# google-research/frame-interpolation

Measured on AMD Instinct MI355X. Metric: interpolated frames/sec @1080p, higher is better.
Workload: dtype f32; 1 GPU; 1080p_2x2: 1920x1080 pair, align 64, block_shape [2, 2] -> 4 tile(s) of 960x576 in one batch, film_net published config, seeded synthetic weights, t=0.5; parallelism=1 independent GPU(s), weights RCCL-broadcast once, exec=direct launches, two lanes, lanes=1

## Files before the change

### __graft_entry__.py

```python
import os
import sys

ROOT = os.path.dirname(os.path.abspath(__file__))
PKG = os.path.join(ROOT, 'frame-interpolation_amd')
for _p in (ROOT, PKG):
    if _p not in sys.path:
        sys.path.insert(0, _p)


def build() -> None:
    from film_hip import build as film_build
    out = film_build.build(verbose=True)
    if os.environ.get('FILM_EXTRA_FAMILIES', '0') in ('', '0'):
        os.environ['FILM_EXTRA_FAMILIES'] = '1'
        try:
            print('built', film_build.build(verbose=True))
        finally:
            os.environ['FILM_EXTRA_FAMILIES'] = '0'
    from film_hip import engine
    lib = engine.load_library()
    for sym in engine.EXPORTED_SYMBOLS:
        getattr(lib, sym)
    import eval.interpolator
    print('built', out, engine.FilmEngine.version())


def smoke() -> None:
    import numpy as np
    from film_hip import weights as W
    from film_hip.options import PUBLISHED
    from eval.interpolator import Interpolator
    from oracle import film_oracle as fo

    weights = W.make_synthetic_weights(PUBLISHED, seed=0)
    rng = np.random.default_rng(7)
    x0 = rng.random((1, 64, 64, 3), dtype=np.float32)
    x1 = np.roll(x0, (2, -1), axis=(1, 2)) + rng.normal(0, 0.01, x0.shape).astype(np.float32)
    it = Interpolator('', align=64, weights=weights, device=0)
    got = it(x0, x1, np.full((1,), 0.5, np.float32))
    want = fo.film_forward(x0, x1, weights, fo.Options())
    err = float(np.abs(got - want).max())
    print(f'smoke: hip vs oracle max|d| = {err:.3e}, psnr = {fo.psnr(got, want):.1f} dB')
    assert got.shape == want.shape and np.isfinite(got).all()
    assert err < 1e-3, f'smoke parity failed: {err}'


if __name__ == '__main__':
    if len(sys.argv) > 1 and sys.argv[1] == 'smoke':
        smoke()
    else:
        build()
```

### frame-interpolation_amd/csrc/conv_buf_impl.h

```cpp
#pragma once
#include "conv_common.h"

template <int BM, int BN, int WGM, int WGN, int FLAGS>
__global__ __launch_bounds__(WGM* WGN * 64) void conv_buf_kernel(ConvParams p) {
  constexpr int NW = WGM * WGN, NT = NW * 64;
  constexpr int WTM = BM / WGM, WTN = BN / WGN;
  constexpr int TM = WTM / 32, TN = WTN / 32;
  constexpr int RPP = NT / 4;
  constexpr int AR = BM / RPP;
  constexpr int BR = (BN + RPP - 1) / RPP;
  constexpr int STAGE = (BM + BN) * 16;
  static_assert(BM % RPP == 0 && TM >= 1 && TN >= 1 && RPP % 16 == 0, "bad tile");
  constexpr unsigned OOB = 0xFFFFFFFFu;

  extern __shared__ __attribute__((aligned(1024))) float smem[];

  const int t = threadIdx.x;
  const int lane = t & 63;
  const int wv = __builtin_amdgcn_readfirstlane(t >> 6);
  const int l31 = lane & 31, half = lane >> 5;
  const int wm = wv / WGN, wn = wv % WGN;

  int bx = blockIdx.x, by = blockIdx.y;
  if constexpr ((FLAGS & CONV_B_XCD_M) != 0) conv_xcd_remap(bx, by);
  const int m0 = bx * BM;
  const int n0 = by * BN;

  const int srow = t >> 2;
  const int scol = (t & 3) * 4;
  const int pcol = ((t & 3) ^ ((t >> 4) & 3)) * 4;
  const int ksz = p.ksize;
  const int pad = (ksz - 1) >> 1;
  const int fpy = p.fold == 2 ? (int)(blockIdx.z >> 1) : p.py, fpx = p.fold == 2 ? (int)(blockIdx.z & 1) : p.px;
  const int ntaps = p.fold == 2 ? (fpy + 1) * (fpx + 1) : p.fold ? p.ftaps : ksz * ksz;
  auto tap_dy = [&](int tp) { return p.fold == 2 ? (fpx ? tp >> 1 : tp) : p.fold ? (int)p.tdy[tp] : tp / ksz - pad; };
  auto tap_dx = [&](int tp) { return p.fold == 2 ? (fpx ? tp & 1 : 0) : p.fold ? (int)p.tdx[tp] : tp % ksz - pad; };
  const float* const wbase = p.fold == 2 ? p.w + p.fold_woff[blockIdx.z] : p.w;
  const int ksplit = p.fold ? 1 : (p.ksplit > 1 ? p.ksplit : 1);
  const int split = ksplit > 1 ? (int)blockIdx.z : 0;
  const int HW = p.H * p.W;
  int ab[AR], ay[AR], ax[AR];
  unsigned amask[AR];
#pragma unroll
  for (int i = 0; i < AR; ++i) {
    const int m = m0 + srow + RPP * i;
    const bool valid = m < p.M;
    const int mm = valid ? m : 0;
    const int b = mm / HW;
    const int r = mm - b * HW;
    const int y = r / p.W;
    const int x = r - y * p.W;
    ab[i] = b; ay[i] = y; ax[i] = x;
    unsigned mask = 0;
    for (int tp = 0; tp < ntaps; ++tp) {
      const int yy = y + tap_dy(tp), xx = x + tap_dx(tp);
      if (valid && yy >= 0 && yy < p.H && xx >= 0 && xx < p.W) mask |= 1u << tp;
    }
    amask[i] = mask;
  }
  const int Ktot = ntaps * p.Ctot;
  const conv_rsrc_t brsrc = conv_make_rsrc(wbase);
  unsigned boff[BR];
#pragma unroll
  for (int i = 0; i < BR; ++i) boff[i] = (unsigned)(((n0 + (srow + RPP * i) % BN) * Ktot + scol) * 4);
  const bool bstore = (BN % RPP == 0) || srow < BN;

  int tap = 0, sg = 0, c0 = 0, segC = p.seg[0].C;
  conv_rsrc_t arsrc = conv_make_rsrc(p.seg[0].ptr);
  unsigned aoff[AR];
  unsigned acen[AR];
  auto setup_seg = [&]() {
    const ConvSeg& s = p.seg[sg];
    arsrc = conv_make_rsrc(s.ptr);
    segC = s.C;
    if (!s.up) {
#pragma unroll
      for (int i = 0; i < AR; ++i) {
        int be = ab[i] + s.boff;
        if (s.bmod && be >= s.bmod) be -= s.bmod;
        acen[i] = (unsigned)((((size_t)be * p.H + ay[i]) * p.W + ax[i]) * s.stride + scol) * 4u;
      }
    }
  };
  auto setup_tap = [&]() {
    const ConvSeg& s = p.seg[sg];
    const int dy = tap_dy(tap), dx = tap_dx(tap);
    if (!s.up) {
      const unsigned delta = (unsigned)((dy * p.W + dx) * s.stride * 4);
#pragma unroll
      for (int i = 0; i < AR; ++i) aoff[i] = ((amask[i] >> tap) & 1u) ? acen[i] + delta : OOB;
    } else {
      const int Hs = p.H >> 1, Ws = p.W >> 1;
#pragma unroll
      for (int i = 0; i < AR; ++i) {
        const int yy = (ay[i] + dy) >> 1, xx = (ax[i] + dx) >> 1;
        int be = ab[i] + s.boff;
        if (s.bmod && be >= s.bmod) be -= s.bmod;
        const unsigned off = (unsigned)((((size_t)be * Hs + yy) * Ws + xx) * s.stride + scol) * 4u;
        aoff[i] = ((amask[i] >> tap) & 1u) ? off : OOB;
      }
    }
  };
  auto advance = [&]() {
    c0 += 16;
    if (c0 >= segC) {
      c0 = 0;
      if (++sg == p.nseg) { sg = 0; ++tap; }
      if (p.nseg > 1) setup_seg();
      setup_tap();
    }
  };

  struct Stage {
    bf4 a[AR];
    bf4 b[BR];
  };
  Stage sx, sy;
  const int nsteps_all = ntaps * (p.Ctot / 16);
  const int k_begin = (int)((long long)split * nsteps_all / ksplit);
  const int nsteps = (int)((long long)(split + 1) * nsteps_all / ksplit);
  int kstep = k_begin;
  if (k_begin > 0) {
    const int spt = p.Ctot / 16;
    tap = k_begin / spt;
    int rem = (k_begin - tap * spt) * 16;
    sg = 0;
    while (rem >= p.seg[sg].C) { rem -= p.seg[sg].C; ++sg; }
    c0 = rem;
  }
  auto load_global = [&](Stage& st) {
    const unsigned asoff = (unsigned)c0 * 4u;
#pragma unroll
    for (int i = 0; i < AR; ++i) st.a[i] = conv_buf_load(arsrc, aoff[i], asoff);
    const unsigned bsoff = (unsigned)(kstep < nsteps ? kstep : nsteps - 1) * 64u;
#pragma unroll
    for (int i = 0; i < BR; ++i) st.b[i] = conv_buf_load(brsrc, boff[i], bsoff);
    ++kstep;
    if (kstep < nsteps) advance();
    else {
#pragma unroll
      for (int i = 0; i < AR; ++i) aoff[i] = OOB;
    }
  };
  auto store_lds = [&](const Stage& st, int buf) {
    float* As = smem + buf * STAGE;
    float* Bs = As + BM * 16;
#pragma unroll
    for (int i = 0; i < AR; ++i) *reinterpret_cast<bf4*>(As + (srow + RPP * i) * 16 + pcol) = st.a[i];
    if (bstore) {
#pragma unroll
      for (int i = 0; i < BR; ++i) *reinterpret_cast<bf4*>(Bs + ((srow + RPP * i) % BN) * 16 + pcol) = st.b[i];
    }
  };

  f32x16 acc[TM][TN];
#pragma unroll
  for (int i = 0; i < TM; ++i)
#pragma unroll
    for (int j = 0; j < TN; ++j)
#pragma unroll
      for (int r = 0; r < 16; ++r) acc[i][j][r] = 0.f;

  const int sw = (l31 >> 2) & 3;
  const int ch0 = (half ^ sw) * 4, ch1 = ((2 + half) ^ sw) * 4;
  const int a_row = (wm * WTM + l31) * 16;
  const int b_row = (BM + wn * WTN + l31) * 16;
  auto compute = [&](int buf) {
    const float* S = smem + buf * STAGE;
    bf4 a[2][TM], b[2][TN];
#pragma unroll
    for (int mt = 0; mt < TM; ++mt) {
      a[0][mt] = *reinterpret_cast<const bf4*>(S + a_row + mt * 512 + ch0);
      a[1][mt] = *reinterpret_cast<const bf4*>(S + a_row + mt * 512 + ch1);
    }
#pragma unroll
    for (int nt = 0; nt < TN; ++nt) {
      b[0][nt] = *reinterpret_cast<const bf4*>(S + b_row + nt * 512 + ch0);
      b[1][nt] = *reinterpret_cast<const bf4*>(S + b_row + nt * 512 + ch1);
    }
#pragma unroll
    for (int kq = 0; kq < 2; ++kq)
#pragma unroll
      for (int j = 0; j < 4; ++j)
#pragma unroll
        for (int mt = 0; mt < TM; ++mt)
#pragma unroll
          for (int nt = 0; nt < TN; ++nt)
            acc[mt][nt] = __builtin_amdgcn_mfma_f32_32x32x2f32(b[kq][nt][j], a[kq][mt][j], acc[mt][nt], 0, 0, 0);
  };

  setup_seg();
  setup_tap();
  load_global(sx);
  load_global(sy);
  store_lds(sx, 0);
  __syncthreads();
  for (int s = k_begin; s < nsteps; s += 2) {
    load_global(sx);
    __builtin_amdgcn_sched_barrier(0);
    compute(0);
    __builtin_amdgcn_sched_barrier(0);
    store_lds(sy, 1);
    __syncthreads();
    load_global(sy);
    __builtin_amdgcn_sched_barrier(0);
    compute(1);
    __builtin_amdgcn_sched_barrier(0);
    store_lds(sx, 0);
    __syncthreads();
  }

#pragma unroll
  for (int mt = 0; mt < TM; ++mt) {
    const int m = m0 + wm * WTM + mt * 32 + l31;
    if (m >= p.M) continue;
    size_t opix = (size_t)m;
    if (p.fold) {
      const int bq = m / HW, rr = m - bq * HW, y = rr / p.W, x = rr - y * p.W;
      opix = ((size_t)bq * 2 * p.H + 2 * y + fpy) * (2 * p.W) + 2 * x + fpx;
    }
#pragma unroll
    for (int nt = 0; nt < TN; ++nt)
#pragma unroll
      for (int g = 0; g < 4; ++g) {
        const int n = n0 + wn * WTN + nt * 32 + 8 * g + 4 * half;
        bf4 v;
#pragma unroll
        for (int c = 0; c < 4; ++c) v[c] = acc[mt][nt][4 * g + c];
        if (ksplit > 1) {
          *reinterpret_cast<bf4*>(p.part + ((size_t)split * p.M + m) * p.Cout + n) = v;
          continue;
        }
#pragma unroll
        for (int c = 0; c < 4; ++c) {
          float u = v[c] + p.bias[n + c];
          if (p.leaky) u = leaky02(u);
          v[c] = u;
        }
        *reinterpret_cast<bf4*>(p.out + opix * p.ostride + n) = v;
      }
  }
}

template <int BM, int BN, int WGM, int WGN, int FLAGS>
hipError_t conv_buf_launch(const ConvParams& p, hipStream_t s) {
  constexpr size_t lds = 2 * (size_t)(BM + BN) * 16 * sizeof(float);
  if (p.ksplit > 1 && p.fold) return hipErrorInvalidValue;
  if (p.ksplit > 1 ? (p.Cout % 4 || (reinterpret_cast<uintptr_t>(p.part) & 15)) : (p.ostride % 4 || (reinterpret_cast<uintptr_t>(p.out) & 15))) return hipErrorInvalidValue;
  dim3 grid((p.M + BM - 1) / BM, p.Cout / BN, p.fold == 2 ? 4 : (p.ksplit > 1 ? p.ksplit : 1));
  return conv_launch<conv_buf_kernel<BM, BN, WGM, WGN, FLAGS>>(grid, dim3(WGM * WGN * 64), lds, s, p);
}
```

### frame-interpolation_amd/csrc/conv_common.h

```cpp
#pragma once
#include <atomic>
#include <type_traits>
#include <utility>

#include "film_kernels.h"

typedef float f32x16 __attribute__((ext_vector_type(16)));
typedef float bf4 __attribute__((ext_vector_type(4)));
typedef int bi4 __attribute__((ext_vector_type(4)));

enum : int {
  CONV_B_XCD_M = 4,
};

typedef __amdgpu_buffer_rsrc_t conv_rsrc_t;
__device__ __forceinline__ conv_rsrc_t conv_make_rsrc(const void* p) {
  return __builtin_amdgcn_make_buffer_rsrc(const_cast<void*>(p), 0, -1, 0x00020000);
}

__device__ __forceinline__ bf4 conv_buf_load(conv_rsrc_t rsrc, unsigned voff, unsigned soff) {
  return __builtin_bit_cast(bf4, __builtin_amdgcn_raw_buffer_load_b128(rsrc, (int)voff, (int)soff, 0));
}


struct ConvLdsAttrFlags { std::atomic<bool> set[64]; };
inline hipError_t conv_allow_dynamic_lds(const void* kern, ConvLdsAttrFlags& flags, int bytes) {
  int dev = 0;
  (void)hipGetDevice(&dev);
  const bool tracked = dev >= 0 && dev < 64;
  if (tracked && flags.set[dev].load(std::memory_order_relaxed)) return hipSuccess;
  const hipError_t e = hipFuncSetAttribute(kern, hipFuncAttributeMaxDynamicSharedMemorySize, bytes);
  if (e == hipSuccess && tracked) flags.set[dev].store(true, std::memory_order_relaxed);
  return e;
}

template <auto KERN>
hipError_t conv_launch(dim3 grid, dim3 block, size_t lds, hipStream_t s, const ConvParams& p, size_t lds_allow) {
  if (lds_allow > 64 * 1024) {
    static ConvLdsAttrFlags attr_flags;
    if (const hipError_t e = conv_allow_dynamic_lds(reinterpret_cast<const void*>(KERN), attr_flags, (int)lds_allow); e != hipSuccess) return e;
  }
  hipLaunchKernelGGL(KERN, grid, block, lds, s, p);
  return hipGetLastError();
}
template <auto KERN>
hipError_t conv_launch(dim3 grid, dim3 block, size_t lds, hipStream_t s, const ConvParams& p) { return conv_launch<KERN>(grid, block, lds, s, p, lds); }

inline unsigned conv_magic(unsigned long long d, unsigned long long xmax, bool& exact) {
  if (d <= 1) return 0u;
  if (xmax * d >= (1ull << 32)) { exact = false; return 0u; }
  return (unsigned)(((1ull << 32) + d - 1) / d);
}


template <class F, int... G>
__device__ __forceinline__ void conv_for_each(F&& f, std::integer_sequence<int, G...>) { (f(std::integral_constant<int, G>{}), ...); }

__device__ __forceinline__ unsigned conv_udiv(unsigned x, unsigned magic) {
  unsigned q;
  const unsigned h = __umulhi(x, magic);
  asm("s_cmp_eq_u32 %2, 0\n\ts_cselect_b32 %0, %1, %3" : "=s"(q) : "s"(x), "s"(magic), "s"(h) : "scc");
  return q;
}

__device__ __forceinline__ void conv_xcd_remap(int& bx, int& by) {
  const int nbx = gridDim.x, nby = gridDim.y;
  const int nwg = nbx * nby;
  const int lin = by * nbx + bx;
  const int xcd = lin & 7, idx = lin >> 3;
  const int q = nwg >> 3, r = nwg & 7;
  const int base = xcd < r ? xcd * (q + 1) : r * (q + 1) + (xcd - r) * q;
  const int nl = base + idx;
  bx = nl / nby;
  by = nl - bx * nby;
}
__device__ __forceinline__ float leaky02(float v) { return v > 0.f ? v : 0.2f * v; }

__device__ __forceinline__ const float* conv_uniform_ptr(const float* q) {
  const unsigned long long v = (unsigned long long)(uintptr_t)q;
  return reinterpret_cast<const float*>((uintptr_t)(((unsigned long long)(unsigned)__builtin_amdgcn_readfirstlane((int)(v >> 32)) << 32) |
                                                      (unsigned)__builtin_amdgcn_readfirstlane((int)(unsigned)v)));
}
```

### frame-interpolation_amd/csrc/conv_igemm.hip

```cpp
#include "conv_buf_impl.h"
#include "conv_wino43_impl.h"
#include "conv_wino2d_impl.h"
#include "conv_fold4_impl.h"
#include "conv_c3_impl.h"
#ifdef FILM_EXTRA_FAMILIES
#include "conv_halo_impl.h"
#include "conv_split_impl.h"
#include "conv_wino_impl.h"
#include "conv_winox3_impl.h"
#include "conv_foldx3_impl.h"
#endif

template <int F>
static hipError_t launch_shape(const ConvParams& p, int shape, hipStream_t s) {
  switch (shape) {
    case TILE_128x128: return conv_buf_launch<128, 128, 2, 2, F>(p, s);
    case TILE_256x64: return conv_buf_launch<256, 64, 4, 1, F>(p, s);
    case TILE_256x32: return conv_buf_launch<256, 32, 4, 1, F>(p, s);
    case TILE_64x64: return conv_buf_launch<64, 64, 2, 2, F>(p, s);
    case TILE_128x32: return conv_buf_launch<128, 32, 4, 1, F>(p, s);
    case TILE_128x64: return conv_buf_launch<128, 64, 2, 2, F>(p, s);
    case TILE_256x128: return conv_buf_launch<256, 128, 4, 2, F>(p, s);
    default: return hipErrorInvalidValue;
  }
}

static hipError_t launch_c3(const ConvParams& p, int shape, hipStream_t s) {
  if (shape != TILE_C3_DIRECT) return hipErrorInvalidValue;
  return p.Cout % 64 == 0 ? conv_c3_launch<64>(p, s) : conv_c3_launch<32>(p, s);
}

#ifdef FILM_EXTRA_FAMILIES
template <int F>
static hipError_t launch_halo(const ConvParams& p, int shape, hipStream_t s) {
  switch (shape) {
    case HALO_8x128: return conv_halo_launch<8, 128, 4, 2, F>(p, s);
    case HALO_8x64: return conv_halo_launch<8, 64, 4, 1, F>(p, s);
    case HALO_8x32: return conv_halo_launch<8, 32, 4, 1, F>(p, s);
    case HALO_4x64: return conv_halo_launch<4, 64, 4, 1, F>(p, s);
    case HALO_4x128: return conv_halo_launch<4, 128, 2, 2, F>(p, s);
    case HALO_4x32: return conv_halo_launch<4, 32, 4, 1, F>(p, s);
    default: return hipErrorInvalidValue;
  }
}

template <int F, int NP>
static hipError_t launch_split(const ConvParams& p, int shape, hipStream_t s) {
  switch (shape) {
    case HALO_8x128: return conv_halo_split_launch<8, 128, 4, 2, NP, F>(p, s);
    case HALO_8x64: return conv_halo_split_launch<8, 64, 4, 1, NP, F>(p, s);
    case HALO_8x32: return conv_halo_split_launch<8, 32, 4, 1, NP, F>(p, s);
    case HALO_4x64: return conv_halo_split_launch<4, 64, 4, 1, NP, F>(p, s);
    case HALO_4x128: return conv_halo_split_launch<4, 128, 2, 2, NP, F>(p, s);
    case HALO_4x32: return conv_halo_split_launch<4, 32, 4, 1, NP, F>(p, s);
    default: return hipErrorInvalidValue;
  }
}

template <int F>
static hipError_t launch_wino(const ConvParams& p, int shape, hipStream_t s) {
  switch (shape) {
    case WINO_4x128: return conv_wino_launch<4, 128, 4, 2, F>(p, s);
    case WINO_4x64: return conv_wino_launch<4, 64, 4, 1, F>(p, s);
    case WINO_4x128_W16: return conv_wino_launch<4, 128, 4, 4, F>(p, s);
    case WINO_4x32: return conv_wino_launch<4, 32, 4, 1, F>(p, s);
    case WINO_8x64_W16: return conv_wino_launch<8, 64, 8, 2, F>(p, s);
    case WINO_8x32_W8: return conv_wino_launch<8, 32, 8, 1, F>(p, s);
    case WINO_2x64: return conv_wino_launch<2, 64, 2, 2, F>(p, s);
    case WINO_4x64_W8: return conv_wino_launch<4, 64, 4, 2, F>(p, s);
    default: return hipErrorInvalidValue;
  }
}

#endif

template <int F>
static hipError_t launch_wino43(const ConvParams& p, int shape, hipStream_t s) {
  switch (shape) {
    case W43_Q16_4x64_T21_P2: return conv_wino43_launch<4, 64, 2, 1, F | W43_F_PF2, 16>(p, s);
    case W43_Q16_4x32_T11_P2: return conv_wino43_launch<4, 32, 1, 1, F | W43_F_PF2, 16>(p, s);
    case W43_Q16_4x64_N1_P2: return conv_wino43_launch<4, 64, 1, 1, F | W43_F_PF2, 16, 1>(p, s);
    case W43_Q8_8x64_T21_P2: return conv_wino43_launch<8, 64, 2, 1, F | W43_F_PF2, 8>(p, s);
    case W43_Q8_8x64_N1_P2: return conv_wino43_launch<8, 64, 1, 1, F | W43_F_PF2, 8, 1>(p, s);
    case W43_Q8_8x32_T11_BG: return conv_wino43_launch<8, 32, 1, 1, F | W43_F_BG, 8>(p, s);
    case W43_Q8_8x32_T11_P2: return conv_wino43_launch<8, 32, 1, 1, F | W43_F_PF2, 8>(p, s);
#ifdef FILM_EXTRA_FAMILIES
    case W43_4x64_T21: return conv_wino43_launch<4, 64, 2, 1, F>(p, s);
    case W43_4x64_T12: return conv_wino43_launch<4, 64, 1, 2, F>(p, s);
    case W43_4x32_T11: return conv_wino43_launch<4, 32, 1, 1, F>(p, s);
    case W43_Q16_4x64_T21: return conv_wino43_launch<4, 64, 2, 1, F, 16>(p, s);
    case W43_Q16_4x64_T12: return conv_wino43_launch<4, 64, 1, 2, F, 16>(p, s);
    case W43_Q16_4x32_T11: return conv_wino43_launch<4, 32, 1, 1, F, 16>(p, s);
    case W43_Q16_4x64_N1: return conv_wino43_launch<4, 64, 1, 1, F, 16, 1>(p, s);
    case W43_Q16_4x64_T12_P2: return conv_wino43_launch<4, 64, 1, 2, F | W43_F_PF2, 16>(p, s);
    case W43_Q16_4x32_T11_BG: return conv_wino43_launch<4, 32, 1, 1, F | W43_F_BG, 16>(p, s);
    case W43_Q8_8x64_T12_P2: return conv_wino43_launch<8, 64, 1, 2, F | W43_F_PF2, 8>(p, s);
#endif
    default: return hipErrorInvalidValue;
  }
}

template <int F>
static hipError_t launch_wino2d(const ConvParams& p, int shape, hipStream_t s) {
  switch (shape) {
    case W2D_8x64: return conv_wino2d_launch_any<64, F>(p, s);
    case W2D_8x32: return conv_wino2d_launch_any<32, F>(p, s);
    case W2D_8x32_S2: return conv_wino2d_launch_any<32, F, 2>(p, s);
    case W2D_16x64: return conv_wino2d_launch_any<64, F | W2D_F_SQ>(p, s);
    case W2D_16x32: return conv_wino2d_launch_any<32, F | W2D_F_SQ>(p, s);
    case W2D_16x32_S2: return conv_wino2d_launch_any<32, F | W2D_F_SQ, 2>(p, s);
    default: return hipErrorInvalidValue;
  }
}

template <int F>
static hipError_t launch_fold4(const ConvParams& p, int shape, hipStream_t s) {
  switch (shape) {
    case F4_4x64: return conv_fold4_launch<2, F>(p, s);
    case F4_4x32: return conv_fold4_launch<1, F>(p, s);
    default: return hipErrorInvalidValue;
  }
}

#ifdef FILM_EXTRA_FAMILIES
template <int F>
static hipError_t launch_winox3(const ConvParams& p, int shape, hipStream_t s) {
  switch (shape) {
    case WX3_4x128_T22: return conv_winox3_launch<4, 128, 2, 2, F>(p, s);
    case WX3_4x64_T12: return conv_winox3_launch<4, 64, 1, 2, F>(p, s);
    case WX3_4x64_T21: return conv_winox3_launch<4, 64, 2, 1, F>(p, s);
    case WX3_4x32_T11: return conv_winox3_launch<4, 32, 1, 1, F>(p, s);
    default: return hipErrorInvalidValue;
  }
}

template <int F>
static hipError_t launch_foldx3(const ConvParams& p, int shape, hipStream_t s) {
  switch (shape) {
    case FX3_4x64: return conv_foldx3_launch<4, 64, 4, 1, F>(p, s);
    case FX3_8x64: return conv_foldx3_launch<8, 64, 8, 1, F>(p, s);
    case FX3_4x128: return conv_foldx3_launch<4, 128, 4, 2, F>(p, s);
    default: return hipErrorInvalidValue;
  }
}
#endif


__global__ __launch_bounds__(256) void conv_splitk_reduce_kernel(const float* __restrict__ part, const float* __restrict__ bias,
                                                                 float* __restrict__ out, int M, int Cout, int ostride,
                                                                 int S, int leaky) {
  const int G = Cout >> 2;
  const unsigned idx = blockIdx.x * 256u + threadIdx.x;
  if (idx >= (unsigned)M * (unsigned)G) return;
  const unsigned m = idx / (unsigned)G, g = idx - m * (unsigned)G;
  const size_t plane = (size_t)M * Cout;
  const float4* src = reinterpret_cast<const float4*>(part + (size_t)m * Cout + g * 4);
  float4 a = *reinterpret_cast<const float4*>(bias + g * 4);
  for (int sidx = 0; sidx < S; ++sidx) {
    const float4 v = src[(size_t)sidx * (plane >> 2)];
    a.x += v.x; a.y += v.y; a.z += v.z; a.w += v.w;
  }
  if (leaky) {
    a.x = a.x > 0.f ? a.x : 0.2f * a.x; a.y = a.y > 0.f ? a.y : 0.2f * a.y;
    a.z = a.z > 0.f ? a.z : 0.2f * a.z; a.w = a.w > 0.f ? a.w : 0.2f * a.w;
  }
  *reinterpret_cast<float4*>(out + (size_t)m * ostride + g * 4) = a;
}

static hipError_t film_launch_conv_main(const ConvParams& p, int fam, int tile, hipStream_t s) {
  const int shape = conv_tile_shape(tile);
  const bool xcd = tile & CONV_TILE_XCD;
  if ((p.pool_out != nullptr || p.pw_out != nullptr) && kConvFamily[fam].fused_shape < 0) return hipErrorInvalidValue;
  switch (fam) {
    case FAM_BUF: return xcd ? launch_shape<CONV_B_XCD_M>(p, shape, s) : launch_shape<0>(p, shape, s);
    case FAM_C3: return launch_c3(p, shape, s);
    case FAM_FOLD4: return xcd ? launch_fold4<CONV_B_XCD_M>(p, shape, s) : launch_fold4<0>(p, shape, s);
    case FAM_W2D:
      if (p.ksize != 3) return hipErrorInvalidValue;
      return xcd ? launch_wino2d<CONV_B_XCD_M>(p, shape, s) : launch_wino2d<0>(p, shape, s);
    case FAM_W43:
      if (p.ksize != 3) return hipErrorInvalidValue;
      if (p.pool_out != nullptr && shape < W43_Q16_4x64_T21) return hipErrorInvalidValue;
      if (p.pw_out != nullptr && ((shape != W43_Q16_4x64_N1 && shape != W43_Q16_4x64_N1_P2 && shape != W43_Q8_8x64_N1_P2) || p.Cout != 64 || p.ksplit > 1 ||
                                  p.pool_out != nullptr || p.pw_cout < 1 || p.pw_cout > 4))
        return hipErrorInvalidValue;
      return xcd ? launch_wino43<CONV_B_XCD_M>(p, shape, s) : launch_wino43<0>(p, shape, s);
#ifdef FILM_EXTRA_FAMILIES
    case FAM_HALO:
      if (p.ksize != 3) return hipErrorInvalidValue;
      return xcd ? launch_halo<CONV_B_XCD_M>(p, shape, s) : launch_halo<0>(p, shape, s);
    case FAM_SPLIT6:
      if (p.ksize != 3) return hipErrorInvalidValue;
      return xcd ? launch_split<CONV_B_XCD_M, 6>(p, shape, s) : launch_split<0, 6>(p, shape, s);
    case FAM_SPLIT3:
      if (p.ksize != 3) return hipErrorInvalidValue;
      return xcd ? launch_split<CONV_B_XCD_M, 3>(p, shape, s) : launch_split<0, 3>(p, shape, s);
    case FAM_WINO:
      if (p.ksize != 3) return hipErrorInvalidValue;
      return xcd ? launch_wino<CONV_B_XCD_M>(p, shape, s) : launch_wino<0>(p, shape, s);
    case FAM_WINOX3:
      if (p.ksize != 3) return hipErrorInvalidValue;
      return xcd ? launch_winox3<CONV_B_XCD_M>(p, shape, s) : launch_winox3<0>(p, shape, s);
    case FAM_FOLDX3:
      if (p.ksize != 2 || p.fold != 2) return hipErrorInvalidValue;
      return xcd ? launch_foldx3<CONV_B_XCD_M>(p, shape, s) : launch_foldx3<0>(p, shape, s);
#endif
    default: return hipErrorNotSupported;
  }
}

hipError_t film_launch_conv(const ConvParams& p, int tile, hipStream_t s) {
  const int fam = conv_family_of(tile);
  if (fam < 0 || (p.ksplit > 1 && !kConvFamily[fam].splitk)) return hipErrorInvalidValue;
  const hipError_t e = film_launch_conv_main(p, fam, tile, s);
  if (e != hipSuccess || p.ksplit <= 1) return e;
  const long long Mout = (long long)p.M * (p.fold == 3 ? 4 : 1);
  if (!p.part || (p.Cout & 3) || Mout * (p.Cout >> 2) >= (1ll << 32)) return hipErrorInvalidValue;
  const unsigned units = (unsigned)Mout * (unsigned)(p.Cout >> 2);
  hipLaunchKernelGGL(conv_splitk_reduce_kernel, dim3((units + 255) / 256), dim3(256), 0, s, p.part, p.bias, p.out, (int)Mout, p.Cout,
                     p.ostride, p.ksplit, p.leaky);
  return hipGetLastError();
}
```

### frame-interpolation_amd/csrc/conv_wino2d_impl.h

```cpp
#pragma once
#include "conv_common.h"

enum { W2D_F_SQ = 128,
       W2D_F_XEPI = 8,
       W2D_DBG_TIME = 8192 };


template <bool SQ> struct W2dSlotTable { unsigned v[24 * 64]; };
template <bool SQ> constexpr W2dSlotTable<SQ> w2d_make_slot_table() {
  constexpr int QW = SQ ? 4 : 8, TH = SQ ? 16 : 8, HR = TH + 2, PW = 4 * QW + 2;
  constexpr int CO4 = (PW + 3) / 4, MO4 = 4 * CO4, RP4 = 4 * MO4 + (SQ ? 2 : 4);
  W2dSlotTable<SQ> t{};
  for (int sl = 0; sl < 24 * 64; ++sl) {
    const int r = sl / RP4, rem = sl % RP4, m = rem / MO4, rr = rem % MO4, c = rr / CO4, k = rr % CO4, px = 4 * k + m;
    const bool ok = r < HR && rem < 4 * MO4 && px < PW;
    t.v[sl] = ok ? ((unsigned)r << 24 | (unsigned)px << 8 | (unsigned)c << 4) : 0xFFFFFFFFu;
  }
  return t;
}
template <bool SQ> __device__ const W2dSlotTable<SQ> w2d_slot_table = w2d_make_slot_table<SQ>();

template <int BN, int FLAGS, int NS_ = 3>
__global__ __launch_bounds__(4 * (BN / 32) * 64, (BN == 32) ? 2 : 1) void conv_wino2d_kernel(ConvParams p) {
  constexpr bool SQ = (FLAGS & W2D_F_SQ) != 0;
  constexpr int QW = SQ ? 4 : 8, TH = SQ ? 16 : 8, HR = TH + 2, PXW = 4 * QW, PW = PXW + 2;
  static_assert(QW * (TH / 2) == 32, "32 units per tile");
  constexpr int NG = BN / 32, NW = 4 * NG;
  constexpr int CO4 = (PW + 3) / 4, MO4 = 4 * CO4, RP4 = 4 * MO4 + (SQ ? 2 : 4);
  constexpr int NREQ = 24;
  constexpr int STAGE4 = NREQ * 64;
  constexpr int NS = NS_;
  static_assert(NS == 2 || NS == 3, "stages");
  constexpr int IPW = NREQ / NW;
  static_assert(NREQ % NW == 0, "requests per wave");
  static_assert(HR * RP4 <= STAGE4, "stage size");
  constexpr bool XE = (FLAGS & W2D_F_XEPI) != 0;
  constexpr unsigned OOB = 0xFFFFFFFFu;

  extern __shared__ __attribute__((aligned(1024))) float smem[];

  const int t = threadIdx.x;
  const int lane = t & 63;
  const int wv = __builtin_amdgcn_readfirstlane(t >> 6);
  const int l31 = lane & 31, half = lane >> 5;
  const int mu = wv & 3, ng = wv >> 2;

  unsigned long long tm0 = 0, tm1 = 0, tm2 = 0, tmA = 0, tmB = 0, tmC = 0, tmW = 0, tmE1 = 0, tmE2 = 0, tmE3 = 0;
  unsigned long long rt0 = 0;
  if constexpr ((FLAGS & W2D_DBG_TIME) != 0) { rt0 = __builtin_amdgcn_s_memrealtime(); tm0 = __builtin_readcyclecounter(); }

  int aH = p.H, aW = p.W, aNB = p.NB, aCtot = p.Ctot, aKsplit = p.ksplit, aNseg = p.nseg, aUnused = p.unused_chain;
  unsigned a_tpi = p.mg_tpi, a_ntx = p.mg_ntx, a_nby = p.mg_nby;
  int ntx_ = p.tl_ntx, tpi_ = p.tl_tpi;
  int aGx = (int)gridDim.x, aGy = (int)gridDim.y;
  const float* aS0ptr = p.seg[0].ptr;
  int aS0stride = p.seg[0].stride, aS0C = p.seg[0].C, aS0boff = p.seg[0].boff, aS0bmod = p.seg[0].bmod;
  const float* aWptr = p.w;
  unsigned rtab[(24 / (4 * (BN / 32)))];
#pragma unroll
  for (int n = 0; n < 24 / NW; ++n) rtab[n] = w2d_slot_table<SQ>.v[t + 64 * NW * n];
  {
    unsigned long long q0 = (unsigned long long)(uintptr_t)aS0ptr, q1 = (unsigned long long)(uintptr_t)aWptr;
    asm volatile("" : "+s"(aH), "+s"(aW), "+s"(aNB), "+s"(aCtot), "+s"(aKsplit), "+s"(aNseg), "+s"(aUnused), "+s"(a_tpi), "+s"(a_ntx), "+s"(a_nby), "+s"(ntx_), "+s"(tpi_),
                      "+s"(aGx), "+s"(aGy), "+s"(q0), "+s"(q1), "+s"(aS0stride), "+s"(aS0C), "+s"(aS0boff), "+s"(aS0bmod));
    aS0ptr = reinterpret_cast<const float*>((uintptr_t)q0);
    aWptr = reinterpret_cast<const float*>((uintptr_t)q1);
  }
  unsigned long long tmK = 0, tmT = 0;
  if constexpr ((FLAGS & W2D_DBG_TIME) != 0) tmK = __builtin_readcyclecounter();
  int bx = blockIdx.x, by = blockIdx.y;
  if constexpr ((FLAGS & CONV_B_XCD_M) != 0) {
    const int nbx = aGx, nby = aGy;
    const int nwg = nbx * nby;
    const int lin = by * nbx + bx;
    const int xcd = lin & 7, idx = lin >> 3;
    const int q = nwg >> 3, r = nwg & 7;
    const int base = xcd < r ? xcd * (q + 1) : r * (q + 1) + (xcd - r) * q;
    const int nl = base + idx;
    bx = (int)conv_udiv((unsigned)nl, a_nby);
    by = nl - bx * nby;
  }
  const int ntx = ntx_, tpi = tpi_;
  const int img = (int)conv_udiv((unsigned)bx, a_tpi);
  const int trow0 = (int)conv_udiv((unsigned)(bx - img * tpi), a_ntx);
  const int y0 = trow0 * TH, x0 = (bx - img * tpi - trow0 * ntx) * PXW;
  const int n0 = by * BN;

  unsigned rvoff[IPW];
  int rsg = 0, rc0 = 0, rsegC = 0;
  conv_rsrc_t rrsrc = conv_make_rsrc(conv_uniform_ptr(aS0ptr));
  const unsigned lds0 = (unsigned)(size_t)(__attribute__((address_space(3))) float*)smem;
  unsigned rpk[IPW];
  auto set_rpk = [&]() {
    const int H = aH, W = aW;
    const bool inside = y0 >= 1 && y0 + TH + 1 <= H && x0 >= 1 && x0 + PXW + 1 <= W;
    if (inside) {
#pragma unroll
      for (int n = 0; n < IPW; ++n) rpk[n] = rtab[n];
    } else {
#pragma unroll
      for (int n = 0; n < IPW; ++n) {
        const unsigned tv = rtab[n];
        const unsigned y = (unsigned)(y0 - 1) + (tv >> 24), x = (unsigned)(x0 - 1) + ((tv >> 8) & 255u);
        rpk[n] = ((y < (unsigned)H) & (x < (unsigned)W)) ? tv : OOB;
      }
    }
  };
  set_rpk();
#pragma unroll
  for (int n = 0; n < IPW; ++n) asm volatile("" : "+v"(rpk[n]));
  if constexpr ((FLAGS & W2D_DBG_TIME) != 0) tmT = __builtin_readcyclecounter();
  auto raw_setup_seg_of = [&](const float* sptr, int sstride, int sC, int sboff, int sbmod) {
    rsegC = __builtin_amdgcn_readfirstlane(sC);
    int be = img + sboff;
    if (sbmod && be >= sbmod) be -= sbmod;
    const int spix = (be * aH + (y0 - 1)) * aW + (x0 - 1);
    rrsrc = conv_make_rsrc(conv_uniform_ptr(sptr + (long long)spix * sstride));
    const unsigned st4 = (unsigned)sstride * 4u;
    const unsigned wst4 = (unsigned)aW * st4;
#pragma unroll
    for (int n = 0; n < IPW; ++n) {
      const unsigned tv = rpk[n];
      unsigned off, tmp;
      asm("v_and_b32 %0, 48, %2\n\tv_bfe_u32 %1, %2, 8, 8\n\tv_mad_u32_u24 %0, %1, %3, %0\n\tv_lshrrev_b32 %1, 24, %2\n\tv_mad_u32_u24 %0, %1, %4, %0"
          : "=&v"(off), "=&v"(tmp) : "v"(tv), "s"(st4), "s"(wst4));
      rvoff[n] = tv == OOB ? OOB : off;
    }
  };
  auto raw_setup_seg = [&]() {
    const ConvSeg& s = p.seg[rsg];
    raw_setup_seg_of(s.ptr, s.stride, s.C, s.boff, s.bmod);
  };
  auto dma_piece = [&](int n, int stage) {
    const unsigned so = (unsigned)rc0 * 4u;
    const unsigned base = lds0 + (unsigned)stage * (STAGE4 * 16u) + (unsigned)(wv + NW * n) * 1024u;
    asm volatile("s_mov_b32 m0, %0\n\ts_nop 0\n\tbuffer_load_dwordx4 %1, %2, %3 offen lds" ::"s"(base), "v"(rvoff[n]), "s"(rrsrc), "s"(so)
                 : "memory");
  };
  auto dma_advance = [&]() {
    rc0 += 16;
    if (rc0 >= rsegC) {
      if (rsg + 1 < aNseg) { rc0 = 0; ++rsg; raw_setup_seg(); }
    }
  };
  const int ksp = XE && aKsplit > 1 ? aKsplit : 1;
  const int nsc_all = aCtot >> 4;
  int sc0 = 0, sc1 = nsc_all;
  if (ksp > 1) {
    sc0 = (int)((unsigned)nsc_all * blockIdx.z / (unsigned)ksp);
    sc1 = (int)((unsigned)nsc_all * (blockIdx.z + 1u) / (unsigned)ksp);
    int c = sc0 * 16;
    while (rsg + 1 < aNseg && c >= p.seg[rsg].C) { c -= p.seg[rsg].C; ++rsg; }
    rc0 = c;
  }
  auto raw_issue = [&](int stage) {
#pragma unroll
    for (int n = 0; n < IPW; ++n) dma_piece(n, stage);
    dma_advance();
  };

  const int nkc = aCtot / 8, nsc = sc1 - sc0, kc0 = 2 * sc0, kc1 = 2 * sc1;
  const conv_rsrc_t brsrc = conv_make_rsrc(conv_uniform_ptr(aWptr));
  const unsigned bvoff = (unsigned)((half * 32 + l31) * 16);
  const int ct = n0 / 32 + ng;
  auto slab = [&](int kc) { return (unsigned)(((ct * nkc + (kc < nkc ? kc : nkc - 1)) * 4 + mu) * 6) * 1024u; };
  bf4 fbg[2][6];

  f32x16 acc[6];

  const bf4* const smem4 = reinterpret_cast<const bf4*>(smem);
  const int ur = l31 / QW, lq = l31 % QW;
  const int ra = mu == 0 ? 0 : mu == 2 ? 2 : 1, rb = mu == 0 ? 2 : mu == 1 ? 2 : mu == 2 ? 1 : 3;
  const float sgn = mu == 1 ? 1.f : -1.f;
  const int ix_a = (2 * ur + ra) * RP4 + half * CO4 + lq, ix_b = (2 * ur + rb) * RP4 + half * CO4 + lq;
  typedef float f2 __attribute__((ext_vector_type(2)));
  f2 A[2][6][2];
  bf4 d[6];
  bf4 d2[6];

  using C0 = std::integral_constant<int, 0>;
  using C1 = std::integral_constant<int, 1>;
  auto read_row = [&](bf4 (&dst)[6], int ix, int stage, auto h_c) {
    constexpr int IMM = decltype(h_c)::value * 2 * CO4;
    const int ixs = ix + stage * STAGE4;
#pragma unroll
    for (int j = 0; j < 6; ++j) dst[j] = smem4[ixs + IMM + (j & 3) * MO4 + (j >> 2)];
  };
  auto pair_of = [](const bf4& v, int q) -> f2 { return q ? f2{v[2], v[3]} : f2{v[0], v[1]}; };
  auto set_pair = [](bf4& v, int q, f2 x) { if (q) { v[2] = x[0]; v[3] = x[1]; } else { v[0] = x[0]; v[1] = x[1]; } };
  auto fma2 = [](float k, f2 x, f2 y) -> f2 {
    f2 r;
    const f2 kk = {k, k};
    asm("v_pk_fma_f32 %0, %1, %2, %3" : "=v"(r) : "s"(kk), "v"(x), "v"(y));
    return r;
  };
  auto add2 = [](f2 x, f2 y) -> f2 { f2 r; asm("v_pk_add_f32 %0, %1, %2" : "=v"(r) : "v"(x), "v"(y)); return r; };
  auto mul2 = [](float k, f2 x) -> f2 {
    f2 r;
    const f2 kk = {k, k};
    asm("v_pk_mul_f32 %0, %1, %2" : "=v"(r) : "s"(kk), "v"(x));
    return r;
  };
  auto max1 = [](float x, float y) -> float { float r; asm("v_max_f32 %0, %1, %2" : "=v"(r) : "v"(x), "v"(y)); return r; };
  auto sub2 = [](f2 x, f2 y) -> f2 { f2 r; asm("v_pk_add_f32 %0, %1, %2 neg_lo:[0,1] neg_hi:[0,1]" : "=v"(r) : "v"(x), "v"(y)); return r; };
  f2 xt[4];
  auto xf_t = [&](int q) {
    const f2 d1 = pair_of(d[1], q), d2v = pair_of(d[2], q), d3 = pair_of(d[3], q), d4 = pair_of(d[4], q);
    xt[0] = fma2(-4.f, d2v, d4);
    xt[1] = fma2(-4.f, d1, d3);
    xt[2] = sub2(d4, d2v);
    xt[3] = sub2(d3, d1);
  };
  auto xf_v = [&](int q, int nu) -> f2 {
    switch (nu) {
      case 0: return fma2(4.f, pair_of(d[0], q), fma2(-5.f, pair_of(d[2], q), pair_of(d[4], q)));
      case 1: return add2(xt[0], xt[1]);
      case 2: return sub2(xt[0], xt[1]);
      case 3: return fma2(2.f, xt[3], xt[2]);
      case 4: return fma2(-2.f, xt[3], xt[2]);
      default: return fma2(4.f, pair_of(d[1], q), fma2(-5.f, pair_of(d[3], q), pair_of(d[5], q)));
    }
  };
  auto pin = [](f2& v) { asm volatile("" : "+v"(v)); };
  auto prepare = [&](f2 (&An)[6][2], int stage, auto h_c) {
    read_row(d, ix_a, stage, h_c);
    read_row(d2, ix_b, stage, h_c);
#pragma unroll
    for (int j = 0; j < 6; ++j)
#pragma unroll
      for (int q = 0; q < 2; ++q) set_pair(d[j], q, fma2(sgn, pair_of(d2[j], q), pair_of(d[j], q)));
#pragma unroll
    for (int q = 0; q < 2; ++q) {
      xf_t(q);
#pragma unroll
      for (int nu = 0; nu < 6; ++nu) An[nu][q] = xf_v(q, nu);
    }
  };

  if (ksp > 1) raw_setup_seg();
  else raw_setup_seg_of(aS0ptr, aS0stride, aS0C, aS0boff, aS0bmod);
  raw_issue(0);
  if constexpr ((FLAGS & W2D_DBG_TIME) != 0) tmA = __builtin_readcyclecounter();
#pragma unroll
  for (int j = 0; j < 6; ++j) fbg[0][j] = conv_buf_load(brsrc, bvoff, slab(kc0) + (unsigned)j * 1024u);
  __builtin_amdgcn_sched_barrier(0);
  asm volatile("s_waitcnt vmcnt(6)" ::: "memory");
  if constexpr ((FLAGS & W2D_DBG_TIME) != 0) tmB = __builtin_readcyclecounter();
  __syncthreads();
  if constexpr ((FLAGS & W2D_DBG_TIME) != 0) tmC = __builtin_readcyclecounter();
#pragma unroll
  for (int j = 0; j < 6; ++j) fbg[1][j] = conv_buf_load(brsrc, bvoff, slab(kc0 + 1) + (unsigned)j * 1024u);
  __builtin_amdgcn_sched_barrier(0);
  if (nsc > 1) raw_issue(1);
  if constexpr (NS > 2) { if (nsc > 2) raw_issue(2); }
  prepare(A[0], 0, C0{});

  int st_s = 0, st_n = 1;
  int st_dma = 0;
  bool dma_on = false;
  int gs = 0;
  constexpr int P1 = NS == 2 ? IPW : (IPW + 1) / 2, P0 = IPW - P1;
  auto dma_slot = [](int g, int cnt) constexpr -> int {
    if (cnt <= 0) return -1;
    if (cnt == 6) return g == 2 ? 0 : (g >= 5 && (g - 5) % 4 == 0) ? 1 + (g - 5) / 4 : -1;
    const int step = 24 / cnt, at = cnt == 1 ? 13 : 5;
    return (g % step == at && g / step < cnt) ? g / step : -1;
  };
  auto chunk = [&](int kc, auto h_c, auto first_c, auto last_c) {
    constexpr int H = decltype(h_c)::value;
    constexpr bool FIRST = decltype(first_c)::value != 0;
    constexpr bool LAST = decltype(last_c)::value != 0;
    constexpr bool PREP = !(LAST && H == 1);
    using RH = std::integral_constant<int, 1 - H>;
    const int rs = H == 0 ? st_s : st_n;
    f2(&Ac)[6][2] = A[H];
    f2(&An)[6][2] = A[1 - H];
    if constexpr (H == 1 && !LAST) {
      unsigned long long tw0 = 0;
      if constexpr ((FLAGS & W2D_DBG_TIME) != 0) tw0 = __builtin_readcyclecounter();
      if (NS == 2 || gs == 0) asm volatile("s_waitcnt vmcnt(6)" ::: "memory");
      else asm volatile("s_waitcnt vmcnt(12)" ::: "memory");
      __syncthreads();
      if constexpr ((FLAGS & W2D_DBG_TIME) != 0) tmW += __builtin_readcyclecounter() - tw0;
      dma_on = (kc >> 1) + NS < sc1;
      st_dma = st_s;
    }
    const unsigned so2 = LAST ? 0u : slab(kc + 2);
    __builtin_amdgcn_sched_barrier(0);
    auto gap = [&](auto g_c) {
      constexpr int g = decltype(g_c)::value;
      constexpr int jp = g >> 3, i8 = g & 7, k = i8 >> 1, j = 2 * jp + (i8 & 1);
      if constexpr (FIRST && k == 0) {
        const f32x16 zero = {0.f, 0.f, 0.f, 0.f, 0.f, 0.f, 0.f, 0.f, 0.f, 0.f, 0.f, 0.f, 0.f, 0.f, 0.f, 0.f};
        acc[j] = __builtin_amdgcn_mfma_f32_32x32x2f32(fbg[H][j][k], Ac[j][k >> 1][k & 1], zero, 0, 0, 0);
      } else {
        acc[j] = __builtin_amdgcn_mfma_f32_32x32x2f32(fbg[H][j][k], Ac[j][k >> 1][k & 1], acc[j], 0, 0, 0);
      }
      if constexpr (!LAST) {
        if constexpr (k == 3) fbg[H][j] = conv_buf_load(brsrc, bvoff, so2 + (unsigned)j * 1024u);
      }
      if constexpr (PREP) {
        if constexpr (g == 0) read_row(d, ix_a, rs, RH{});
        if constexpr (g == 1) read_row(d2, ix_b, rs, RH{});
        if constexpr (g >= 4 && g < 10) {
          constexpr int jj = g - 4;
#pragma unroll
          for (int q = 0; q < 2; ++q) { f2 v = fma2(sgn, pair_of(d2[jj], q), pair_of(d[jj], q)); pin(v); set_pair(d[jj], q, v); }
        }
        if constexpr (g >= 10 && g < 16) {
          constexpr int q = (g - 10) / 3, part = (g - 10) % 3;
          if constexpr (part == 0) {
            xf_t(q);
            pin(xt[0]); pin(xt[1]); pin(xt[2]); pin(xt[3]);
          } else if constexpr (part == 1) {
            An[0][q] = xf_v(q, 0);
            An[5][q] = xf_v(q, 5);
            pin(An[0][q]); pin(An[5][q]);
          } else {
#pragma unroll
            for (int nu = 1; nu < 5; ++nu) { An[nu][q] = xf_v(q, nu); pin(An[nu][q]); }
          }
        }
      }
      if constexpr (!LAST) {
        constexpr int CNT = H == 1 ? P1 : P0, N0 = H == 1 ? 0 : P1;
        constexpr int idx = dma_slot(g, CNT);
        if constexpr (idx >= 0) {
          if (dma_on) {
            dma_piece(N0 + idx, st_dma);
            if constexpr (N0 + idx == IPW - 1) dma_advance();
          }
        }
      }
      __builtin_amdgcn_sched_barrier(0);
    };
    conv_for_each(gap, std::make_integer_sequence<int, 24>{});
    if constexpr (H == 1) {
      st_s = st_n;
      st_n = st_n + 1 == NS ? 0 : st_n + 1;
      ++gs;
    }
  };

  auto epilogue = [&]() {
    const int t = threadIdx.x, lane = t & 63, l31 = lane & 31, half = lane >> 5;
    __syncthreads();
    if constexpr ((FLAGS & W2D_DBG_TIME) != 0) tmE1 = __builtin_readcyclecounter();
    float o[4][16];
  #pragma unroll
    for (int r = 0; r < 16; ++r) {
      const float m0 = acc[0][r], m1 = acc[1][r], m2 = acc[2][r], m3 = acc[3][r], m4 = acc[4][r], m5 = acc[5][r];
      const float s34 = m3 + m4, d34 = m3 - m4, d12 = m1 - m2, s12 = m1 + m2;
      o[0][r] = ((m0 + m1) + m2) + s34;
      o[1][r] = __builtin_fmaf(2.f, d34, d12);
      o[2][r] = __builtin_fmaf(4.f, s34, s12);
      o[3][r] = d12 + __builtin_fmaf(8.f, d34, m5);
    }
    bf4* const xb = reinterpret_cast<bf4*>(smem);
    constexpr int XB4 = NG * 4 * 256;
    static_assert(2 * XB4 <= NS * STAGE4, "exchange buffers");
    const int widx = (ng * 4 + mu) * 256 + l31 * 8;
    const int rng = t >> 8, run = (t >> 3) & 31, rcg = t & 7;
    const int ridx = rng * 1024 + run * 8 + (rcg ^ (run & 7));
    const int nrd = n0 + rng * 32 + rcg * 4;
    const bool rawsum = XE && ksp > 1;
    const bool has_pw = XE && p.pw_out != nullptr;
    float b0 = 0.f, b1 = 0.f, b2 = 0.f, b3 = 0.f;
    if (!rawsum) { const float* const bp = p.bias + nrd; b0 = bp[0]; b1 = bp[1]; b2 = bp[2]; b3 = bp[3]; }
    const int oy = y0 + 2 * (run / QW), ox = x0 + 4 * (run % QW);
    const int ostr = rawsum ? p.Cout : p.ostride;
    const float slope = (p.leaky && !rawsum) ? 0.2f : 1.f;
    const int dyo = 2 * (run / QW), dxo = 4 * (run % QW), nth = rng * 32 + rcg * 4;
    const int cpix = (img * p.H + y0) * p.W + x0;
    float* obase = p.out;
    if (rawsum) { asm volatile(""); obase = p.part + (size_t)blockIdx.z * p.M * p.Cout; }
    float* const ocorner = obase + ((long long)cpix * ostr + n0);
    float* const orow = ocorner + (__umul24(__umul24(dyo, p.W) + dxo, ostr) + nth);
    float* pool_base = nullptr;
    if (XE && p.pool_out) {
      asm volatile("");
      const int ppix = (img * (p.H >> 1) + (y0 >> 1)) * (p.W >> 1) + (x0 >> 1);
      pool_base = p.pool_out + ((long long)ppix * p.pool_ostride + n0) + (__umul24(__umul24(dyo >> 1, p.W >> 1) + (dxo >> 1), p.pool_ostride) + nth);
    }
    constexpr int PWS = 68;
    float* const pwt = smem + 2 * XB4 * 4;
    float* const pww = pwt + TH * PXW * PWS;
    if (has_pw && t < 256) pww[t] = (t & 3) < p.pw_cout ? p.pw_w[(t >> 2) * p.pw_cout + (t & 3)] : 0.f;
    bf4 k0 = {0.f, 0.f, 0.f, 0.f}, k1 = {0.f, 0.f, 0.f, 0.f};
    auto write_round = [&](int jx, bf4* xw) {
  #pragma unroll
      for (int g = 0; g < 4; ++g) {
        bf4 v;
        v[0] = o[jx][4 * g]; v[1] = o[jx][4 * g + 1]; v[2] = o[jx][4 * g + 2]; v[3] = o[jx][4 * g + 3];
        xw[widx + ((2 * g + half) ^ (l31 & 7))] = v;
      }
    };
  #pragma unroll
    for (int jx = 0; jx < 4; ++jx) {
      bf4* const xw = xb + (jx & 1) * XB4;
      write_round(jx, xw);
      __syncthreads();
      if constexpr ((FLAGS & W2D_DBG_TIME) != 0) { if (jx == 0) tmE2 = __builtin_readcyclecounter(); if (jx == 3) tmE3 = __builtin_readcyclecounter(); }
      const bf4 m0 = xw[ridx], m1 = xw[ridx + 256], m2 = xw[ridx + 512], m3 = xw[ridx + 768];
      bf4 r0, r1;
  #pragma unroll
      for (int q = 0; q < 2; ++q) {
        const f2 bq = q ? f2{b2, b3} : f2{b0, b1};
        const f2 v0 = add2(add2(add2(pair_of(m0, q), pair_of(m1, q)), pair_of(m2, q)), bq);
        const f2 v1 = add2(sub2(sub2(pair_of(m1, q), pair_of(m2, q)), pair_of(m3, q)), bq);
        const f2 s0 = mul2(slope, v0), s1 = mul2(slope, v1);
        set_pair(r0, q, f2{max1(v0[0], s0[0]), max1(v0[1], s0[1])});
        set_pair(r1, q, f2{max1(v1[0], s1[0]), max1(v1[1], s1[1])});
      }
      if (!has_pw) {
        if (ox + jx < p.W) {
          float* const o0 = orow + (size_t)jx * ostr;
          if (oy < p.H) *reinterpret_cast<bf4*>(o0) = r0;
          if (oy + 1 < p.H) *reinterpret_cast<bf4*>(o0 + (size_t)p.W * ostr) = r1;
        }
        if (XE && pool_base != nullptr) {
          if (jx & 1) {
            bf4 pv;
  #pragma unroll
            for (int c = 0; c < 4; ++c) pv[c] = (((k0[c] + r0[c]) + k1[c]) + r1[c]) * 0.25f;
            if (oy < p.H && ox + jx < p.W) *reinterpret_cast<bf4*>(pool_base + (size_t)(jx >> 1) * p.pool_ostride) = pv;
          } else {
            k0 = r0; k1 = r1;
          }
        }
      } else {
        float* const tr = pwt + ((2 * (run / QW)) * PXW + 4 * (run % QW) + jx) * PWS + rng * 32 + rcg * 4;
        *reinterpret_cast<bf4*>(tr) = r0;
        *reinterpret_cast<bf4*>(tr + PXW * PWS) = r1;
      }
    }
    if (has_pw) {
      __syncthreads();
      if (t < TH * PXW) {
        const int y = y0 + t / PXW, x = x0 + (t % PXW);
        float a[4] = {0.f, 0.f, 0.f, 0.f};
        const bf4* row = reinterpret_cast<const bf4*>(pwt + t * PWS);
        const bf4* wq = reinterpret_cast<const bf4*>(pww);
  #pragma unroll 4
        for (int c4 = 0; c4 < 16; ++c4) {
          const bf4 v = row[c4];
  #pragma unroll
          for (int k = 0; k < 4; ++k) {
            const bf4 w = wq[c4 * 4 + k];
  #pragma unroll
            for (int j = 0; j < 4; ++j) a[j] = __builtin_fmaf(v[k], w[j], a[j]);
          }
        }
        if (y < p.H && x < p.W) {
          float* dd = p.pw_out + (((size_t)img * p.H + y) * p.W + x) * p.pw_ostride;
  #pragma unroll
          for (int j = 0; j < 4; ++j)
            if (j < p.pw_cout) dd[j] = a[j] + p.pw_bias[j];
        }
      }
    }
  };
  if constexpr ((FLAGS & W2D_DBG_TIME) != 0) tm1 = __builtin_readcyclecounter();
  for (int tile = 0; tile < 1; ++tile) {
    chunk(kc0, C0{}, C1{}, C0{});
    chunk(kc0 + 1, C1{}, C0{}, C0{});
    for (int kc = kc0 + 2; kc < kc1 - 2; kc += 2) {
      chunk(kc, C0{}, C0{}, C0{});
      chunk(kc + 1, C1{}, C0{}, C0{});
    }
    if (nsc > 1) {
      chunk(kc1 - 2, C0{}, C0{}, C1{});
      chunk(kc1 - 1, C1{}, C0{}, C1{});
    }
    if constexpr ((FLAGS & W2D_DBG_TIME) != 0) tm2 = __builtin_readcyclecounter();
    epilogue();
  }
  if constexpr ((FLAGS & W2D_DBG_TIME) != 0) {
    const unsigned long long tm3 = __builtin_readcyclecounter();
    if (t == 0) {
      unsigned long long* o8 = reinterpret_cast<unsigned long long*>(p.part) + (size_t)(blockIdx.y * gridDim.x + blockIdx.x) * 16;
      o8[0] = tm0; o8[1] = tm1; o8[2] = tm2; o8[3] = tm3; o8[4] = tmA; o8[5] = tmB; o8[6] = tmC; o8[7] = tmW;
      o8[8] = rt0; o8[9] = __builtin_amdgcn_s_memrealtime();
      o8[10] = (unsigned long long)__builtin_amdgcn_s_getreg((31 << 11) | 4) | ((unsigned long long)__builtin_amdgcn_s_getreg((31 << 11) | 20) << 32);
      o8[11] = tmE1; o8[12] = tmE2; o8[13] = tmE3; o8[14] = tmK; o8[15] = tmT;
    }
  }
}

template <int BN, int FLAGS, int NS = 3>
hipError_t conv_wino2d_launch(const ConvParams& p, hipStream_t s) {
  if (!(FLAGS & W2D_F_XEPI) && (p.ksplit > 1 || p.pool_out || p.pw_out)) return hipErrorInvalidValue;
  const size_t lds = p.pw_out ? (size_t)2 * (BN / 32) * 16 * 1024 + 256 * 68 * 4 + 1024 : (size_t)NS * 24 * 1024;
  constexpr int NT = 4 * (BN / 32) * 64;
  if (p.ksize != 3 || p.Ctot % 16 || p.Cout % BN) return hipErrorInvalidValue;
  if (p.ksplit > 1 && (!p.part || (reinterpret_cast<uintptr_t>(p.part) & 15) || p.Cout % 4 || p.pool_out || p.pw_out || p.ksplit > p.Ctot / 16)) return hipErrorInvalidValue;
  if (p.pw_out) {
    if (BN != 64 || p.Cout != 64 || p.pool_out || p.pw_cout < 1 || p.pw_cout > 4) return hipErrorInvalidValue;
  } else if (p.ostride % 4 || (reinterpret_cast<uintptr_t>(p.out) & 15)) return hipErrorInvalidValue;
  if (p.pool_out && ((p.H | p.W) & 1 || p.pool_ostride % 4 || (reinterpret_cast<uintptr_t>(p.pool_out) & 15))) return hipErrorInvalidValue;
  {
    long long nimg = p.NB;
    for (int i = 0; i < p.nseg; ++i) nimg = std::max<long long>(nimg, (long long)p.seg[i].bmod);
    if ((nimg + 1) * p.H * p.W >= (1ll << 31)) return hipErrorInvalidValue;
  }
  if (p.W <= 0 || p.H <= 0 || p.W >= (1 << 20) || p.ostride >= (1 << 22) || p.pool_ostride >= (1 << 22) || p.Cout >= (1 << 22) ||
      (long long)8 * p.W * (p.ostride > p.Cout ? p.ostride : p.Cout) >= (1ll << 31)) return hipErrorInvalidValue;
  for (int i = 0; i < p.nseg; ++i)
    if ((long long)p.W * p.seg[i].stride * 4 >= (1ll << 24) || p.seg[i].C % 16 || p.seg[i].stride % 4 || p.seg[i].stride <= 0 || p.seg[i].stride >= (1 << 22) || p.seg[i].up || (reinterpret_cast<uintptr_t>(p.seg[i].ptr) & 15)) return hipErrorInvalidValue;
  constexpr bool SQ = (FLAGS & W2D_F_SQ) != 0;
  const int ntx = SQ ? (p.W + 15) / 16 : (p.W + 31) / 32, nty = SQ ? (p.H + 15) / 16 : (p.H + 7) / 8;
  const int ntiles = p.NB * ntx * nty;
  dim3 grid((unsigned)ntiles, p.Cout / BN, (unsigned)(p.ksplit > 1 ? p.ksplit : 1));
  ConvParams q = p;
  bool exact = true;
  q.mg_nby = conv_magic(grid.y, (unsigned long long)grid.x * grid.y, exact);
  q.mg_tpi = conv_magic((unsigned long long)ntx * nty, (unsigned long long)ntiles + 1, exact);
  q.mg_ntx = conv_magic(ntx, (unsigned long long)ntx * nty, exact);
  q.tl_ntx = ntx; q.tl_tpi = ntx * nty;
  if (!exact) return hipErrorInvalidValue;
  return conv_launch<conv_wino2d_kernel<BN, FLAGS, NS>>(grid, dim3(NT), lds, s, q, 144 * 1024);
}

template <int BN, int FLAGS, int NS = 3>
hipError_t conv_wino2d_launch_any(const ConvParams& p, hipStream_t s) {
  if (p.ksplit > 1 || p.pool_out || p.pw_out) return conv_wino2d_launch<BN, FLAGS | W2D_F_XEPI, NS>(p, s);
  return conv_wino2d_launch<BN, FLAGS, NS>(p, s);
}
```

### frame-interpolation_amd/csrc/film_engine.cpp

```cpp
#include "film_internal.h"

namespace film_internal {

thread_local std::string g_create_error;

int fail(film_t* h, int code, const char* fmt, ...) {
  char buf[1024];
  va_list ap;
  va_start(ap, fmt);
  vsnprintf(buf, sizeof buf, fmt, ap);
  va_end(ap);
  if (h) h->err = buf; else g_create_error = buf;
  return code;
}

int copy_out_string(film_t* h, const std::string& s, char* buf, int64_t cap, int64_t* needed) {
  if (needed) *needed = (int64_t)s.size() + 1;
  if (!buf || cap < (int64_t)s.size() + 1) {
    if (!buf && needed) return FILM_OK;
    return fail(h, FILM_ERR_INVALID, "buffer too small: need %lld bytes", (long long)s.size() + 1);
  }
  memcpy(buf, s.c_str(), s.size() + 1);
  return FILM_OK;
}

}

using namespace film_internal;

namespace {

enum OptNorm { AS_IS, BOOL, NONNEG, LOW5 };
struct OptionRow {
  const char* key;
  int film_t::*field;
  OptNorm norm;
  bool drops_plans;
  int64_t lo = 0, hi = 0;
  const char* refusal = nullptr;
  ConvFamily family = FAM_BUF;
  int need_lo = 0, need_hi = 0;
  const char* family_refusal = nullptr;
};
constexpr OptionRow kOptions[] = {
    {"graph", &film_t::opt_graph, AS_IS, false, 0, 2, "graph: 0 (one stream, eager), 1 (hipGraph replay) or 2 (two lanes, eager: the default)"},
    {"profile", &film_t::opt_profile, BOOL, false},
    {"autotune", &film_t::opt_autotune, BOOL, false},
    {"max_batch", &film_t::opt_max_batch, NONNEG, false},
    {"host_overlap", &film_t::opt_host_overlap, BOOL, false},
    {"block_overlap_h", &film_t::opt_block_overlap_h, AS_IS, false, -1, 65535, "block_overlap_h: -1 (what the align padding of a tile holds) or 0 .. 65535 rows"},
    {"block_overlap_w", &film_t::opt_block_overlap_w, AS_IS, false, -1, 65535, "block_overlap_w: -1 (what the align padding of a tile holds) or 0 .. 65535 columns"},
    {"tune_ms", &film_t::opt_tune_ms, NONNEG, false},
    {"splitk", &film_t::opt_splitk, BOOL, true},
    {"pack_groups", nullptr, AS_IS, false, 1, 4, "pack_groups: 1 .. 4"},
    {"fuse", &film_t::opt_fuse, LOW5, true},
    {"fold2x2", &film_t::opt_fold2x2, AS_IS, true, 0, 2, "fold2x2: 0, 1 or 2"},
    {"planar", &film_t::opt_planar, BOOL, true},
    {"winograd", &film_t::opt_wino, AS_IS, true, 0, 3, "winograd: 0, 1, 2 or 3", FAM_WINO, 2, 2,
     "winograd = 2 (F(2,3) kernel on every level) needs a library built with FILM_EXTRA_FAMILIES=1"},
    {"halo_all", &film_t::opt_halo_all, BOOL, true, 0, 0, nullptr, FAM_HALO, 1, 1, "halo_all needs a library built with FILM_EXTRA_FAMILIES=1"},
    {"lanes", &film_t::opt_lanes, AS_IS, true, 0, 3, "lanes: 0, 1, 2 or 3"},
    {"wino2d", &film_t::opt_wino2d, AS_IS, true, 0, 2, "wino2d: 0, 1 or 2"},
    {"w2d_small_px", &film_t::opt_w2d_small_px, AS_IS, true, 0, 1 << 30, "w2d_small_px: pixels per image, 0 = never"},
    {"w2d_min_px", &film_t::opt_w2d_min_px, AS_IS, true, 1, 1 << 30, "w2d_min_px: pixels per image"},
    {"w2d_splitk", &film_t::opt_w2d_splitk, AS_IS, true, 0, 16, "w2d_splitk: 0 (off), 1 (default rule) or 2..16 (A/B: the cap on levels of <= 1024 pixels)"},
    {"w2d_shape", &film_t::opt_w2d_shape, AS_IS, true, -1, W2D_SHAPES - 1, "w2d_shape: -1 (autotuned) or a Wino2dTile shape index"},
    {"fold4_shape", &film_t::opt_fold4_shape, AS_IS, true, -1, F4_4x32, "fold4_shape: -1 (autotuned) or a Fold4Tile shape index"},
    {"w43_shape", &film_t::opt_w43_shape, AS_IS, true, -1, 31, "w43_shape: -1 (autotuned) or a Wino43Tile shape index"},
    {"precision", &film_t::opt_precision, AS_IS, true, 0, 2, "precision: 0 (f32), 1 (bf16x6) or 2 (bf16x3)", FAM_SPLIT6, 1, 2,
     "precision %d (bf16 split modes) needs a library built with FILM_EXTRA_FAMILIES=1; this build runs fp32 MFMA only"},
};
constexpr bool option_rows_complete() {
  for (const OptionRow& o : kOptions)
    if ((o.lo < o.hi) != (o.refusal != nullptr) || ((o.family != FAM_BUF) != (o.family_refusal != nullptr))) return false;
  return true;
}
static_assert(option_rows_complete(), "a row with a range (a family) carries its refusal message, a row without leaves lo = hi (family = FAM_BUF)");

int tile_geometry(film_t* h, int H, int W, int block_h, int block_w, int align, TileMapParams* tp) {
  const int bh = block_h > 0 ? block_h : 1, bw = block_w > 0 ? block_w : 1;
  if (H % bh) return fail(h, FILM_ERR_INVALID, "block_height=%d should evenly divide height=%d.", bh, H);
  if (W % bw) return fail(h, FILM_ERR_INVALID, "block_width=%d should evenly divide width=%d.", bw, W);
  tp->H = H; tp->W = W; tp->bh = bh; tp->bw = bw; tp->ph = H / bh; tp->pw = W / bw;
  struct Axis { const char* key; int nb, p, want; int *ov, *e, *T, *off; };
  const Axis axes[2] = {{"block_overlap_h", bh, tp->ph, h->opt_block_overlap_h, &tp->ovy, &tp->eh, &tp->TH, &tp->oy},
                        {"block_overlap_w", bw, tp->pw, h->opt_block_overlap_w, &tp->ovx, &tp->ew, &tp->TW, &tp->ox}};
  for (const Axis& a : axes) {
    const int pad0 = (align > 0 && a.p % align) ? align - a.p % align : 0;
    const int o = a.nb == 1 ? 0 : a.want < 0 ? std::min(pad0 / 2, a.p / 2) : a.want;
    if (2 * (int64_t)o > a.p)
      return fail(h, FILM_ERR_INVALID, "%s: twice the overlap (%d) must not exceed the patch size %d", a.key, o, a.p);
    const int e = a.p + 2 * o;
    const int pad = (align > 0 && e % align) ? align - e % align : 0;
    *a.ov = o; *a.e = e; *a.T = e + pad; *a.off = pad / 2;
  }
  return FILM_OK;
}
hipError_t cut_tiles(const TileMapParams& tp, hipStream_t s) {
  return (tp.ovy | tp.ovx) ? film_launch_frame_to_tiles_overlap(tp, s) : film_launch_frame_to_tiles(tp, s);
}
hipError_t join_tiles(const TileMapParams& tp, hipStream_t s) {
  return (tp.ovy | tp.ovx) ? film_launch_blend_tiles(tp, s) : film_launch_tiles_to_frame(tp, s);
}
int pix_layout(int pix) { return pix & 0xff; }
bool pix_is_yuv(int pix) { return pix_layout(pix) == FILM_PIX_I420 || pix_layout(pix) == FILM_PIX_NV12; }
int check_pix(film_t* h, int pix, int H, int W) {
  const int layout = pix_layout(pix), flags = pix & ~0xff;
  if (layout != FILM_PIX_F32 && layout != FILM_PIX_U8 && !pix_is_yuv(pix))
    return fail(h, FILM_ERR_INVALID, "bad pix layout %d: FILM_PIX_F32 (0), FILM_PIX_U8 (1), FILM_PIX_I420 (16) or FILM_PIX_NV12 (17)", layout);
  if (flags & ~(FILM_YUV_BT601 | FILM_YUV_FULL))
    return fail(h, FILM_ERR_INVALID, "bad pix 0x%x: unknown bits 0x%x set (flags: FILM_YUV_BT601 0x100, FILM_YUV_FULL 0x400)", (unsigned)pix,
                (unsigned)(flags & ~(FILM_YUV_BT601 | FILM_YUV_FULL)));
  if (flags && !pix_is_yuv(pix))
    return fail(h, FILM_ERR_INVALID, "bad pix 0x%x: the colour flags belong to FILM_PIX_I420 / FILM_PIX_NV12, not to an RGB layout", (unsigned)pix);
  if (pix_is_yuv(pix) && H > 0 && W > 0 && ((H | W) & 1))
    return fail(h, FILM_ERR_INVALID, "pix: 4:2:0 needs even sizes, got %d x %d", H, W);
  return FILM_OK;
}
size_t frame_bytes(int pix, int H, int W) {
  const size_t px = (size_t)H * W;
  return pix_is_yuv(pix) ? px + px / 2 : pix_layout(pix) == FILM_PIX_U8 ? px * 3 : px * 3 * sizeof(float);
}
hipError_t cut_tiles_pix(const TileMapParams& tp, int pix, hipStream_t s) {
  if (pix_layout(pix) == FILM_PIX_F32) return cut_tiles(tp, s);
  const uint8_t* src = reinterpret_cast<const uint8_t*>(tp.src);
  if (pix_is_yuv(pix))
    return film_launch_yuv420_to_tiles(tp, src, pix_layout(pix) == FILM_PIX_NV12, (pix & FILM_YUV_BT601) != 0, (pix & FILM_YUV_FULL) != 0, s);
  return (tp.ovy | tp.ovx) ? film_launch_frame_to_tiles_overlap_u8(tp, src, s) : film_launch_frame_to_tiles_u8(tp, src, s);
}
int ensure_stage(film_t* h, size_t bytes, hipStream_t s) {
  if (h->stage_bytes >= bytes) return FILM_OK;
  if (h->stage) { HIPCHK(h, hipStreamSynchronize(s)); HIPCHK(h, hipFree(h->stage)); h->stage = nullptr; h->stage_bytes = 0; }
  hipError_t e = hipMalloc(&h->stage, bytes);
  if (e != hipSuccess) return fail(h, FILM_ERR_NOMEM, "frame staging hipMalloc of %.1f MB failed", bytes * 1e-6);
  h->stage_bytes = bytes;
  return FILM_OK;
}
int balanced_chunk(int n, int maxc) {
  if (n <= maxc) return n;
  for (int c = maxc; 2 * c > maxc; --c)
    if (n % c == 0) return c;
  return maxc;
}
void sequence_chunk(int n, int T, int cap, int* k, int* nt) {
  int bk = 0, bt = 1;
  for (int t = std::min(T, cap); t >= 1; --t) {
    const int kk = std::min(n, cap / t);
    if (kk > bk) { bk = kk; bt = t; }
  }
  *k = balanced_chunk(n, std::max(bk, 1));
  *nt = balanced_chunk(T, bt);
}
int need_device(film_t* h, const char* fn) {
  if (h->plan_only) return fail(h, FILM_ERR_NO_DEVICE, "plan-only handle: %s needs a HIP device (no CPU fallback)", fn);
  if (!h->finalized) return fail(h, FILM_ERR_STATE, "film_finalize has not been called");
  return FILM_OK;
}
bool halve_on_nomem(int rc, int* chunk) {
  if (rc != FILM_ERR_NOMEM || *chunk <= 1) return false;
  *chunk = (*chunk + 1) / 2;
  return true;
}
struct FrameStage {
  film_t* h; hipStream_t s; bool host;
  float* result; size_t out_floats;
  float* out = nullptr;
  size_t used = 0;
  int open(size_t in_floats) {
    out = result;
    if (!host) return FILM_OK;
    int rc = ensure_stage(h, (in_floats + out_floats) * sizeof(float), s);
    if (rc == FILM_OK) out = (float*)h->stage + in_floats;
    return rc;
  }
  int upload(const float* src, size_t floats, const float** dev) {
    *dev = src;
    if (!host) return FILM_OK;
    HIPCHK(h, hipMemcpyAsync((float*)h->stage + used, src, floats * sizeof(float), hipMemcpyHostToDevice, s));
    *dev = (float*)h->stage + used;
    used += floats;
    return FILM_OK;
  }
  int finish() {
    if (!host) return FILM_OK;
    HIPCHK(h, hipMemcpyAsync(result, out, out_floats * sizeof(float), hipMemcpyDeviceToHost, s));
    HIPCHK(h, hipStreamSynchronize(s));
    return FILM_OK;
  }
};
template <class T> struct TileCopy { T* frames; int tile0, ntiles; int64_t slot; };
using Cut = TileCopy<const float>;
using Join = TileCopy<float>;
int run_chunk(film_t* h, Plan* P, TileMapParams tp, const std::vector<Cut>& cuts, const std::vector<Join>& joins, hipStream_t s) {
  const int64_t tile_floats = (int64_t)tp.TH * tp.TW * 3;
  for (const Cut& c : cuts) {
    tp.tile0 = c.tile0; tp.ntiles = c.ntiles; tp.src = c.frames; tp.dst = P->at("img0") + c.slot * tile_floats;
    HIPCHK(h, cut_tiles(tp, s));
  }
  int rc = run_plan(h, P, s);
  if (rc) return rc;
  for (const Join& j : joins) {
    tp.tile0 = j.tile0; tp.ntiles = j.ntiles; tp.src = P->at("out") + j.slot * tile_floats; tp.dst = j.frames;
    HIPCHK(h, join_tiles(tp, s));
  }
  return FILM_OK;
}

hipStream_t pick_stream(film_t* h, int mem_kind, void* stream) {
  return stream ? (hipStream_t)stream : (mem_kind == FILM_MEM_DEVICE ? (hipStream_t) nullptr : h->stream);
}

int forward_chunk(film_t* h, const float* x0, const float* x1, int B, int H, int W, float* out, int mem_kind, void* stream) {
  HIPCHK(h, hipSetDevice(h->device));
  Plan* P = nullptr;
  int rc = get_plan(h, B, H, W, true, &P);
  if (rc) return rc;
  hipStream_t s = pick_stream(h, mem_kind, stream);
  const size_t in_bytes = (size_t)B * H * W * 3 * sizeof(float);
  const hipMemcpyKind kin = mem_kind == FILM_MEM_HOST ? hipMemcpyHostToDevice : hipMemcpyDeviceToDevice;
  const hipMemcpyKind kout = mem_kind == FILM_MEM_HOST ? hipMemcpyDeviceToHost : hipMemcpyDeviceToDevice;
  HIPCHK(h, hipMemcpyAsync(P->at("img0"), x0, in_bytes, kin, s));
  HIPCHK(h, hipMemcpyAsync(P->at("img0") + (int64_t)B * H * W * 3, x1, in_bytes, kin, s));
  rc = run_plan(h, P, s);
  if (rc) return rc;
  HIPCHK(h, hipMemcpyAsync(out, P->at("out"), in_bytes, kout, s));
  if (mem_kind == FILM_MEM_HOST) HIPCHK(h, hipStreamSynchronize(s));
  return FILM_OK;
}

int interpolate_host_pipeline(film_t* h, Plan* P, TileMapParams tp, const float* x0, const float* x1, float* out, float* st, size_t frame_bytes, hipStream_t s) {
  const int nt = P->B;
  const size_t nf = frame_bytes / sizeof(float);
  for (hipEvent_t& e : h->pipe_ev)
    if (!e) HIPCHK(h, hipEventCreateWithFlags(&e, hipEventDisableTiming));
  LanePipe lp;
  for (size_t i = 0; i < P->ops.size() && lp.head.size() < 2; ++i) {
    const OpDesc& op = P->ops[i];
    if (op.lane == 1) continue;
    if (!batch_splittable(op, 2) || !op.xdeps.empty() || op.NB != 2 * nt) break;
    lp.head.push_back(i);
  }
  const OpDesc& last = P->ops.back();
  lp.tail = tp.B == 1 && tp.bh % 2 == 0 && last.lane == 0 && last.pw_out.buf >= 0 && last.NB == nt && batch_splittable(last, 2) && P->ops.size() > lp.head.size() + 1 &&
            std::find(lp.head.begin(), lp.head.end(), P->ops.size() - 1) == lp.head.end();
  tp.tile0 = 0;
  lp.mid_tail = [&]() -> hipError_t {
    TileMapParams t2 = tp;
    t2.ntiles = nt / 2; t2.src = P->at("out"); t2.dst = st + 2 * nf;
    hipError_t e = film_launch_tiles_to_frame(t2, s);
    if (e == hipSuccess) e = hipEventRecord(h->pipe_ev[1], s);
    return e;
  };
  struct Drain {
    film_t* h; hipStream_t s; bool armed;
    ~Drain() { if (armed) { (void)hipStreamSynchronize(h->stream2); (void)hipStreamSynchronize(s); } }
  } drain{h, s, true};
  HIPCHK(h, hipMemcpyAsync(st, x0, frame_bytes, hipMemcpyHostToDevice, s));
  tp.ntiles = nt; tp.src = st; tp.dst = P->at("img0");
  HIPCHK(h, film_launch_frame_to_tiles(tp, s));
  HIPCHK(h, hipEventRecord(h->pipe_ev[0], s));
  HIPCHK(h, hipStreamWaitEvent(h->stream2, h->pipe_ev[0], 0));
  for (size_t i : lp.head) HIPCHK(h, launch_op(batch_part(P->ops[i], 0, 2), P->arena, h->packed_dev, s));
  HIPCHK(h, hipMemcpyAsync(st + nf, x1, frame_bytes, hipMemcpyHostToDevice, h->stream2));
  tp.src = st + nf; tp.dst = P->at("img0") + (int64_t)nt * tp.TH * tp.TW * 3;
  HIPCHK(h, film_launch_frame_to_tiles(tp, h->stream2));
  HIPCHK(h, hipEventRecord(h->pipe_ev[0], h->stream2));
  HIPCHK(h, hipStreamWaitEvent(s, h->pipe_ev[0], 0));
  const hipError_t le = issue_lanes(h, P, s, false, &lp);
  if (le != hipSuccess) return fail(h, FILM_ERR_HIP, "kernel launch failed: %s", hipGetErrorString(le));
  h->last_plan = P;
  const int64_t tile_floats = (int64_t)tp.TH * tp.TW * 3;
  if (lp.tail) {
    TileMapParams t2 = tp;
    t2.tile0 = nt / 2; t2.ntiles = nt - nt / 2; t2.src = P->at("out") + (int64_t)(nt / 2) * tile_floats; t2.dst = st + 2 * nf;
    HIPCHK(h, film_launch_tiles_to_frame(t2, s));
    const size_t half = frame_bytes / 2;
    HIPCHK(h, hipStreamWaitEvent(h->stream2, h->pipe_ev[1], 0));
    HIPCHK(h, hipMemcpyAsync(out, st + 2 * nf, half, hipMemcpyDeviceToHost, h->stream2));
    HIPCHK(h, hipMemcpyAsync((char*)out + half, (const char*)(st + 2 * nf) + half, frame_bytes - half, hipMemcpyDeviceToHost, s));
    HIPCHK(h, hipStreamSynchronize(h->stream2));
  } else {
    tp.tile0 = 0; tp.ntiles = nt; tp.src = P->at("out"); tp.dst = st + 2 * nf;
    HIPCHK(h, film_launch_tiles_to_frame(tp, s));
    HIPCHK(h, hipMemcpyAsync(out, st + 2 * nf, frame_bytes, hipMemcpyDeviceToHost, s));
  }
  HIPCHK(h, hipStreamSynchronize(s));
  drain.armed = false;
  return FILM_OK;
}

void stream_free(film_t* h) {
  FilmStream& fs = h->fs;
  for (void* p : {fs.keep, (void*)fs.result, (void*)fs.result8})
    if (p) (void)hipFree(p);
  fs = FilmStream{};
}
bool same_geometry(const TileMapParams& a, const TileMapParams& b) {
  const int va[] = {a.H, a.W, a.bh, a.bw, a.ph, a.pw, a.TH, a.TW, a.oy, a.ox, a.ovy, a.ovx, a.eh, a.ew};
  const int vb[] = {b.H, b.W, b.bh, b.bw, b.ph, b.pw, b.TH, b.TW, b.oy, b.ox, b.ovy, b.ovx, b.eh, b.ew};
  return std::equal(std::begin(va), std::end(va), std::begin(vb));
}
hipError_t stream_cut(const FilmStream& fs, TileMapParams tp, const Plan* P, int slot, hipStream_t s) {
  tp.tile0 = 0; tp.ntiles = tp.bh * tp.bw;
  tp.src = (const float*)fs.keep;
  tp.dst = P->at("img0") + (int64_t)slot * tp.ntiles * tp.TH * tp.TW * 3;
  return cut_tiles_pix(tp, fs.pix, s);
}

int debug_plan(film_t* h, int B, int H, int W, int tiles, Plan** P) {
  if (h->plan_only) return fail(h, FILM_ERR_NO_DEVICE, "plan-only handle has no device");
  if (!h->finalized) return fail(h, FILM_ERR_STATE, "weights are not finalized");
  if (tiles < 0 || (tiles > 0 && B % tiles)) return fail(h, FILM_ERR_INVALID, "tiles must be 0 (pair plan) or divide B (sequence plan)");
  HIPCHK(h, hipSetDevice(h->device));
  return get_plan(h, B, H, W, true, P, tiles);
}

}

extern "C" {

int film_to_uint8(const float* src, unsigned char* dst, int64_t n, void* stream) {
  if (n < 0 || (n > 0 && (!src || !dst))) return FILM_ERR_INVALID;
  return film_launch_to_uint8(src, dst, n, (hipStream_t)stream) == hipSuccess ? FILM_OK : FILM_ERR_HIP;
}

int film_to_yuv420(const float* src, void* dst, int H, int W, int pix, void* stream) {
  if (!src || !dst || H < 1 || W < 1 || !pix_is_yuv(pix) || check_pix(nullptr, pix, H, W) != FILM_OK) return FILM_ERR_INVALID;
  return film_launch_rgb_to_yuv420(src, static_cast<uint8_t*>(dst), H, W, pix_layout(pix) == FILM_PIX_NV12, (pix & FILM_YUV_BT601) != 0,
                                   (pix & FILM_YUV_FULL) != 0, (hipStream_t)stream) == hipSuccess ? FILM_OK : FILM_ERR_HIP;
}

#ifndef FILM_SRC_ID
#define FILM_SRC_ID "unknown"
#endif
#ifdef FILM_EXTRA_FAMILIES
#define FILM_FLAVOUR "+extra"
#else
#define FILM_FLAVOUR ""
#endif
const char* film_version(void) { return "gfx950;film_hip r6;src=" FILM_SRC_ID FILM_FLAVOUR; }

int film_default_config(film_config* cfg) {
  if (!cfg) return FILM_ERR_INVALID;
  memset(cfg, 0, sizeof *cfg);
  cfg->pyramid_levels = 7; cfg->fusion_pyramid_levels = 5; cfg->specialized_levels = 3; cfg->sub_levels = 4;
  cfg->filters = 64;
  const int fcv[4] = {3, 3, 3, 3}, ffl[4] = {32, 64, 128, 256};
  for (int i = 0; i < 4; ++i) { cfg->flow_convs[i] = fcv[i]; cfg->flow_filters[i] = ffl[i]; }
  return FILM_OK;
}

int film_create(film_t** out, int device, const film_config* cfg) {
  if (!out) return fail(nullptr, FILM_ERR_INVALID, "out is NULL");
  *out = nullptr;
  std::unique_ptr<film_handle> h(new film_handle);
  if (cfg) h->cfg = *cfg; else film_default_config(&h->cfg);
  int rc = validate_config(h.get(), h->cfg);
  if (rc) { g_create_error = h->err; return rc; }
  h->device = device;
  h->plan_only = device < 0;
  if (!h->plan_only) {
    int ndev = 0;
    hipError_t e = hipGetDeviceCount(&ndev);
    if (e != hipSuccess || ndev <= 0)
// ... 458 lines not shown
```

### frame-interpolation_amd/csrc/film_exec.cpp

```cpp
#include "film_internal.h"

namespace film_internal {
namespace {
inline const float* cptr(const float* base, const View& v) { return base + v.off; }
inline float* mptr(float* base, const View& v) { return base + v.off; }
}

hipError_t launch_op(const OpDesc& op, float* arena, const float* wts, hipStream_t s) {
  switch (op.kind) {
    case OP_CONV: {
      ConvParams p{};
      p.nseg = op.nseg;
      for (int i = 0; i < op.nseg; ++i) {
        p.seg[i].ptr = cptr(arena, op.seg[i].v);
        p.seg[i].stride = op.seg[i].v.stride;
        p.seg[i].C = op.seg[i].v.C;
        p.seg[i].boff = op.seg[i].boff; p.seg[i].bmod = op.seg[i].bmod; p.seg[i].up = op.seg[i].up;
      }
      p.ksize = op.ksize;
      p.w = wts + op.*kConvFamily[op.family].weights;
      p.bias = wts + op.b_off;
      p.out = mptr(arena, op.out); p.ostride = op.out.stride;
      p.NB = op.NB; p.H = op.H; p.W = op.W; p.Cout = op.Cout; p.Ctot = op.Ctot; p.leaky = op.leaky;
      p.M = op.NB * op.H * op.W;
      p.fold = op.fold; p.py = op.py; p.px = op.px; p.ftaps = op.ftaps;
      p.ksplit = op.ksplit; p.part = op.ksplit > 1 ? arena + op.part_off : nullptr;
      if (op.out2.buf >= 0) { p.pool_out = mptr(arena, op.out2); p.pool_ostride = op.out2.stride; }
      if (op.pw_out.buf >= 0) {
        p.pw_w = wts + op.w2_off; p.pw_bias = wts + op.b2_off; p.pw_out = mptr(arena, op.pw_out); p.pw_ostride = op.pw_out.stride; p.pw_cout = op.pw_cout;
      }
      for (int q = 0; q < 4; ++q) { p.tdy[q] = (signed char)op.tdy[q]; p.tdx[q] = (signed char)op.tdx[q]; p.fold_woff[q] = op.fold_woff[q]; }
      return film_launch_conv(p, op.tile, s);
    }
    case OP_FLOW_HEAD: {
      FlowHeadParams p{};
      p.in = cptr(arena, op.in); p.istride = op.in.stride; p.Cin = op.Ctot;
      p.w3 = wts + op.w_off; p.b3 = wts + op.b_off; p.w4 = wts + op.w2_off; p.b4 = wts + op.b2_off;
      p.out = mptr(arena, op.out); p.M = (int)op.n;
      if (op.out2.buf >= 0) { p.add = cptr(arena, op.in2); p.sum = mptr(arena, op.out2); }
      return film_launch_flow_head(p, s);
    }
    case OP_CONV_PW: {
      ConvPwParams p{};
      p.in = cptr(arena, op.in); p.istride = op.in.stride; p.Cin = op.Ctot;
      p.w = wts + op.w_off; p.bias = wts + op.b_off;
      p.out = mptr(arena, op.out); p.ostride = op.out.stride; p.Cout = op.Cout; p.leaky = op.leaky;
      p.M = (int)op.n;
      if (op.out2.buf >= 0) { p.add = cptr(arena, op.in2); p.sum = mptr(arena, op.out2); }
      return film_launch_conv_pw(p, s);
    }
    case OP_POOL: {
      PoolParams p{};
      p.in = cptr(arena, op.in); p.istride = op.in.stride; p.out = mptr(arena, op.out); p.ostride = op.out.stride;
      p.C = op.in.C; p.NB = op.NB; p.H = op.H; p.W = op.W;
      return film_launch_pool(p, s);
    }
    case OP_FLOW_UP: {
      FlowUpParams p{};
      p.in = cptr(arena, op.in); p.out = mptr(arena, op.out); p.NB = op.NB; p.h = op.H; p.w = op.W;
      return film_launch_flow_up(p, s);
    }
    case OP_FLOW_ADD: {
      FlowAddParams p{};
      p.a = cptr(arena, op.in); p.b = cptr(arena, op.in2); p.out = mptr(arena, op.out); p.n = op.n;
      return film_launch_flow_add(p, s);
    }
    case OP_WARP: {
      WarpParams p{};
      p.src = cptr(arena, op.in); p.sstride = op.in.stride; p.C = op.in.C;
      p.flow = op.in2.buf >= 0 ? cptr(arena, op.in2) : nullptr; p.fscale = op.fscale;
      p.dst = mptr(arena, op.out); p.dstride = op.out.stride;
      p.NB = op.NB; p.H = op.H; p.W = op.W;
      p.src_brot = op.src_brot; p.flow_brot = op.flow_brot; p.misc_nb = op.misc_nb;
      if (op.in3.buf >= 0) { p.coarse = cptr(arena, op.in3); p.flow_out = mptr(arena, op.out2); }
      if (op.img_out.buf >= 0) {
        p.src3 = cptr(arena, op.img_in); p.s3stride = op.img_in.stride;
        p.src3b = p.src3 + (int64_t)(op.misc_nb > 0 ? op.misc_nb : op.NB) * op.H * op.W * op.img_in.stride;
        p.dst3 = mptr(arena, op.img_out); p.d3stride = op.img_out.stride;
        p.pack_b = cptr(arena, op.pack_b); p.pack_f = cptr(arena, op.pack_f);
      }
      return film_launch_warp(p, s);
    }
    case OP_PACK_FLOW: {
      PackFlowParams p{};
      p.bflow = cptr(arena, op.in); p.fflow = cptr(arena, op.in2);
      p.dst = mptr(arena, op.out); p.dstride = op.out.stride; p.npix = op.n;
      return film_launch_pack_flow(p, s);
    }
  }
  return hipErrorInvalidValue;
}

bool batch_splittable(const OpDesc& op, int nparts) {
  return op.kind == OP_CONV && op.nseg == 1 && op.seg[0].bmod == 0 && op.seg[0].boff == 0 && op.seg[0].up == 0 && op.ksplit <= 1 && op.fold == 0 &&
         op.NB >= nparts && op.NB % nparts == 0 && (op.out2.buf < 0 || (!(op.H & 1) && !(op.W & 1)));
}
OpDesc batch_part(const OpDesc& op, int part, int nparts) {
  OpDesc q = op;
  q.NB = op.NB / nparts;
  const int64_t px = (int64_t)part * q.NB * op.H * op.W;
  q.seg[0].v.off += px * op.seg[0].v.stride;
  q.out.off += px * op.out.stride;
  if (op.out2.buf >= 0) q.out2.off += (int64_t)part * q.NB * (op.H / 2) * (op.W / 2) * op.out2.stride;
  if (op.pw_out.buf >= 0) q.pw_out.off += px * op.pw_out.stride;
  return q;
}

hipError_t issue_lanes(film_t* h, Plan* P, hipStream_t main, bool capturing, const LanePipe* lp) {
  const size_t nops = P->ops.size();
  if (P->lane_ev.size() < nops + 2) P->lane_ev.resize(nops + 2, nullptr);
  hipError_t ev_err = hipSuccess;
  auto event_of = [&](size_t i) -> hipEvent_t {
    if (!P->lane_ev[i]) {
      hipError_t e = hipEventCreateWithFlags(&P->lane_ev[i], hipEventDisableTiming);
      if (e != hipSuccess) { ev_err = e; P->lane_ev[i] = nullptr; }
    }
    return P->lane_ev[i];
  };
  const bool two_lanes = h->opt_lanes != 0;
  hipError_t le = hipSuccess;
  if (two_lanes) {
    le = hipEventRecord(event_of(nops), main);
    if (le == hipSuccess) le = hipStreamWaitEvent(h->stream2, event_of(nops), 0);
  }
  for (size_t i = 0; i < nops && le == hipSuccess; ++i) {
    const OpDesc& op = P->ops[i];
    const int lane = (two_lanes && op.lane == 1) ? 1 : 0;
    hipStream_t ls = lane ? h->stream2 : main;
    if (two_lanes)
      for (int d : op.xdeps) {
        le = hipStreamWaitEvent(ls, event_of((size_t)d), 0);
        if (le != hipSuccess) break;
      }
    if (le != hipSuccess) break;
    if (lp && std::find(lp->head.begin(), lp->head.end(), i) != lp->head.end()) le = launch_op(batch_part(op, 1, 2), P->arena, h->packed_dev, ls);
    else if (lp && lp->tail && i + 1 == nops) {
      le = launch_op(batch_part(op, 0, 2), P->arena, h->packed_dev, ls);
      if (le == hipSuccess) le = lp->mid_tail();
      if (le == hipSuccess) le = launch_op(batch_part(op, 1, 2), P->arena, h->packed_dev, ls);
    } else le = launch_op(op, P->arena, h->packed_dev, ls);
    if (le == hipSuccess && two_lanes && op.signal) le = hipEventRecord(event_of(i), ls);
  }
  if (two_lanes && le == hipSuccess) {
    le = hipEventRecord(event_of(nops + 1), h->stream2);
    if (le == hipSuccess) le = hipStreamWaitEvent(main, event_of(nops + 1), 0);
  } else if (two_lanes && !capturing) {
    (void)hipStreamSynchronize(h->stream2);
  }
  return le == hipSuccess ? ev_err : le;
}

int run_plan(film_t* h, Plan* P, hipStream_t s, size_t n_ops) {
  const int B = P->B, H = P->H, W = P->W;
  const bool prefix = n_ops < P->ops.size();
  if (h->opt_profile) {
    const size_t n = std::min(n_ops, P->ops.size());
    while (P->ev.size() < n + 1) { hipEvent_t e; HIPCHK(h, hipEventCreate(&e)); P->ev.push_back(e); }
    HIPCHK(h, hipEventRecord(P->ev[0], s));
    for (size_t i = 0; i < n; ++i) {
      HIPCHK(h, launch_op(P->ops[i], P->arena, h->packed_dev, s));
      HIPCHK(h, hipEventRecord(P->ev[i + 1], s));
    }
    HIPCHK(h, hipStreamSynchronize(s));
    struct Acc { int launches = 0; double ms = 0, flops = 0, bytes = 0; };
    std::map<std::string, Acc> cls;
    std::ostringstream ops;
    for (size_t i = 0; i < n; ++i) {
      float ms = 0;
      HIPCHK(h, hipEventElapsedTime(&ms, P->ev[i], P->ev[i + 1]));
      Acc& a = cls[kKindName[P->ops[i].kind]];
      a.launches++; a.ms += ms; a.flops += P->ops[i].flops; a.bytes += P->ops[i].bytes;
      ops << (i ? "," : "") << "{\"tag\":\"" << P->ops[i].tag << "\",\"kind\":\"" << kKindName[P->ops[i].kind] << "\",\"ms\":" << ms
          << ",\"flops\":" << P->ops[i].flops << ",\"bytes\":" << P->ops[i].bytes << ",\"tile\":" << P->ops[i].tile << "}";
    }
    std::ostringstream o;
    o << "{\"B\":" << B << ",\"H\":" << H << ",\"W\":" << W << ",\"classes\":{";
    bool first = true;
    for (auto& kv : cls) {
      o << (first ? "" : ",") << "\"" << kv.first << "\":{\"launches\":" << kv.second.launches << ",\"ms\":" << kv.second.ms
        << ",\"flops\":" << kv.second.flops << ",\"bytes\":" << kv.second.bytes << "}";
      first = false;
    }
    o << "},\"ops\":[" << ops.str() << "]}";
    h->profile_json = o.str();
  } else if (prefix) {
    for (size_t i = 0; i < n_ops; ++i) HIPCHK(h, launch_op(P->ops[i], P->arena, h->packed_dev, s));
  } else if (h->opt_graph == 1) {
    if (!P->graph_exec) {
      HIPCHK(h, hipStreamSynchronize(s));
      HIPCHK(h, hipStreamBeginCapture(h->stream, hipStreamCaptureModeThreadLocal));
      const hipError_t le = issue_lanes(h, P, h->stream, true);
      hipError_t ce = hipStreamEndCapture(h->stream, &P->graph);
      if (le != hipSuccess) return fail(h, FILM_ERR_HIP, "kernel launch failed during capture: %s", hipGetErrorString(le));
      HIPCHK(h, ce);
      HIPCHK(h, hipGraphInstantiate(&P->graph_exec, P->graph, nullptr, nullptr, 0));
    }
    HIPCHK(h, hipGraphLaunch(P->graph_exec, s));
  } else if (h->opt_graph == 2 && h->opt_lanes != 0) {
    const hipError_t le = issue_lanes(h, P, s, false);
    if (le != hipSuccess) return fail(h, FILM_ERR_HIP, "kernel launch failed: %s", hipGetErrorString(le));
  } else {
    for (const OpDesc& op : P->ops) HIPCHK(h, launch_op(op, P->arena, h->packed_dev, s));
  }
  h->last_plan = P;
  return FILM_OK;
}

}
```

### frame-interpolation_amd/csrc/film_internal.h

```cpp
#pragma once
#include <hip/hip_runtime.h>

#include <algorithm>
#include <atomic>
#include <cmath>
#include <cstdarg>
#include <cstdint>
#include <cstdio>
#include <cstdlib>
#include <cstring>
#include <functional>
#include <map>
#include <memory>
#include <sstream>
#include <string>
#include <thread>
#include <vector>

#include "../../include/film_hip.h"
#include "film_kernels.h"

namespace film_internal {


extern thread_local std::string g_create_error;

enum OpKind { OP_CONV = 0, OP_FLOW_HEAD, OP_CONV_PW, OP_POOL, OP_FLOW_UP, OP_FLOW_ADD, OP_WARP, OP_PACK_FLOW, OP_KINDS };
extern const char* const kKindName[OP_KINDS];

struct Buffer {
  std::string name;
  int64_t off;
  int N, H, W, C;
  int64_t floats;
  int planar = 0;
  int64_t size() const { return floats; }
};

struct View {
  int buf = -1;
  int64_t off = 0;
  int stride = 0;
  int C = 0;
};

struct SegDesc {
  View v;
  int boff = 0, bmod = 0, up = 0;
};

struct OpDesc : ConvWeights {
  int kind = 0;
  std::string tag;
  SegDesc seg[FILM_MAX_SEG];
  int nseg = 0;
  int ksize = 1, leaky = 0, Cout = 0, Ctot = 0, tile = 0;
  ConvFamily family = FAM_BUF;
  int64_t b_off = 0;
  int64_t w2_off = 0, b2_off = 0;
  int ksplit = 1;
  int64_t part_off = 0;
  int fold = 0, py = 0, px = 0;
  int ftaps = 0; int tdy[4] = {0, 0, 0, 0}, tdx[4] = {0, 0, 0, 0};
  int64_t fold_woff[4] = {0, 0, 0, 0};
  int lane = 0;
  std::vector<int> xdeps;
  bool signal = false;
  View in, in2, out;
  View pack_b, pack_f;
  View img_in, img_out;
  View pw_out; int pw_cout = 0;
  View in3, out2;
  int NB = 0, H = 0, W = 0;
  float fscale = 1.f;
  int src_brot = 0, flow_brot = 0, misc_nb = 0;
  int64_t n = 0;
  double flops = 0;
  double bytes = 0;
};

struct LayerPack : ConvWeights {
  std::string name;
  int kh, kw, cin, cout;
  std::vector<int> perm;
  bool c3 = false;
  bool kmajor() const { return !c3 && cout % 32 == 0; }
  int64_t b_off = 0;
  int64_t wf_off = -1;
  bool has_halo() const { return kmajor() && kh == 3 && kw == 3; }
  bool has_fold() const { return kmajor() && kh == 2 && kw == 2; }
  bool has_fold4() const { return has_fold() && ctot() % 16 == 0 && cout % 32 == 0; }
  bool has_w2d() const { return has_halo() && ctot() % 16 == 0 && cout % 32 == 0; }
  int ctot() const { return (int)perm.size(); }
  int64_t packed_rows() const { return c3 ? 48 : (int64_t)kh * kw * ctot(); }
};

struct HostTensor {
  std::vector<int64_t> dims;
  std::vector<float> data;
};

struct Plan {
  int B = 0, H = 0, W = 0;
  int tiles = 0;
  int slot = -1;
  size_t n_extract = 0;
  std::unique_ptr<Plan> twin;
  Plan* orientation(int s) { return s == slot ? this : twin.get(); }
  uint64_t id = 0;
  std::vector<Buffer> bufs;
  std::vector<OpDesc> ops;
  int64_t arena_floats = 0;
  float* arena = nullptr;
  hipGraphExec_t graph_exec = nullptr;
  hipGraph_t graph = nullptr;
  std::vector<hipEvent_t> ev;
  std::vector<hipEvent_t> lane_ev;
  uint64_t last_use = 0;
  int find(const std::string& n) const {
    for (size_t i = 0; i < bufs.size(); ++i)
      if (bufs[i].name == n) return (int)i;
    return -1;
  }
  float* at(const char* name) const { return arena + bufs[find(name)].off; }
};

enum FuseBit {
  FUSE_FLOW_UP = 1,
  FUSE_FLOW_ADD = 2,
  FUSE_MISC16 = 4,
  FUSE_POOL = 8,
  FUSE_RGB_HEAD = 16,
};

}

struct FilmStream {
  bool open = false;
  int H = 0, W = 0, align = 0, block_h = 0, block_w = 0, pix = 0;
  void* keep = nullptr;
  float* result = nullptr;
  unsigned char* result8 = nullptr;
  bool primed = false;
  int slot = 0;
  uint64_t plan_id = 0;
  TileMapParams geo{};
};

struct film_handle {
  FilmStream fs;
  uint64_t plan_ids = 0;
  void* stage = nullptr;
  size_t stage_bytes = 0;
  void* metrics_buf = nullptr;
  size_t metrics_bytes = 0;
  int device = -1;
  bool plan_only = true;
  film_config cfg{};
  hipStream_t stream = nullptr;
  std::string err;
  std::map<std::string, film_internal::HostTensor> host_w;
  std::vector<film_internal::LayerPack> layers;
  std::map<std::string, int> layer_idx;
  int64_t packed_floats = 0;
  int64_t group_end[4] = {0, 0, 0, 0};
  int groups_packed = 0;
  std::vector<float> packed_host;
  float* packed_dev = nullptr;
  bool finalized = false;
  std::vector<std::unique_ptr<film_internal::Plan>> plans;
  film_internal::Plan* last_plan = nullptr;
  uint64_t tick = 0;
  int opt_graph = 2;
  int opt_profile = 0, opt_autotune = 1;
  int opt_max_batch = 0;
  int opt_block_overlap_h = 0, opt_block_overlap_w = 0;
  int opt_host_overlap = 1;
  hipEvent_t pipe_ev[2] = {nullptr, nullptr};
  int opt_splitk = 1;
  int opt_fuse = 31;
  int opt_planar = 1;
  int opt_fold2x2 = 1;
  int opt_wino = 1;
  int opt_halo_all = 0;
  int opt_tune_ms = 0;
  int opt_lanes = 1;
  hipStream_t stream2 = nullptr;
  int opt_precision = 0;
  int opt_wino2d = 1;
  int opt_w2d_min_px = 1536;
  int opt_w2d_small_px = 256;
  int opt_w2d_splitk = 1;
  int opt_w2d_shape = -1;
  int opt_fold4_shape = -1;
  int opt_w43_shape = -1;
  std::string profile_json;
  std::map<std::string, int> tune_cache;
  std::map<std::string, int> tune_import;
};

extern "C" int film_ensure_groups_(film_t* h, int n);

namespace film_internal {

int fail(film_t* h, int code, const char* fmt, ...);

#define HIPCHK(h, expr)                                                                     \
  do {                                                                                      \
    hipError_t e_ = (expr);                                                                 \
    if (e_ != hipSuccess)                                                                   \
      return fail(h, FILM_ERR_HIP, "%s failed: %s (%s:%d)", #expr, hipGetErrorString(e_), __FILE__, __LINE__); \
  } while (0)


std::vector<int> feature_channels(const film_config& c);
int slot_offset(const film_config& c, int j);
std::vector<int> fusion_filters(const film_config& c);
std::string predictor_prefix(const film_config& c, int level);
int predictor_index(const film_config& c, int level);
int validate_config(film_t* h, const film_config& c);
void build_layers(film_t* h);
int layout_groups(int64_t ConvWeights::* copy);

struct FamilyCodes { int c3 = 0, halo = 0, split = 0, wino = 0; };
inline FamilyCodes family_codes(ConvFamily f) {
  FamilyCodes c;
  switch (f) {
    case FAM_C3: c.c3 = 1; break;
    case FAM_HALO: c.halo = 1; break;
    case FAM_SPLIT6: c.split = 1; break;
    case FAM_SPLIT3: case FAM_FOLDX3: c.split = 2; break;
    case FAM_WINO: c.wino = 1; break;
    case FAM_WINOX3: c.wino = 2; break;
    case FAM_W43: c.wino = 3; break;
    case FAM_W2D: c.wino = 4; break;
    default: break;
  }
  return c;
}

int copy_out_string(film_t* h, const std::string& s, char* buf, int64_t cap, int64_t* needed);

hipError_t launch_op(const OpDesc& op, float* arena, const float* wts, hipStream_t s);
bool batch_splittable(const OpDesc& op, int nparts);
OpDesc batch_part(const OpDesc& op, int part, int nparts);
struct LanePipe {
  std::vector<size_t> head;
  bool tail = false;
  std::function<hipError_t()> mid_tail;
};
hipError_t issue_lanes(film_t* h, Plan* P, hipStream_t main, bool capturing, const LanePipe* lp = nullptr);
int run_plan(film_t* h, Plan* P, hipStream_t s, size_t n_ops = SIZE_MAX);

std::vector<int> conv_candidates(const OpDesc& op);
int autotune_plan(film_t* h, Plan* P);

int get_plan(film_t* h, int B, int H, int W, bool need_device, Plan** out, int tiles = 0, bool stream = false);
void drop_plans(film_t* h);
int max_units(film_t* h, int H, int W, const char* what, const char* advice, int* units);

int plan_build(film_t* h, Plan* P, int B, int H, int W, int tiles = 0, int slot = -1);
int64_t limited_buffer_bytes(const Plan* P);
std::string plan_json(film_t* h, const Plan& P);

}
```

### frame-interpolation_amd/csrc/film_kernels.h

```cpp
#pragma once
#include <hip/hip_runtime.h>
#include <stdint.h>

#include <vector>

#define FILM_MAX_SEG 4
#define FILM_BK 16

struct ConvSeg {
  const float* ptr;
  int stride;
  int C;
  int boff, bmod;
  int up;
};

struct ConvParams {
  ConvSeg seg[FILM_MAX_SEG];
  int nseg;
  int ksize;
  const float* w;
  const float* bias;
  float* out;
  int ostride;
  int NB, H, W;
  int Cout, Ctot;
  int leaky;
  int M;
  int fold, py, px, ftaps;
  signed char tdy[4], tdx[4];
  long long fold_woff[4];
  int ksplit;
  float* part;
  int unused_chain;
  unsigned mg_tpi, mg_ntx, mg_nby;
  int tl_ntx, tl_tpi;
  float* pool_out;
  int pool_ostride;
  const float* pw_w;
  const float* pw_bias;
  float* pw_out;
  int pw_ostride, pw_cout;
};

struct FlowHeadParams {
  const float* in;
  int istride;
  int Cin;
  const float* w3;
  const float* b3;
  const float* w4;
  const float* b4;
  float* out;
  int M;
  const float* add;
  float* sum;
};

struct ConvPwParams {
  const float* in;
  int istride;
  int Cin;
  const float* w;
  const float* bias;
  float* out;
  int ostride;
  int Cout;
  int leaky;
  int M;
  const float* add;
  float* sum;
};

struct PoolParams {
  const float* in;
  int istride;
  float* out;
  int ostride;
  int C;
  int NB, H, W;
};

struct FlowUpParams {
  const float* in;
  float* out;
  int NB, h, w;
};

struct FlowAddParams {
  const float* a;
  const float* b;
  float* out;
  int64_t n;
};

struct WarpParams {
  const float* src;
  int sstride;
  int C;
  const float* flow;
  float fscale;
  float* dst;
  int dstride;
  int NB, H, W;
  const float* coarse;
  float* flow_out;
  const float* src3;
  const float* src3b;
  int s3stride;
  float* dst3;
  int d3stride;
  const float* pack_b;
  const float* pack_f;
  int src_brot = 0, flow_brot = 0, misc_nb = 0;
};

struct PackFlowParams {
  const float* bflow;
  const float* fflow;
  float* dst;
  int dstride;
  int64_t npix;
};

struct TileMapParams {
  const float* src;
  float* dst;
  int B, H, W;
  int bh, bw;
  int ph, pw;
  int TH, TW;
  int oy, ox;
  int tile0, ntiles;
  int ovy, ovx;
  int eh, ew;
};
__host__ __device__ inline int film_tile_origin(int i, int p, int o, int n, int e) {
  const int s = i * p - o;
  return s < 0 ? 0 : (s > n - e ? n - e : s);
}

enum ConvTile { TILE_128x128 = 0, TILE_256x64 = 1, TILE_256x32 = 2, TILE_64x64 = 3, TILE_128x32 = 4,
                TILE_128x64 = 5, TILE_256x128 = 6 , TILE_SHAPES = 7,
                TILE_C3_DIRECT = 7 , CONV_TILE_XCD = 16,
                CONV_TILE_C3 = 32 ,
                CONV_TILE_HALO = 64 ,
                CONV_TILE_WINO = 256 ,
                CONV_TILE_SPLIT = 128 ,
                CONV_TILE_X3 = 512 ,
                CONV_TILE_F43 = 2048 ,
                CONV_TILE_W2D = 8192 ,
                CONV_TILE_EXT = 4096 ,
                CONV_TILE_FOLD4 = 16384 ,
                CONV_TILE_FOLDX3 = 1024  };
enum Wino43Tile { W43_4x64_T21 = 0, W43_4x64_T12 = 1, W43_4x32_T11 = 2, W43_Q16_4x64_T21 = 3, W43_Q16_4x64_T12 = 4, W43_Q16_4x32_T11 = 5,
                  W43_Q16_4x64_N1 = 6 ,
                  W43_Q16_4x64_T21_P2 = 7, W43_Q16_4x64_T12_P2 = 8, W43_Q16_4x32_T11_P2 = 9, W43_Q16_4x64_N1_P2 = 10,
                  W43_Q16_4x32_T11_BG = 11,
                  W43_Q8_8x64_T21_P2 = 12, W43_Q8_8x64_N1_P2 = 13, W43_Q8_8x32_T11_BG = 14, W43_Q8_8x64_T12_P2 = 15,
                  W43_Q8_8x32_T11_P2 = 16 };
#ifdef FILM_EXTRA_FAMILIES
constexpr bool kExtraFamilies = true;
#else
constexpr bool kExtraFamilies = false;
#endif
static inline bool film_w43_shape_built(int sh) {
  if (kExtraFamilies) return sh >= 0 && sh <= W43_Q8_8x32_T11_P2;
  return sh == W43_Q16_4x64_T21_P2 || sh == W43_Q16_4x32_T11_P2 || sh == W43_Q16_4x64_N1_P2 || sh == W43_Q8_8x64_T21_P2 || sh == W43_Q8_8x64_N1_P2 ||
         sh == W43_Q8_8x32_T11_BG || sh == W43_Q8_8x32_T11_P2;
}
enum Wino2dTile { W2D_8x64 = 0, W2D_8x32 = 1, W2D_8x32_S2 = 2, W2D_16x64 = 3, W2D_16x32 = 4, W2D_16x32_S2 = 5, W2D_SHAPES = 6 };
inline bool film_w2d_square(int shape) { return shape >= W2D_16x64 && shape <= W2D_16x32_S2; }
inline bool film_w2d_64(int shape) { return shape == W2D_8x64 || shape == W2D_16x64; }
enum Fold4Tile { F4_4x64 = 0, F4_4x32 = 1 };
enum FoldX3Tile { FX3_4x64 = 0 , FX3_8x64 = 1 , FX3_4x128 = 2  };
enum WinoX3Tile { WX3_4x128_T22 = 0, WX3_4x64_T12 = 1, WX3_4x64_T21 = 3, WX3_4x32_T11 = 4 };
enum WinoTile { WINO_4x128 = 0 , WINO_4x64 = 1 , WINO_4x128_W16 = 2 ,
                WINO_4x64_W8 = 3 , WINO_4x32 = 4 , WINO_8x64_W16 = 5 ,
                WINO_8x32_W8 = 6 , WINO_2x64 = 7 , WINO_SHAPES = 8 };
enum HaloTile { HALO_8x128 = 0 , HALO_8x64 = 1 , HALO_8x32 = 2 , HALO_4x64 = 3 ,
                HALO_4x128 = 4 , HALO_4x32 = 5 , HALO_SHAPES = 6 };

struct TileShape { int bm, bn; };
static inline TileShape film_tile_shape(int tile) {
  switch (tile & (CONV_TILE_XCD - 1)) {
    case TILE_128x128: return {128, 128};
    case TILE_256x64: return {256, 64};
    case TILE_256x32: return {256, 32};
    case TILE_64x64: return {64, 64};
    case TILE_128x64: return {128, 64};
    case TILE_256x128: return {256, 128};
    default: return {128, 32};
  }
}

enum ConvFamily { FAM_BUF , FAM_C3, FAM_W2D, FAM_W43, FAM_FOLD4 ,
                  FAM_HALO, FAM_SPLIT6, FAM_SPLIT3, FAM_WINO, FAM_WINOX3, FAM_FOLDX3 ,
                  CONV_FAMILIES };
constexpr int CONV_TILE_FAMILY = CONV_TILE_C3 | CONV_TILE_HALO | CONV_TILE_SPLIT | CONV_TILE_WINO | CONV_TILE_X3 | CONV_TILE_FOLDX3 |
                                 CONV_TILE_F43 | CONV_TILE_W2D | CONV_TILE_FOLD4;

struct ConvWeights {
  int64_t w_off = 0;
  int64_t wh_off = -1;
  int64_t ws_off = -1;
  int64_t ww_off = -1;
  int64_t wx_off = -1;
  int64_t w43_off = -1;
  int64_t w2d_off = -1;
  int64_t wfx_off = -1;
  int64_t wf4_off = -1;
};

namespace film_internal {
struct OpDesc;
std::vector<int> tile_candidates(const OpDesc&), c3_candidates(const OpDesc&), wino2d_candidates(const OpDesc&), wino43_candidates(const OpDesc&),
    fold4_candidates(const OpDesc&), halo_candidates(const OpDesc&), wino_candidates(const OpDesc&), winox3_candidates(const OpDesc&),
    foldx3_candidates(const OpDesc&);
}
struct ConvFamilyRow {
  int flags;
  int64_t ConvWeights::* weights;
  bool splitk;
  bool in_default;
  int fused_shape;
  std::vector<int> (*candidates)(const film_internal::OpDesc&);
  int (*default_shape)(int Cout, int64_t M);
};

constexpr int conv_buf_shape(int Cout, int64_t M) {
  auto blocks = [&](int bm, int bn) { return ((M + bm - 1) / bm) * (Cout / bn); };
  if (Cout % 128 == 0) return blocks(128, 128) >= 768 ? TILE_128x128 : TILE_64x64;
  if (Cout % 64 == 0) return blocks(256, 64) >= 768 ? TILE_256x64 : TILE_64x64;
  return blocks(256, 32) >= 768 ? TILE_256x32 : TILE_128x32;
}
constexpr int film_split_shape(int Cout, int64_t) { return Cout % 128 == 0 ? HALO_8x128 : Cout % 64 == 0 ? HALO_4x64 : HALO_8x32; }

inline constexpr ConvFamilyRow kConvFamily[CONV_FAMILIES] = {
   {0, &ConvWeights::w_off, true, true, -1, film_internal::tile_candidates, conv_buf_shape},
   {CONV_TILE_C3, &ConvWeights::w_off, false, true, -1, film_internal::c3_candidates, [](int, int64_t) -> int { return TILE_C3_DIRECT; }},
   {CONV_TILE_W2D, &ConvWeights::w2d_off, true, true, W2D_8x64, film_internal::wino2d_candidates, [](int c, int64_t) -> int { return c % 64 == 0 ? W2D_8x64 : W2D_8x32; }},
   {CONV_TILE_WINO | CONV_TILE_F43, &ConvWeights::w43_off, true, true, W43_Q16_4x64_N1_P2, film_internal::wino43_candidates, [](int c, int64_t) -> int { return c % 64 == 0 ? W43_Q16_4x64_T21_P2 : W43_Q16_4x32_T11_P2; }},
   {CONV_TILE_FOLD4, &ConvWeights::wf4_off, true, true, -1, film_internal::fold4_candidates, [](int c, int64_t) -> int { return c % 64 == 0 ? F4_4x64 : F4_4x32; }},
   {CONV_TILE_HALO, &ConvWeights::wh_off, false, false, -1, film_internal::halo_candidates, [](int c, int64_t) -> int { return c % 64 == 0 ? HALO_4x64 : HALO_8x32; }},
   {CONV_TILE_SPLIT, &ConvWeights::ws_off, false, false, -1, film_internal::halo_candidates, film_split_shape},
   {CONV_TILE_SPLIT | CONV_TILE_X3, &ConvWeights::ws_off, false, false, -1, film_internal::halo_candidates, film_split_shape},
   {CONV_TILE_WINO, &ConvWeights::ww_off, false, false, -1, film_internal::wino_candidates, [](int c, int64_t) -> int { return c % 64 == 0 ? WINO_4x64_W8 : WINO_4x32; }},
   {CONV_TILE_WINO | CONV_TILE_X3, &ConvWeights::wx_off, false, false, -1, film_internal::winox3_candidates, [](int c, int64_t) -> int { return c % 128 == 0 ? WX3_4x128_T22 : c % 64 == 0 ? WX3_4x64_T12 : WX3_4x32_T11; }},
   {CONV_TILE_FOLDX3, &ConvWeights::wfx_off, false, false, -1, film_internal::foldx3_candidates, [](int, int64_t) -> int { return FX3_4x64; }},
};

constexpr bool conv_family_built(int f) { return kConvFamily[f].in_default || kExtraFamilies; }
constexpr int conv_family_of(int tile) {
  for (int f = 0; f < CONV_FAMILIES; ++f) if ((tile & CONV_TILE_FAMILY) == kConvFamily[f].flags) return f;
  return -1;
}
constexpr int conv_tile(int f, int shape, bool xcd) { return kConvFamily[f].flags | (shape & 15) | (shape >= 16 ? CONV_TILE_EXT : 0) | (xcd ? CONV_TILE_XCD : 0); }
constexpr int conv_tile_shape(int tile) { return (tile & 15) + ((tile & CONV_TILE_EXT) ? 16 : 0); }
constexpr int conv_default_tile(int f, int Cout, int64_t M) { return conv_tile(f, kConvFamily[f].default_shape(Cout, M), true); }

hipError_t film_launch_conv(const ConvParams& p, int tile, hipStream_t s);
hipError_t film_launch_conv_pw(const ConvPwParams& p, hipStream_t s);
hipError_t film_launch_flow_head(const FlowHeadParams& p, hipStream_t s);
hipError_t film_launch_pool(const PoolParams& p, hipStream_t s);
hipError_t film_launch_flow_up(const FlowUpParams& p, hipStream_t s);
hipError_t film_launch_flow_add(const FlowAddParams& p, hipStream_t s);
hipError_t film_launch_warp(const WarpParams& p, hipStream_t s);
hipError_t film_launch_pack_flow(const PackFlowParams& p, hipStream_t s);
hipError_t film_launch_frame_to_tiles(const TileMapParams& p, hipStream_t s);
hipError_t film_launch_tiles_to_frame(const TileMapParams& p, hipStream_t s);
hipError_t film_launch_frame_to_tiles_overlap(const TileMapParams& p, hipStream_t s);
hipError_t film_launch_frame_to_tiles_u8(const TileMapParams& p, const uint8_t* src, hipStream_t s);
hipError_t film_launch_frame_to_tiles_overlap_u8(const TileMapParams& p, const uint8_t* src, hipStream_t s);
hipError_t film_launch_yuv420_to_tiles(TileMapParams p, const uint8_t* src, bool nv12, bool bt601, bool full, hipStream_t s);
hipError_t film_launch_rgb_to_yuv420(const float* src, uint8_t* dst, int H, int W, bool nv12, bool bt601, bool full, hipStream_t s);
hipError_t film_launch_blend_tiles(const TileMapParams& p, hipStream_t s);
hipError_t film_launch_to_uint8(const float* src, uint8_t* dst, int64_t n, hipStream_t s);
hipError_t film_launch_fill_random(float* dst, int64_t n, uint32_t seed, hipStream_t s);

#define FILM_SSIM_TAPS 11
struct MetricsParams {
  const float* pred;
  const float* ref;
  int B, H, W, C;
  int flags;
  double g[FILM_SSIM_TAPS];
  double c1, c2;
  int sum_blocks, ssim_tiles_x, ssim_tiles_y;
  int64_t part_per_image;
  double* part;
  double* out;
};
void film_metrics_layout(MetricsParams& p);
hipError_t film_launch_image_metrics(const MetricsParams& p, hipStream_t s);
```

### frame-interpolation_amd/csrc/film_planner.cpp

```cpp
#include "film_internal.h"

namespace film_internal {

const char* const kKindName[OP_KINDS] = {"conv_mfma", "flow_head", "conv_pw", "pool", "flow_up", "flow_add", "warp", "pack_flow"};

namespace {
struct ConvSite {
  const LayerPack* L;
  int H, W;
  int ctot;
  bool folded;
  bool any_up;
  bool out_16b;
  bool segs_16b;
  bool segs_c16;
  bool halo_row_24bit;
  bool fold4_rows_32bit;
  int64_t px() const { return (int64_t)H * W; }
};

ConvSite conv_site(const LayerPack& L, const std::vector<SegDesc>& segs, const View& out, int H, int W, bool folded) {
  ConvSite s{&L, H, W, 0, folded, false, out.off % 4 == 0 && out.stride % 4 == 0, true, true, true,
             (int64_t)16 * W * std::max(out.stride, L.cout) < (1ll << 31)};
  for (const SegDesc& g : segs) {
// ... 146 lines not shown
    op.kind = OP_CONV;
    op.tag = tag + ":" + name + (folded ? ":phases" : "");
    op.nseg = (int)segs.size();
    for (int i = 0; i < op.nseg && i < FILM_MAX_SEG; ++i) op.seg[i] = segs[i];
    op.ksize = L.kh; op.leaky = leaky; op.Cout = L.cout; op.Ctot = s.ctot;
    op.out = out; op.NB = NB; op.H = s.H; op.W = s.W;
    static_cast<ConvWeights&>(op) = L;
    op.b_off = L.b_off;
    if (s.ctot != L.ctot() || out.C != L.cout || op.nseg > FILM_MAX_SEG || !L.kmajor()) refuse("planner: channel mismatch at " + tag + ":" + name);
    if (!folded && (!s.out_16b || L.cout % 32 != 0))
      refuse("planner: " + op.tag + " writes " + std::to_string(L.cout) + " channels at float offset " + std::to_string(out.off) + " of a " +
                std::to_string(out.stride) + "-float pixel: the convolution kernels need Cout % 32 == 0 and 16-byte aligned output slices");
    set_family(op, folded ? folded_conv_family(s, *h) : plain_conv_family(s, *h), (int64_t)NB * s.H * s.W * (folded ? 2 : 1));
    if (folded) {
      op.seg[0].up = 0;
      op.fold = op.family == FAM_FOLD4 ? 3 : 2;
      op.w_off = op.fold == 3 ? L.wf4_off : L.wf_off;
      int64_t rel = 0;
      for (int q = 0; q < 4 && op.fold == 2; ++q) { op.fold_woff[q] = rel; rel += (int64_t)((q >> 1) + 1) * ((q & 1) + 1) * s.ctot * L.cout; }
    }
    const int S = conv_ksplit(op.family, s, *h);
    if (S > 1) split_k(op, S);
    const double out_px = (double)NB * H * W;
    op.flops = 2.0 * out_px * L.cout * L.kh * L.kw * L.cin;
    op.bytes = 4.0 * out_px * ((folded ? L.cin / 4.0 : L.cin) + L.cout);
    P->ops.push_back(op);
  }
  void conv_c3(const std::string& tag, const std::string& name, View in, View out, int NB, int H, int W) {
    const LayerPack& L = layer(name);
    OpDesc op;
    op.kind = OP_CONV; op.family = FAM_C3; op.tag = tag + ":" + name;
    op.nseg = 1; op.seg[0].v = in;
    op.ksize = 3; op.leaky = 1; op.Cout = out.C; op.Ctot = 3;
    op.w_off = L.w_off; op.b_off = L.b_off;
    op.out = out; op.NB = NB; op.H = H; op.W = W;
    op.tile = conv_default_tile(FAM_C3, out.C, 0);
    op.flops = 2.0 * NB * H * W * out.C * 27; op.bytes = 4.0 * NB * H * W * (3 + out.C);
    P->ops.push_back(op);
  }
  void conv_pw(const std::string& tag, const std::string& name, View in, View out, int64_t M, bool leaky) {
    const LayerPack& L = layer(name);
    OpDesc op;
    op.kind = OP_CONV_PW; op.tag = tag + ":" + name;
    op.in = in; op.out = out; op.n = M; op.leaky = leaky; op.Cout = L.cout; op.Ctot = L.cin;
    op.w_off = L.w_off; op.b_off = L.b_off;
    op.flops = 2.0 * M * L.cout * L.cin; op.bytes = 4.0 * M * (L.cin + L.cout);
    P->ops.push_back(op);
  }
  void pool(const std::string& tag, View in, View out, int NB, int H, int W) {
    OpDesc op;
    op.kind = OP_POOL; op.tag = tag; op.in = in; op.out = out; op.NB = NB; op.H = H; op.W = W;
    op.bytes = 4.0 * NB * H * W * in.C * 1.25;
    P->ops.push_back(op);
  }
  void warp(const std::string& tag, View src, View flow, View dst, int NB, int H, int W, float fscale,
            bool count_flow = true) {
    OpDesc op;
    op.kind = OP_WARP; op.tag = tag; op.in = src; op.in2 = flow; op.out = dst;
    op.NB = NB; op.H = H; op.W = W; op.fscale = fscale;
    op.bytes = 4.0 * NB * H * W * (2.0 * src.C + (count_flow ? 2 : 0));
    P->ops.push_back(op);
  }

  void add_buffers() {
    const film_config& c = h->cfg;
    for (int l = 0; l < NL; ++l) img.push_back(add_buffer("img" + std::to_string(l), NI, HL(l), WL(l), 3));
    for (int l = 0; l < NL; ++l) feat.push_back(add_buffer("feat" + std::to_string(l), NI, HL(l), WL(l), fc[l]));
    for (int i = 0; i < NL; ++i) {
      const bool pooled = std::min(NL - i, c.sub_levels) > 1;
      fx_a.push_back(add_scratch("scratch_fx_a" + std::to_string(i), (int64_t)NI * HL(i) * WL(i) * c.filters));
      fx_p.push_back(add_scratch("scratch_fx_p" + std::to_string(i), pooled ? (int64_t)NI * HL(i + 1) * WL(i + 1) * c.filters : 0));
    }
    int64_t fp_sz = 0;
    for (int l = 0; l < NL; ++l) fp_sz = std::max<int64_t>(fp_sz, (int64_t)N2 * HL(l) * WL(l) * c.flow_filters[predictor_index(c, l)]);
    for (int k = 0; k < 3; ++k) fp[k] = add_scratch("scratch_fp_" + std::to_string(k), fp_sz);
    for (int l = 0; l < NL; ++l) res.push_back(add_buffer("res" + std::to_string(l), N2, HL(l), WL(l), 2));
    for (int l = 0; l < NL - 1; ++l) {
      vup.push_back(add_buffer("vup" + std::to_string(l), N2, HL(l), WL(l), 2));
      v.push_back(add_buffer("v" + std::to_string(l), N2, HL(l), WL(l), 2));
      warped.push_back(add_buffer("warped" + std::to_string(l), N2, HL(l), WL(l), fc[l]));
    }
    v.push_back(res[NL - 1]);
    for (int l = 0; l < FL; ++l) {
      aligned.push_back(add_buffer("aligned" + std::to_string(l), B, HL(l), WL(l), 2 * fc[l] + 16));
      if (h->opt_planar && l < FL - 1 && fc[l] % 16 == 0) P->bufs[aligned[l]].planar = fc[l];
    }
    for (int i = 0; i < FL - 1; ++i) {
      fu_u.push_back(add_buffer("fusion_up" + std::to_string(i), B, HL(i), WL(i), ff[i]));
      fu_a.push_back(add_buffer("fusion_a" + std::to_string(i), B, HL(i), WL(i), ff[i]));
      fu_b.push_back(add_buffer("fusion_b" + std::to_string(i), B, HL(i), WL(i), ff[i]));
    }
    out_buf = add_buffer("out", B, H0, W0, 3);
  }

  void emit_image_pyramids() {
    for (int l = 0; l + 1 < NL; ++l) {
      pool("image_pyramid_l" + std::to_string(l + 1), view(img[l], e0, 0, 3), view(img[l + 1], e0, 0, 3), NE, HL(l), WL(l));
      P->ops.back().lane = 1;
    }
  }

  void emit_extractor(int i) {
    const film_config& c = h->cfg;
    const int n = std::min(NL - i, c.sub_levels);
    const size_t first_op = P->ops.size();
    const int64_t a_img = (int64_t)HL(i) * WL(i) * c.filters, p_img = (int64_t)HL(i + 1) * WL(i + 1) * c.filters;
    for (int j = 0; j < n; ++j) {
      const int lv = i + j, k = c.filters << j;
      const std::string tg = "feat_s" + std::to_string(i) + "_" + std::to_string(j);
      const std::string w0 = "feat_net/sub_extractor/cfeat_conv_" + std::to_string(2 * j);
      const std::string w1 = "feat_net/sub_extractor/cfeat_conv_" + std::to_string(2 * j + 1);
      View tmp = fx_scratch(fx_a[i], k, a_img);
      if (j == 0) conv_c3(tg, w0, view(img[i], e0, 0, 3), tmp, NE, HL(lv), WL(lv));
      else conv(tg, w0, {seg(fx_scratch(fx_p[i], k >> 1, p_img))}, tmp, NE, HL(lv), WL(lv), true);
      View dst = view(feat[lv], e0, slot_offset(c, j), k);
      conv(tg, w1, {seg(tmp)}, dst, NE, HL(lv), WL(lv), true);
      if (j == n - 1) continue;
      OpDesc& cv = P->ops.back();
      if ((h->opt_fuse & FUSE_POOL) && cv.kind == OP_CONV && kConvFamily[cv.family].fused_shape >= 0 && cv.ksplit <= 1 && !(HL(lv) & 1) && !(WL(lv) & 1)) {
        cv.tag += "+pool";
        cv.out2 = fx_scratch(fx_p[i], k, p_img);
      } else
        pool(tg + ":pool", dst, fx_scratch(fx_p[i], k, p_img), NE, HL(lv), WL(lv));
    }
    const int side_from = (int64_t)H0 * W0 <= 512 * 512 ? 3 : 1;
    if (i >= side_from) to_lane(first_op, 1);
  }

  void emit_flow(int l) {
    const film_config& c = h->cfg;
    const size_t first_op = P->ops.size();
    const std::string tg = "flow_l" + std::to_string(l);
    const int pi = predictor_index(c, l);
    const int nf = c.flow_filters[pi], nconv = c.flow_convs[pi];
    const std::string prefix = predictor_prefix(c, l);
    const int Hl = HL(l), Wl = WL(l);
    const bool coarsest = l == NL - 1;
    if (!coarsest) {
      const bool fuse_up = (h->opt_fuse & FUSE_FLOW_UP) && (int64_t)Hl * Wl < 100000;
      if (!fuse_up) {
        OpDesc up;
        up.kind = OP_FLOW_UP; up.tag = tg + ":resize2x";
        up.in = view(v[l + 1], 0, 0, 2); up.out = view(vup[l], 0, 0, 2);
        up.NB = N2; up.H = HL(l + 1); up.W = WL(l + 1);
        up.bytes = 4.0 * N2 * Hl * Wl * 2 * 1.25;
        P->ops.push_back(up);
      }
      for (int d = 0; d < (seq ? 2 : 1); ++d) {
        if (seq)
          warp(tg + ":warp_d" + std::to_string(d), view(feat[l], d ? i0 : i1, 0, fc[l]), view(vup[l], d * B, 0, 2),
               view(warped[l], d * B, 0, fc[l]), B, Hl, Wl, 1.f);
        else {
          warp(tg + ":warp_d01", view(feat[l], 0, 0, fc[l]), view(vup[l], 0, 0, 2), view(warped[l], 0, 0, fc[l]), N2, Hl, Wl, 1.f);
          P->ops.back().src_brot = B;
        }
        if (fuse_up) {
          OpDesc& w = P->ops.back();
          w.tag += "+resize2x";
          w.in2 = View();
          w.in3 = view(v[l + 1], d * B, 0, 2);
          w.out2 = view(vup[l], d * B, 0, 2);
        }
      }
    }
    View cur = scratch(fp[0], nf);
    if (!seq) {
      SegDesc sa = seg(view(feat[l], 0, 0, fc[l])), sb = seg(view(coarsest ? feat[l] : warped[l], 0, 0, fc[l]));
      if (coarsest) { sb.boff = B; sb.bmod = N2; }
      conv(tg, prefix + "/conv_0", {sa, sb}, cur, N2, Hl, Wl, true);
    } else {
      for (int d = 0; d < 2; ++d) {
        SegDesc a = seg(view(feat[l], d ? i1 : i0, 0, fc[l]));
        SegDesc b = seg(coarsest ? view(feat[l], d ? i0 : i1, 0, fc[l]) : view(warped[l], d * B, 0, fc[l]));
        View o = cur;
        o.off += (int64_t)d * B * Hl * Wl * nf;
        conv(tg + ":d" + std::to_string(d), prefix + "/conv_0", {a, b}, o, B, Hl, Wl, true);
      }
    }
    int which = 0;
    for (int j = 1; j < nconv; ++j) {
      View nxt = scratch(fp[which ^ 1], nf);
      conv(tg, prefix + "/conv_" + std::to_string(j), {seg(cur)}, nxt, N2, Hl, Wl, true);
      cur = nxt; which ^= 1;
    }
    const int64_t M = (int64_t)N2 * Hl * Wl;
    const std::string l3 = prefix + "/conv_" + std::to_string(nconv), l4 = prefix + "/conv_" + std::to_string(nconv + 1);
    if ((nf / 2) % 32 == 0) {
      View hid = scratch(fp[2], nf / 2);
      conv(tg, l3, {seg(cur)}, hid, N2, Hl, Wl, true);
      conv_pw(tg, l4, hid, view(res[l], 0, 0, 2), M, false);
    } else {
      const LayerPack &L3 = layer(l3), &L4 = layer(l4);
      OpDesc op;
      op.kind = OP_FLOW_HEAD; op.tag = tg + ":" + l3 + "+conv_" + std::to_string(nconv + 1);
      op.in = cur; op.out = view(res[l], 0, 0, 2); op.n = M; op.Ctot = nf;
      op.w_off = L3.w_off; op.b_off = L3.b_off; op.w2_off = L4.w_off; op.b2_off = L4.b_off;
      op.flops = 2.0 * op.n * (nf * 16 + 16 * 2); op.bytes = 4.0 * op.n * (nf + 2);
      P->ops.push_back(op);
    }
    if (!coarsest && (h->opt_fuse & FUSE_FLOW_ADD)) {
      OpDesc& head = P->ops.back();
      head.tag += "+v=res+up";
      head.in2 = view(vup[l], 0, 0, 2); head.out2 = view(v[l], 0, 0, 2);
    } else if (!coarsest) {
      OpDesc ad;
      ad.kind = OP_FLOW_ADD; ad.tag = tg + ":v=res+up";
      ad.in = view(res[l], 0, 0, 2); ad.in2 = view(vup[l], 0, 0, 2); ad.out = view(v[l], 0, 0, 2);
      ad.n = M * 2; ad.bytes = 4.0 * ad.n * 3;
      P->ops.push_back(ad);
    }
    if (l >= 4) to_lane(first_op, 1);
  }

  void emit_align(int l) {
    const size_t first_op = P->ops.size();
    const std::string tg = "align_l" + std::to_string(l);
    const bool pair = P->bufs[aligned[l]].planar > 0 && !seq;
    const bool misc16 = (h->opt_fuse & FUSE_MISC16) && !seq;
    if (pair) {
      warp(tg + ":warp_feat01", view(feat[l], 0, 0, fc[l]), view(v[l], 0, 0, 2), aligned_part(aligned[l], 0, fc[l]), N2, HL(l), WL(l), 0.5f);
      P->ops.back().flow_brot = B;
    }
    for (int s = 0; s < 2; ++s) {
      View fl = view(v[l], (1 - s) * B, 0, 2);
      if (!pair)
        warp(tg + ":warp_feat" + std::to_string(s), view(feat[l], s ? i1 : i0, 0, fc[l]), fl,
             aligned_part(aligned[l], s, fc[l]), B, HL(l), WL(l), 0.5f);
      if (!misc16)
        warp(tg + ":warp_img" + std::to_string(s), view(img[l], s ? i1 : i0, 0, 3), fl,
             sub(aligned_part(aligned[l], 2, fc[l]), 3 * s, 3), B, HL(l), WL(l), 0.5f, false);
    }
    if (misc16) {
      OpDesc& w = P->ops.back();
      w.tag += "+misc16";
      if (pair) w.misc_nb = B;
      w.img_in = view(img[l], 0, 0, 3);
      w.img_out = aligned_part(aligned[l], 2, fc[l]);
      w.pack_b = view(v[l], B, 0, 2);
      w.pack_f = view(v[l], 0, 0, 2);
      w.bytes += 4.0 * B * HL(l) * WL(l) * 12.0;
    } else {
      OpDesc pk;
      pk.kind = OP_PACK_FLOW; pk.tag = tg + ":flows";
      pk.in = view(v[l], B, 0, 2);
      pk.in2 = view(v[l], 0, 0, 2);
      pk.out = sub(aligned_part(aligned[l], 2, fc[l]), 6, 10);
      pk.n = (int64_t)B * HL(l) * WL(l); pk.bytes = 4.0 * pk.n * 14;
      P->ops.push_back(pk);
    }
    to_lane(first_op, 1);
  }

  void emit_fusion(int i, int lane) {
    const size_t first_op = P->ops.size();
    const std::string tg = "fusion_l" + std::to_string(i);
    const std::string base = "fusion/convs_" + std::to_string(i);
    conv(tg, base + "_0", {seg(net, 1)}, view(fu_u[i], 0, 0, ff[i]), B, HL(i), WL(i), false);
    const SegDesc up = seg(view(fu_u[i], 0, 0, ff[i]));
    if (P->bufs[aligned[i]].planar)
      conv(tg, base + "_1", {seg(aligned_part(aligned[i], 0, fc[i])), seg(aligned_part(aligned[i], 1, fc[i])), seg(aligned_part(aligned[i], 2, fc[i])), up},
           view(fu_a[i], 0, 0, ff[i]), B, HL(i), WL(i), true);
    else
      conv(tg, base + "_1", {seg(view(aligned[i], 0, 0, 2 * fc[i] + 16)), up}, view(fu_a[i], 0, 0, ff[i]), B, HL(i), WL(i), true);
    conv(tg, base + "_2", {seg(view(fu_a[i], 0, 0, ff[i]))}, view(fu_b[i], 0, 0, ff[i]), B, HL(i), WL(i), true);
    net = view(fu_b[i], 0, 0, ff[i]);
    to_lane(first_op, lane);
  }

  void emit_rgb_head() {
    OpDesc& last = P->ops.back();
    const LayerPack& LO = layer("fusion/output_conv");
    if ((h->opt_fuse & FUSE_RGB_HEAD) && last.kind == OP_CONV && kConvFamily[last.family].fused_shape >= 0 && last.Cout == 64 && last.ksplit <= 1 &&
        last.out2.buf < 0 && LO.cout <= 4 && LO.cin == 64) {
      last.tag += "+output_conv";
      last.pw_out = view(out_buf, 0, 0, 3); last.pw_cout = LO.cout;
      last.w2_off = LO.w_off; last.b2_off = LO.b_off;
      last.tile = conv_tile(last.family, kConvFamily[last.family].fused_shape, true);
      last.flops += 2.0 * (double)B * H0 * W0 * LO.cout * LO.cin;
      last.bytes = 4.0 * (double)B * H0 * W0 * (64 + LO.cout);
    } else {
      conv_pw("fusion_out", "fusion/output_conv", net, view(out_buf, 0, 0, 3), (int64_t)B * H0 * W0, false);
    }
  }

  int build(int B_, int H_, int W_, int T_, int slot) {
    const film_config& c = h->cfg;
    B = B_; H0 = H_; W0 = W_; T = T_;
    NL = c.pyramid_levels; FL = c.fusion_pyramid_levels;
    seq = T > 0;
    N2 = 2 * B;
    NI = seq ? B + T : N2;
    i0 = 0; i1 = seq ? T : B;
    NE = NI; e0 = 0;
    if (slot >= 0) {
      if (slot > 1 || B != T) return fail(h, FILM_ERR_INVALID, "a stream plan has slot 0 or 1 and one pair of its tiles");
      i0 = (1 - slot) * T; i1 = slot * T;
      NE = T; e0 = i1;
    }
    fc = feature_channels(c);
    ff = fusion_filters(c);
    P->B = B; P->H = H0; P->W = W0; P->tiles = T; P->slot = slot;
    add_buffers();
    emit_image_pyramids();
    for (int i = 0; i < NL; ++i) emit_extractor(i);
    P->n_extract = P->ops.size();
    for (int l = NL - 1; l >= 0; --l) emit_flow(l);
    const bool early_fusion = h->opt_lanes >= 2 && ((int64_t)H0 * W0 > 512 * 512 || h->opt_lanes >= 3) && FL >= 4;
    net = view(aligned[FL - 1], 0, 0, 2 * fc[FL - 1] + 16);
    emit_align(FL - 1);
    if (early_fusion) {
      for (int i = FL - 2; i >= 0; --i) {
        emit_align(i);
        if (i >= 2) emit_fusion(i, 1);
      }
      for (int i = std::min(FL - 2, 1); i >= 0; --i) emit_fusion(i, 0);
    } else {
      for (int i = FL - 2; i >= 0; --i) emit_align(i);
      for (int i = FL - 2; i >= 0; --i) emit_fusion(i, 0);
    }
    emit_rgb_head();
    if (bad) return fail(h, FILM_ERR_INVALID, "%s", bad_msg.c_str());
    P->arena_floats = cursor;
    analyze_lanes();
    return FILM_OK;
  }

  struct Access { int buf; int c0, c1; };
  Access access(const View& v) const {
    const Buffer& b = P->bufs[v.buf];
    if (b.C == 0 || v.stride != b.C) return {v.buf, 0, 1 << 30};
    const int c0 = (int)((v.off - b.off) % b.C);
    return {v.buf, c0, c0 + v.C};
  }
  static bool overlap(const Access& a, const Access& b) { return a.buf == b.buf && a.c0 < b.c1 && b.c0 < a.c1; }
  void accesses(const OpDesc& op, std::vector<Access>& rd, std::vector<Access>& wr) const {
    rd.clear(); wr.clear();
    if (op.kind == OP_CONV) { for (int i = 0; i < op.nseg; ++i) rd.push_back(access(op.seg[i].v)); }
    else { if (op.in.buf >= 0) rd.push_back(access(op.in)); if (op.in2.buf >= 0) rd.push_back(access(op.in2)); }
    if (op.in3.buf >= 0) rd.push_back(access(op.in3));
    if (op.img_in.buf >= 0) rd.push_back(access(op.img_in));
    if (op.pack_b.buf >= 0) { rd.push_back(access(op.pack_b)); rd.push_back(access(op.pack_f)); }
    if (op.out.buf >= 0 && op.pw_out.buf < 0) wr.push_back(access(op.out));
    if (op.pw_out.buf >= 0) wr.push_back(access(op.pw_out));
    if (op.out2.buf >= 0) wr.push_back(access(op.out2));
    if (op.img_out.buf >= 0) wr.push_back(access(op.img_out));
  }
  void analyze_lanes() {
    const size_t n = P->ops.size();
    std::vector<std::vector<Access>> rd(n), wr(n);
    for (size_t i = 0; i < n; ++i) accesses(P->ops[i], rd[i], wr[i]);
    long waited[2] = {-1, -1};
    for (size_t j = 0; j < n; ++j) {
      OpDesc& oj = P->ops[j];
      const int lj = oj.lane ? 1 : 0;
      for (size_t ii = j; ii-- > 0;) {
        const OpDesc& oi = P->ops[ii];
        if ((oi.lane ? 1 : 0) == lj) continue;
        if ((long)ii <= waited[lj]) break;
        bool hit = false;
        for (const Access& w : wr[ii]) {
          for (const Access& r : rd[j]) hit |= overlap(w, r);
          for (const Access& w2 : wr[j]) hit |= overlap(w, w2);
        }
        for (const Access& r : rd[ii])
          for (const Access& w2 : wr[j]) hit |= overlap(r, w2);
        if (hit) { oj.xdeps.push_back((int)ii); P->ops[ii].signal = true; waited[lj] = (long)ii; break; }
      }
    }
  }
};

}

int plan_build(film_t* h, Plan* P, int B, int H, int W, int tiles, int slot) {
  Planner pl{h, P};
  return pl.build(B, H, W, tiles, slot);
}

int64_t limited_buffer_bytes(const Plan* P) {
  int64_t mx = 1;
  for (const OpDesc& op : P->ops) {
    if (op.kind != OP_CONV || op.family == FAM_W43 || op.family == FAM_W2D) continue;
    for (int i = 0; i < op.nseg; ++i) mx = std::max(mx, P->bufs[op.seg[i].v.buf].floats * (int64_t)sizeof(float));
  }
  return mx;
}

namespace {
struct JsonObject {
  std::ostringstream& o;
  const char* sep = "{";
  std::ostringstream& key(const char* k) { o << sep << "\"" << k << "\":"; sep = ","; return o; }
  template <class T> void num(const char* k, const T& v) { key(k) << v; }
  void str(const char* k, const std::string& v) { key(k) << "\"" << v << "\""; }
  template <class T, class F> void list(const char* k, const T* a, size_t n, F each) {
    key(k) << "[";
    for (size_t i = 0; i < n; ++i) { o << (i ? "," : ""); each(a[i]); }
    o << "]";
  }
  template <class T> void ints(const char* k, const T* a, size_t n) { list(k, a, n, [&](const T& v) { o << v; }); }
  template <class T, class F> void objects(const char* k, const T* a, size_t n, F fill) {
    list(k, a, n, [&](const T& v) { JsonObject e{o}; fill(e, v); o << "}"; });
  }
  void view(const char* k, const View& v, const Plan& P) {
    JsonObject j{key(k)};
    j.str("buf", v.buf >= 0 ? P.bufs[v.buf].name : std::string(""));
    j.num("off", v.off); j.num("stride", v.stride); j.num("C", v.C);
    o << "}";
  }
};

void json_op(JsonObject& j, const OpDesc& op, const Plan& P) {
  const FamilyCodes fc = family_codes(op.family);
  j.str("kind", kKindName[op.kind]); j.str("tag", op.tag); j.num("NB", op.NB); j.num("H", op.H); j.num("W", op.W);
  j.num("ksize", op.ksize); j.num("leaky", op.leaky); j.num("Cout", op.Cout); j.num("Ctot", op.Ctot); j.num("tile", op.tile);
  j.num("w_off", op.w_off); j.num("b_off", op.b_off); j.num("wf4_off", op.wf4_off);
  j.num("wh_off", op.wh_off); j.num("halo", fc.halo); j.num("ws_off", op.ws_off); j.num("split", fc.split);
  j.num("ww_off", op.ww_off); j.num("wx_off", op.wx_off); j.num("wfx_off", op.wfx_off); j.num("w43_off", op.w43_off); j.num("w2d_off", op.w2d_off);
  j.num("wino", fc.wino); j.num("fold", op.fold); j.num("ksplit", op.ksplit);
  j.num("py", op.py); j.num("px", op.px); j.num("ftaps", op.ftaps); j.ints("tdy", op.tdy, 4); j.ints("tdx", op.tdx, 4);
  j.ints("fold_woff", op.fold_woff, 4); j.num("lane", op.lane); j.ints("xdeps", op.xdeps.data(), op.xdeps.size());
  j.num("w2_off", op.w2_off); j.num("b2_off", op.b2_off); j.num("c3", fc.c3);
  j.num("fscale", op.fscale); j.num("src_brot", op.src_brot); j.num("flow_brot", op.flow_brot); j.num("misc_nb", op.misc_nb); j.num("n", op.n);
  j.num("flops", op.flops); j.num("bytes", op.bytes);
  j.view("in", op.in, P); j.view("in2", op.in2, P); j.view("in3", op.in3, P); j.view("out2", op.out2, P); j.view("pw_out", op.pw_out, P); j.num("pw_cout", op.pw_cout);
  j.view("img_in", op.img_in, P); j.view("img_out", op.img_out, P); j.view("pack_b", op.pack_b, P); j.view("pack_f", op.pack_f, P); j.view("out", op.out, P);
  j.objects("segs", op.seg, op.nseg, [&](JsonObject& s, const SegDesc& g) {
    s.view("v", g.v, P); s.num("boff", g.boff); s.num("bmod", g.bmod); s.num("up", g.up);
  });
}
}

std::string plan_json(film_t* h, const Plan& P) {
  std::ostringstream o;
  JsonObject j{o};
  j.num("B", P.B); j.num("H", P.H); j.num("W", P.W);
  if (P.slot >= 0) { j.str("kind", "stream"); j.num("tiles", P.tiles); j.num("slot", P.slot); j.num("n_extract", P.n_extract); }
  else if (P.tiles > 0) { j.str("kind", "sequence"); j.num("n_pairs", P.B / P.tiles); j.num("tiles", P.tiles); }
  j.num("arena_floats", P.arena_floats); j.num("offset32_buffer_bytes", limited_buffer_bytes(&P)); j.num("packed_floats", h->packed_floats);
  j.objects("buffers", P.bufs.data(), P.bufs.size(), [](JsonObject& e, const Buffer& b) {
    e.str("name", b.name); e.num("off", b.off); e.num("N", b.N); e.num("H", b.H); e.num("W", b.W); e.num("C", b.C); e.num("floats", b.floats); e.num("planar", b.planar);
  });
  j.objects("layers", h->layers.data(), h->layers.size(), [](JsonObject& e, const LayerPack& L) {
    e.str("name", L.name); e.num("kh", L.kh); e.num("kw", L.kw); e.num("cin", L.cin); e.num("cout", L.cout); e.num("ctot", L.ctot());
    e.num("w_off", L.w_off); e.num("b_off", L.b_off); e.num("wh_off", L.wh_off); e.num("ws_off", L.ws_off); e.num("ww_off", L.ww_off); e.num("wx_off", L.wx_off);
  });
  j.objects("ops", P.ops.data(), P.ops.size(), [&](JsonObject& e, const OpDesc& op) { json_op(e, op, P); });
  o << "}";
  return o.str();
}

}
```

### frame-interpolation_amd/csrc/film_plans.cpp

```cpp
#include "film_internal.h"

namespace film_internal {
namespace {
void free_plan(Plan* p) {
  if (p->twin) { p->twin->arena = nullptr; free_plan(p->twin.get()); }
  if (p->graph_exec) (void)hipGraphExecDestroy(p->graph_exec);
  if (p->graph) (void)hipGraphDestroy(p->graph);
  for (auto e : p->ev) (void)hipEventDestroy(e);
  for (auto e : p->lane_ev) if (e) (void)hipEventDestroy(e);
  if (p->arena) (void)hipFree(p->arena);
}

void forget_plan(film_t* h, size_t index) {
  if (h->last_plan == h->plans[index].get() || (h->last_plan && h->last_plan == h->plans[index]->twin.get())) h->last_plan = nullptr;
  free_plan(h->plans[index].get());
  h->plans.erase(h->plans.begin() + index);
}

constexpr int64_t kMaxBufferBytes = 0xFFF00000ll;
constexpr int64_t kMaxArenaBytes = 64ll << 30;
int64_t arena_budget_bytes(film_t* h) {
  int64_t cap = kMaxArenaBytes;
  if (!h->plan_only) {
    size_t fr = 0, tot = 0;
    if (hipSetDevice(h->device) == hipSuccess && hipMemGetInfo(&fr, &tot) == hipSuccess) {
      int64_t held = 0;
      for (auto& p : h->plans) if (p->arena) held += p->arena_floats * (int64_t)sizeof(float);
      cap = std::min<int64_t>(cap, ((int64_t)fr + held) / 10 * 6);
    } else {
      (void)hipGetLastError();
    }
  }
  return std::max<int64_t>(cap, 1);
}
}

void drop_plans(film_t* h) {
  if (!h->plan_only) { (void)hipSetDevice(h->device); (void)hipDeviceSynchronize(); }
  while (!h->plans.empty()) forget_plan(h, h->plans.size() - 1);
}

int get_plan(film_t* h, int B, int H, int W, bool need_device, Plan** out, int tiles, bool stream) {
  const auto same = [&](const Plan& p) { return p.B == B && p.H == H && p.W == W && p.tiles == tiles && (p.slot >= 0) == stream; };
  const int div = 1 << (h->cfg.pyramid_levels - 1);
  if (B < 1 || H < 1 || W < 1) return fail(h, FILM_ERR_INVALID, "B, H, W must be positive");
  if (H % div || W % div)
    return fail(h, FILM_ERR_INVALID, "input height and width (%d x %d) must be divisible by %d = 2^(pyramid_levels-1); "
                "pad first (Interpolator align)", H, W, div);
  const int wl = std::max(h->cfg.pyramid_levels - 2, h->cfg.fusion_pyramid_levels - 1);
  if ((H >> wl) < 2 || (W >> wl) < 2)
    return fail(h, FILM_ERR_INVALID, "input %d x %d too small: warped pyramid level %d would be smaller than 2x2", H, W, wl);
  if ((int64_t)2 * B * H * W >= (int64_t)1 << 31) return fail(h, FILM_ERR_INVALID, "batch too large (2*B*H*W must fit int32)");
  for (auto& p : h->plans)
    if (same(*p) && (!need_device || p->arena)) { *out = p.get(); p->last_use = ++h->tick; return FILM_OK; }
  if (need_device)
    for (size_t i = 0; i < h->plans.size(); ++i)
      if (same(*h->plans[i])) { forget_plan(h, i); break; }
  std::unique_ptr<Plan> P(new Plan);
  int rc = plan_build(h, P.get(), B, H, W, tiles, stream ? 0 : -1);
  if (rc) return rc;
  P->id = ++h->plan_ids;
  if (stream) {
    P->twin.reset(new Plan);
    Plan& Q = *P->twin;
    if ((rc = plan_build(h, &Q, B, H, W, tiles, 1))) return rc;
    bool alike = Q.arena_floats == P->arena_floats && Q.bufs.size() == P->bufs.size() && Q.n_extract == P->n_extract;
    for (size_t i = 0; alike && i < Q.bufs.size(); ++i) alike = Q.bufs[i].name == P->bufs[i].name && Q.bufs[i].off == P->bufs[i].off && Q.bufs[i].floats == P->bufs[i].floats;
    if (!alike) return fail(h, FILM_ERR_INVALID, "planner: the two orientations of a stream plan lay out different workspaces");
    Q.id = P->id;
  }
  if (need_device) {
    size_t alive = 0;
    for (auto& p : h->plans) alive += p->arena != nullptr;
    while (alive >= 3) {
      size_t victim = h->plans.size();
      for (size_t i = 0; i < h->plans.size(); ++i)
        if (h->plans[i]->arena && (victim == h->plans.size() || h->plans[i]->last_use < h->plans[victim]->last_use)) victim = i;
      if (victim == h->plans.size()) break;
      (void)hipSetDevice(h->device);
      (void)hipDeviceSynchronize();
      forget_plan(h, victim);
      --alive;
    }
    hipError_t e = hipMalloc(&P->arena, (size_t)P->arena_floats * sizeof(float));
    if (e != hipSuccess && alive > 0) {
      (void)hipGetLastError();
      (void)hipDeviceSynchronize();
      for (size_t i = h->plans.size(); i-- > 0;)
        if (h->plans[i]->arena) forget_plan(h, i);
      e = hipMalloc(&P->arena, (size_t)P->arena_floats * sizeof(float));
    }
    if (e != hipSuccess) {
      P->arena = nullptr;
      return fail(h, FILM_ERR_NOMEM, "workspace hipMalloc of %.1f MB failed: %s", P->arena_floats * 4e-6, hipGetErrorString(e));
    }
    HIPCHK(h, hipMemsetAsync(P->arena, 0, (size_t)P->arena_floats * sizeof(float), h->stream));
    HIPCHK(h, hipStreamSynchronize(h->stream));
    if (P->twin) P->twin->arena = P->arena;
    if (h->opt_autotune && h->finalized) {
      int trc = autotune_plan(h, P.get());
      if (trc == FILM_OK && P->twin) trc = autotune_plan(h, P->twin.get());
      if (trc) { free_plan(P.get()); return trc; }
    }
  }
  const std::pair<ConvFamily, int> forced[] = {{FAM_W43, h->opt_w43_shape}, {FAM_W2D, h->opt_w2d_shape}, {FAM_FOLD4, h->opt_fold4_shape}};
  for (const auto& [fam, shape] : forced) {
    if (shape < 0) continue;
    for (Plan* R : {P.get(), P->twin.get()}) {
      if (!R) continue;
      for (OpDesc& op : R->ops) {
        if (op.kind != OP_CONV || op.family != fam) continue;
        const std::vector<int> cands = conv_candidates(op);
        const int want = conv_tile(fam, shape, true);
        if (std::find(cands.begin(), cands.end(), want) != cands.end()) op.tile = want;
      }
    }
  }
  P->last_use = ++h->tick;
  *out = P.get();
  h->plans.push_back(std::move(P));
  return FILM_OK;
}

int max_units(film_t* h, int H, int W, const char* what, const char* advice, int* units) {
  Plan* P1 = nullptr;
  int rc = get_plan(h, 1, H, W, false, &P1);
  if (rc) return rc;
  const int64_t lim = limited_buffer_bytes(P1);
  const int64_t arena = std::max<int64_t>(1, P1->arena_floats * (int64_t)sizeof(float));
  *units = (int)std::max<int64_t>(1, std::min<int64_t>(kMaxBufferBytes / lim, arena_budget_bytes(h) / arena));
  if (lim > kMaxBufferBytes)
    return fail(h, FILM_ERR_INVALID, "a %d x %d %s needs a %.1f GB activation buffer in front of a kernel that addresses 4 GiB per "
                "buffer - %s", H, W, what, lim * 1e-9, advice);
  if (h->opt_max_batch) *units = std::min(*units, h->opt_max_batch);
  return FILM_OK;
}

}
```

### frame-interpolation_amd/csrc/film_tune.cpp

```cpp
#include "film_internal.h"

namespace film_internal {
namespace {
std::vector<int> both_maps(ConvFamily f, const std::vector<int>& shapes) {
  std::vector<int> out;
  for (int sh : shapes) { out.push_back(conv_tile(f, sh, false)); out.push_back(conv_tile(f, sh, true)); }
  return out;
}

std::string conv_signature(const OpDesc& op) {
  std::ostringstream o;
  const FamilyCodes fc = family_codes(op.family);
  o << op.NB << 'x' << op.H << 'x' << op.W << ':' << op.Cout << ':' << op.ksize << ':' << op.out.stride << ':' << fc.c3 << ':' << fc.halo << ':' << fc.split << ':' << fc.wino << ':' << op.fold << ':' << op.ksplit << ':' << (op.out2.buf >= 0) << ':' << op.pw_cout;
  for (int i = 0; i < op.nseg; ++i)
    o << '|' << op.seg[i].v.C << ',' << op.seg[i].v.stride << ',' << op.seg[i].up << ',' << op.seg[i].bmod;
  return o.str();
}
}

std::vector<int> tile_candidates(const OpDesc& op) {
  if (op.Cout % 128 == 0) return both_maps(FAM_BUF, {TILE_128x128, TILE_256x128, TILE_256x64, TILE_128x64, TILE_64x64});
  if (op.Cout % 64 == 0) return both_maps(FAM_BUF, {TILE_256x64, TILE_128x64, TILE_64x64, TILE_256x32, TILE_128x32});
  return both_maps(FAM_BUF, {TILE_256x32, TILE_128x32});
}

std::vector<int> c3_candidates(const OpDesc&) { return {conv_tile(FAM_C3, TILE_C3_DIRECT, false)}; }

std::vector<int> halo_candidates(const OpDesc& op) {
  if (op.Cout % 128 == 0) return both_maps(op.family, {HALO_4x64, HALO_4x128, HALO_8x64, HALO_8x128});
  if (op.Cout % 64 == 0) return both_maps(op.family, {HALO_4x64, HALO_8x64, HALO_4x32, HALO_8x32});
  return both_maps(op.family, {HALO_8x32, HALO_4x32});
}

std::vector<int> wino_candidates(const OpDesc& op) {
  if (op.Cout % 128 == 0) return both_maps(FAM_WINO, {WINO_4x64_W8, WINO_8x64_W16, WINO_2x64, WINO_4x128_W16, WINO_4x128});
  if (op.Cout % 64 == 0) return both_maps(FAM_WINO, {WINO_4x64_W8, WINO_8x64_W16, WINO_2x64, WINO_4x32});
  return both_maps(FAM_WINO, {WINO_4x32, WINO_8x32_W8});
}

std::vector<int> wino43_candidates(const OpDesc& op) {
  const bool pool = op.out2.buf >= 0, pw = op.pw_out.buf >= 0;
  std::vector<int> shapes;
  if (pw)
    shapes = {W43_Q16_4x64_N1, W43_Q16_4x64_N1_P2, W43_Q8_8x64_N1_P2};
  else if (op.Cout % 64 == 0)
    shapes = {W43_4x64_T21, W43_Q16_4x64_T21, W43_Q16_4x64_T12, W43_Q16_4x32_T11, W43_Q16_4x64_N1,
              W43_Q16_4x64_T21_P2, W43_Q16_4x64_T12_P2, W43_Q16_4x32_T11_P2, W43_Q16_4x64_N1_P2, W43_Q16_4x32_T11_BG,
              W43_Q8_8x64_T21_P2, W43_Q8_8x64_T12_P2, W43_Q8_8x64_N1_P2, W43_Q8_8x32_T11_BG, W43_Q8_8x32_T11_P2};
  else
    shapes = {W43_4x32_T11, W43_Q16_4x32_T11, W43_Q16_4x32_T11_P2, W43_Q16_4x32_T11_BG, W43_Q8_8x32_T11_BG, W43_Q8_8x32_T11_P2};
  std::vector<int> keep;
  for (int sh : shapes) {
    if (!film_w43_shape_built(sh)) continue;
    if (pool && (sh == W43_4x64_T21 || sh == W43_4x64_T12 || sh == W43_4x32_T11)) continue;
    keep.push_back(sh);
  }
  return both_maps(FAM_W43, keep);
}

std::vector<int> wino2d_candidates(const OpDesc& op) {
  const int H = op.H, W = op.W;
  const bool pw = op.pw_out.buf >= 0;
  const int64_t pad_r = (int64_t)((W + 31) / 32) * ((H + 7) / 8), pad_s = (int64_t)((W + 15) / 16) * ((H + 15) / 16);
  const bool sq = pad_s <= pad_r;
  std::vector<int> shapes;
  if (pw || op.Cout % 64 == 0) { shapes.push_back(W2D_8x64); if (sq) shapes.push_back(W2D_16x64); }
  if (!pw) {
    shapes.push_back(W2D_8x32); shapes.push_back(W2D_8x32_S2);
    if (sq) { shapes.push_back(W2D_16x32); shapes.push_back(W2D_16x32_S2); }
  }
  return both_maps(FAM_W2D, shapes);
}

std::vector<int> fold4_candidates(const OpDesc& op) {
  return both_maps(FAM_FOLD4, op.Cout % 64 == 0 ? std::vector<int>{F4_4x64, F4_4x32} : std::vector<int>{F4_4x32});
}

std::vector<int> foldx3_candidates(const OpDesc& op) {
  return both_maps(FAM_FOLDX3, op.Cout % 128 == 0 ? std::vector<int>{FX3_4x64, FX3_8x64, FX3_4x128} : std::vector<int>{FX3_4x64, FX3_8x64});
}

std::vector<int> winox3_candidates(const OpDesc& op) {
  if (op.Cout % 128 == 0) return both_maps(FAM_WINOX3, {WX3_4x128_T22, WX3_4x64_T12, WX3_4x64_T21});
  if (op.Cout % 64 == 0) return both_maps(FAM_WINOX3, {WX3_4x64_T12, WX3_4x64_T21, WX3_4x32_T11});
  return both_maps(FAM_WINOX3, {WX3_4x32_T11});
}

std::vector<int> conv_candidates(const OpDesc& op) { return kConvFamily[op.family].candidates(op); }

int autotune_plan(film_t* h, Plan* P) {
  bool need = false;
  for (const OpDesc& op : P->ops) {
    if (op.kind != OP_CONV) continue;
    const std::string sig = conv_signature(op);
    if (h->tune_cache.count(sig)) continue;
    auto it = h->tune_import.find(sig);
    if (it != h->tune_import.end()) {
      const std::vector<int> cands = conv_candidates(op);
      if (std::find(cands.begin(), cands.end(), it->second) != cands.end()) { h->tune_cache[sig] = it->second; continue; }
    }
    need = true;
  }
  if (need) {
    HIPCHK(h, film_launch_fill_random(P->arena, P->arena_floats, 0x9e3779b9u, h->stream));
    hipEvent_t e0, e1;
    HIPCHK(h, hipEventCreate(&e0));
    HIPCHK(h, hipEventCreate(&e1));
    for (OpDesc& op : P->ops) {
      if (op.kind != OP_CONV) continue;
      const std::string sig = conv_signature(op);
      if (h->tune_cache.count(sig)) continue;
      int best = op.tile;
      float best_ms = 1e30f;
      const std::vector<int> cands = conv_candidates(op);
      auto launch_tile = [&](int tile) -> hipError_t {
        OpDesc trial = op;
        trial.tile = tile;
        return launch_op(trial, P->arena, h->packed_dev, h->stream);
      };
      auto time_once = [&](int tile, float* ms) -> int {
        HIPCHK(h, hipEventRecord(e0, h->stream));
        HIPCHK(h, launch_tile(tile));
        HIPCHK(h, hipEventRecord(e1, h->stream));
        HIPCHK(h, hipEventSynchronize(e1));
        HIPCHK(h, hipEventElapsedTime(ms, e0, e1));
        return FILM_OK;
      };
      std::vector<std::pair<float, int>> timed;
      for (int tile : cands) {
        HIPCHK(h, launch_tile(tile));
        float ms_min = 1e30f, ms_sum = 0.f;
        for (int rep = 0; rep < 2 || (ms_sum < (float)h->opt_tune_ms && rep < 64); ++rep) {
          float ms = 0;
          int trc = time_once(tile, &ms);
          if (trc) return trc;
          ms_min = std::min(ms_min, ms);
          ms_sum += ms;
        }
        timed.push_back({ms_min, tile});
      }
      std::sort(timed.begin(), timed.end());
      size_t nfin = 0;
      while (nfin < timed.size() && nfin < 4 && timed[nfin].first <= timed[0].first * 1.06f) ++nfin;
      if (nfin > 1)
        for (int round = 0; round < 4; ++round)
          for (size_t c = 0; c < nfin; ++c) {
            float ms = 0;
            int trc = time_once(timed[c].second, &ms);
            if (trc) return trc;
            timed[c].first = std::min(timed[c].first, ms);
          }
      for (size_t c = 0; c < std::max<size_t>(nfin, 1) && c < timed.size(); ++c)
        if (timed[c].first < best_ms) { best_ms = timed[c].first; best = timed[c].second; }
      if (op.family == FAM_W2D && !film_w2d_64(best & 15)) {
        float ms64 = 1e30f;
        int t64 = -1;
        for (size_t c = 0; c < std::max<size_t>(nfin, 1) && c < timed.size(); ++c)
          if (film_w2d_64(timed[c].second & 15) && timed[c].first < ms64) { ms64 = timed[c].first; t64 = timed[c].second; }
        if (t64 >= 0 && ms64 <= best_ms * 1.02f) best = t64;
      }
      h->tune_cache[sig] = best;
    }
    (void)hipEventDestroy(e0);
    (void)hipEventDestroy(e1);
    HIPCHK(h, hipMemsetAsync(P->arena, 0, (size_t)P->arena_floats * sizeof(float), h->stream));
    HIPCHK(h, hipStreamSynchronize(h->stream));
  }
  for (OpDesc& op : P->ops)
    if (op.kind == OP_CONV) op.tile = h->tune_cache.at(conv_signature(op));
  return FILM_OK;
}

}

using namespace film_internal;

extern "C" {

int film_export_tune(film_t* h, char* buf, int64_t cap, int64_t* needed) {
  if (!h) return FILM_ERR_INVALID;
  std::ostringstream o;
  o << "# film_hip tune cache v1 " << film_version() << "\n";
  std::map<std::string, int> all = h->tune_import;
  for (const auto& kv : h->tune_cache) all[kv.first] = kv.second;
  for (const auto& kv : all) o << kv.first << '\t' << kv.second << '\n';
  return copy_out_string(h, o.str(), buf, cap, needed);
}

int film_import_tune(film_t* h, const char* text) {
  if (!h || !text) return fail(h, FILM_ERR_INVALID, "NULL argument");
  std::istringstream in(text);
  std::string line;
  if (!std::getline(in, line)) return FILM_OK;
  const std::string want = std::string("# film_hip tune cache v1 ") + film_version();
  if (line != want) return FILM_OK;
  std::map<std::string, int> got;
  while (std::getline(in, line)) {
    if (line.empty() || line[0] == '#') continue;
    const size_t tab = line.rfind('\t');
    if (tab == std::string::npos || tab == 0 || tab + 1 >= line.size()) return fail(h, FILM_ERR_INVALID, "tune cache: malformed line '%s'", line.c_str());
    char* end = nullptr;
    const long tile = strtol(line.c_str() + tab + 1, &end, 10);
    if (*end != 0 || tile < 0 || tile > (1 << 20)) return fail(h, FILM_ERR_INVALID, "tune cache: malformed line '%s'", line.c_str());
    got[line.substr(0, tab)] = (int)tile;
  }
  for (const auto& kv : got) h->tune_import[kv.first] = kv.second;
  return FILM_OK;
}

}
```

Before: 30.12 frames/s.

## Group independent convolutions into single grouped kernel launches with autotuned choice

Adds grouped-launch variants of the buffer and Winograd-2D conv kernels, where one grid concatenates the workgroups of up to four independent conv ops and each block finds its op through a start-offset table. A scheduler pass groups ready convs into schedule items with cross-lane waits. The autotuner times each group against running the ops separately and picks whichever is faster. The aim is to cut launch overhead and tail underutilization on small convs, at the cost of heavier kernel arguments, extra index math per block and a more complex schedule.

```diff
diff --git a/__graft_entry__.py b/__graft_entry__.py
--- a/__graft_entry__.py
+++ b/__graft_entry__.py
@@ -17,12 +17,27 @@
             print('built', film_build.build(verbose=True))
         finally:
             os.environ['FILM_EXTRA_FAMILIES'] = '0'
+    build_group_check()
     from film_hip import engine
     lib = engine.load_library()
     for sym in engine.EXPORTED_SYMBOLS:
         getattr(lib, sym)
     import eval.interpolator
     print('built', out, engine.FilmEngine.version())
+
+
+def build_group_check() -> str:
+    import subprocess
+    src = os.path.join(ROOT, 'tools', 'w2d_bench.hip')
+    exe = os.path.join(ROOT, 'tools', 'bin', 'w2d_group_check')
+    csrc = os.path.join(PKG, 'csrc')
+    deps = [src] + [os.path.join(csrc, f) for f in ('conv_wino2d_impl.h', 'conv_common.h', 'film_kernels.h')]
+    if not os.path.isfile(exe) or any(os.path.getmtime(d) > os.path.getmtime(exe) for d in deps):
+        os.makedirs(os.path.dirname(exe), exist_ok=True)
+        cmd = [os.environ.get('HIPCC', 'hipcc'), '--offload-arch=gfx950', '-O3', '-std=c++17', '-ffp-contract=off', '-DW2D_BENCH_GROUP_ONLY', src, '-o', exe]
+        print(' '.join(cmd), flush=True)
+        subprocess.run(cmd, check=True)
+    return exe
 
 
 def smoke() -> None:
diff --git a/frame-interpolation_amd/csrc/conv_buf_impl.h b/frame-interpolation_amd/csrc/conv_buf_impl.h
--- a/frame-interpolation_amd/csrc/conv_buf_impl.h
+++ b/frame-interpolation_amd/csrc/conv_buf_impl.h
@@ -1,8 +1,32 @@
 #pragma once
 #include "conv_common.h"
 
-template <int BM, int BN, int WGM, int WGN, int FLAGS>
-__global__ __launch_bounds__(WGM* WGN * 64) void conv_buf_kernel(ConvParams p) {
+template <int BM, int BN, int WGM, int WGN, int FLAGS, bool GRP = false>
+__global__ __launch_bounds__(WGM* WGN * 64) void conv_buf_kernel(std::conditional_t<GRP, ConvGroupParams, ConvParams> p_arg) {
+  int grp_bx = 0, grp_by = 0, grp_bz = 0;
+  const ConvParams* grp_p = nullptr;
+  if constexpr (GRP) {
+    const int lin = (int)blockIdx.x;
+    const int mi = (lin >= p_arg.start[1] ? 1 : 0) + (lin >= p_arg.start[2] ? 1 : 0) + (lin >= p_arg.start[3] ? 1 : 0);
+    const int nbx = p_arg.gx[mi], nby = p_arg.gy[mi], nxy = nbx * nby;
+    int l = lin - p_arg.start[mi];
+    grp_bz = l / nxy;
+    l -= grp_bz * nxy;
+    if constexpr ((FLAGS & CONV_B_XCD_M) != 0) {
+      const int xcd = l & 7, idx = l >> 3;
+      const int q = nxy >> 3, r = nxy & 7;
+      const int nl = (xcd < r ? xcd * (q + 1) : r * (q + 1) + (xcd - r) * q) + idx;
+      grp_bx = nl / nby;
+      grp_by = nl - grp_bx * nby;
+    } else {
+      grp_by = l / nbx;
+      grp_bx = l - grp_by * nbx;
+    }
+    grp_p = &p_arg.m[mi];
+  } else {
+    grp_p = &p_arg;
+  }
+  const ConvParams& p = *grp_p;
   constexpr int NW = WGM * WGN, NT = NW * 64;
   constexpr int WTM = BM / WGM, WTN = BN / WGN;
   constexpr int TM = WTM / 32, TN = WTN / 32;
@@ -22,7 +46,9 @@
   const int wm = wv / WGN, wn = wv % WGN;
 
   int bx = blockIdx.x, by = blockIdx.y;
-  if constexpr ((FLAGS & CONV_B_XCD_M) != 0) conv_xcd_remap(bx, by);
+  if constexpr (GRP) { bx = grp_bx; by = grp_by; }
+  else if constexpr ((FLAGS & CONV_B_XCD_M) != 0) conv_xcd_remap(bx, by);
+  const unsigned bz = GRP ? (unsigned)grp_bz : blockIdx.z;
   const int m0 = bx * BM;
   const int n0 = by * BN;
 
@@ -31,13 +57,13 @@
   const int pcol = ((t & 3) ^ ((t >> 4) & 3)) * 4;
   const int ksz = p.ksize;
   const int pad = (ksz - 1) >> 1;
-  const int fpy = p.fold == 2 ? (int)(blockIdx.z >> 1) : p.py, fpx = p.fold == 2 ? (int)(blockIdx.z & 1) : p.px;
+  const int fpy = p.fold == 2 ? (int)(bz >> 1) : p.py, fpx = p.fold == 2 ? (int)(bz & 1) : p.px;
   const int ntaps = p.fold == 2 ? (fpy + 1) * (fpx + 1) : p.fold ? p.ftaps : ksz * ksz;
   auto tap_dy = [&](int tp) { return p.fold == 2 ? (fpx ? tp >> 1 : tp) : p.fold ? (int)p.tdy[tp] : tp / ksz - pad; };
   auto tap_dx = [&](int tp) { return p.fold == 2 ? (fpx ? tp & 1 : 0) : p.fold ? (int)p.tdx[tp] : tp % ksz - pad; };
-  const float* const wbase = p.fold == 2 ? p.w + p.fold_woff[blockIdx.z] : p.w;
+  const float* const wbase = p.fold == 2 ? p.w + p.fold_woff[bz] : p.w;
   const int ksplit = p.fold ? 1 : (p.ksplit > 1 ? p.ksplit : 1);
-  const int split = ksplit > 1 ? (int)blockIdx.z : 0;
+  const int split = ksplit > 1 ? (int)bz : 0;
   const int HW = p.H * p.W;
   int ab[AR], ay[AR], ax[AR];
   unsigned amask[AR];
@@ -243,10 +269,39 @@
 }
 
 template <int BM, int BN, int WGM, int WGN, int FLAGS>
+hipError_t conv_buf_prepare(const ConvParams& p, dim3& grid) {
+  if (p.ksplit > 1 && p.fold) return hipErrorInvalidValue;
+  if (p.ksplit > 1 ? (p.Cout % 4 || (reinterpret_cast<uintptr_t>(p.part) & 15)) : (p.ostride % 4 || (reinterpret_cast<uintptr_t>(p.out) & 15))) return hipErrorInvalidValue;
+  grid = dim3((p.M + BM - 1) / BM, p.Cout / BN, p.fold == 2 ? 4 : (p.ksplit > 1 ? p.ksplit : 1));
+  return hipSuccess;
+}
+
+template <int BM, int BN, int WGM, int WGN, int FLAGS>
 hipError_t conv_buf_launch(const ConvParams& p, hipStream_t s) {
   constexpr size_t lds = 2 * (size_t)(BM + BN) * 16 * sizeof(float);
-  if (p.ksplit > 1 && p.fold) return hipErrorInvalidValue;
-  if (p.ksplit > 1 ? (p.Cout % 4 || (reinterpret_cast<uintptr_t>(p.part) & 15)) : (p.ostride % 4 || (reinterpret_cast<uintptr_t>(p.out) & 15))) return hipErrorInvalidValue;
-  dim3 grid((p.M + BM - 1) / BM, p.Cout / BN, p.fold == 2 ? 4 : (p.ksplit > 1 ? p.ksplit : 1));
+  dim3 grid;
+  if (const hipError_t e = conv_buf_prepare<BM, BN, WGM, WGN, FLAGS>(p, grid); e != hipSuccess) return e;
   return conv_launch<conv_buf_kernel<BM, BN, WGM, WGN, FLAGS>>(grid, dim3(WGM * WGN * 64), lds, s, p);
 }
+
+template <int BM, int BN, int WGM, int WGN, int FLAGS>
+hipError_t conv_buf_launch_group(const ConvParams* p, int n, hipStream_t s, int* starts) {
+  constexpr size_t lds = 2 * (size_t)(BM + BN) * 16 * sizeof(float);
+  if (n < 1 || n > FILM_MAX_GROUP) return hipErrorInvalidValue;
+  ConvGroupParams g{};
+  long long total = 0;
+  for (int i = 0; i < FILM_MAX_GROUP; ++i) { g.start[i] = 0x7fffffff; g.gx[i] = g.gy[i] = g.gz[i] = 1; }
+  for (int i = 0; i < n; ++i) {
+    dim3 grid;
+    if (p[i].fold) return hipErrorInvalidValue;
+    if (const hipError_t e = conv_buf_prepare<BM, BN, WGM, WGN, FLAGS>(p[i], grid); e != hipSuccess) return e;
+    g.m[i] = p[i];
+    g.start[i] = (int)total; g.gx[i] = (int)grid.x; g.gy[i] = (int)grid.y; g.gz[i] = (int)grid.z;
+    if (starts) starts[i] = (int)total;
+    total += (long long)grid.x * grid.y * grid.z;
+    if (total >= (1ll << 31)) return hipErrorInvalidValue;
+  }
+  g.n = n;
+  if (starts) starts[n] = (int)total;
+  return conv_launch<conv_buf_kernel<BM, BN, WGM, WGN, FLAGS, true>>(dim3((unsigned)total), dim3(WGM * WGN * 64), lds, s, g);
+}
diff --git a/frame-interpolation_amd/csrc/conv_common.h b/frame-interpolation_amd/csrc/conv_common.h
--- a/frame-interpolation_amd/csrc/conv_common.h
+++ b/frame-interpolation_amd/csrc/conv_common.h
@@ -34,8 +34,8 @@
   return e;
 }
 
-template <auto KERN>
-hipError_t conv_launch(dim3 grid, dim3 block, size_t lds, hipStream_t s, const ConvParams& p, size_t lds_allow) {
+template <auto KERN, class P>
+hipError_t conv_launch(dim3 grid, dim3 block, size_t lds, hipStream_t s, const P& p, size_t lds_allow) {
   if (lds_allow > 64 * 1024) {
     static ConvLdsAttrFlags attr_flags;
     if (const hipError_t e = conv_allow_dynamic_lds(reinterpret_cast<const void*>(KERN), attr_flags, (int)lds_allow); e != hipSuccess) return e;
@@ -43,8 +43,8 @@
   hipLaunchKernelGGL(KERN, grid, block, lds, s, p);
   return hipGetLastError();
 }
-template <auto KERN>
-hipError_t conv_launch(dim3 grid, dim3 block, size_t lds, hipStream_t s, const ConvParams& p) { return conv_launch<KERN>(grid, block, lds, s, p, lds); }
+template <auto KERN, class P>
+hipError_t conv_launch(dim3 grid, dim3 block, size_t lds, hipStream_t s, const P& p) { return conv_launch<KERN>(grid, block, lds, s, p, lds); }
 
 inline unsigned conv_magic(unsigned long long d, unsigned long long xmax, bool& exact) {
   if (d <= 1) return 0u;
diff --git a/frame-interpolation_amd/csrc/conv_igemm.hip b/frame-interpolation_amd/csrc/conv_igemm.hip
--- a/frame-interpolation_amd/csrc/conv_igemm.hip
+++ b/frame-interpolation_amd/csrc/conv_igemm.hip
@@ -209,11 +209,7 @@
   }
 }
 
-hipError_t film_launch_conv(const ConvParams& p, int tile, hipStream_t s) {
-  const int fam = conv_family_of(tile);
-  if (fam < 0 || (p.ksplit > 1 && !kConvFamily[fam].splitk)) return hipErrorInvalidValue;
-  const hipError_t e = film_launch_conv_main(p, fam, tile, s);
-  if (e != hipSuccess || p.ksplit <= 1) return e;
+static hipError_t launch_splitk_reduce(const ConvParams& p, hipStream_t s) {
   const long long Mout = (long long)p.M * (p.fold == 3 ? 4 : 1);
   if (!p.part || (p.Cout & 3) || Mout * (p.Cout >> 2) >= (1ll << 32)) return hipErrorInvalidValue;
   const unsigned units = (unsigned)Mout * (unsigned)(p.Cout >> 2);
@@ -221,3 +217,68 @@
                      p.ostride, p.ksplit, p.leaky);
   return hipGetLastError();
 }
+
+static hipError_t launch_group_wino2d(const ConvParams* p, int n, int shape, hipStream_t s, int* starts) {
+  constexpr int F = CONV_B_XCD_M;
+  switch (shape) {
+    case W2D_8x64: return conv_wino2d_launch_group_any<64, F>(p, n, s, starts);
+    case W2D_8x32: return conv_wino2d_launch_group_any<32, F>(p, n, s, starts);
+    case W2D_8x32_S2: return conv_wino2d_launch_group_any<32, F, 2>(p, n, s, starts);
+    case W2D_16x64: return conv_wino2d_launch_group_any<64, F | W2D_F_SQ>(p, n, s, starts);
+    case W2D_16x32: return conv_wino2d_launch_group_any<32, F | W2D_F_SQ>(p, n, s, starts);
+    case W2D_16x32_S2: return conv_wino2d_launch_group_any<32, F | W2D_F_SQ, 2>(p, n, s, starts);
+    default: return hipErrorInvalidValue;
+  }
+}
+static hipError_t launch_group_buf(const ConvParams* p, int n, int shape, hipStream_t s, int* starts) {
+  constexpr int F = CONV_B_XCD_M;
+  switch (shape) {
+    case TILE_128x128: return conv_buf_launch_group<128, 128, 2, 2, F>(p, n, s, starts);
+    case TILE_256x64: return conv_buf_launch_group<256, 64, 4, 1, F>(p, n, s, starts);
+    case TILE_256x32: return conv_buf_launch_group<256, 32, 4, 1, F>(p, n, s, starts);
+    case TILE_64x64: return conv_buf_launch_group<64, 64, 2, 2, F>(p, n, s, starts);
+    case TILE_128x32: return conv_buf_launch_group<128, 32, 4, 1, F>(p, n, s, starts);
+    case TILE_128x64: return conv_buf_launch_group<128, 64, 2, 2, F>(p, n, s, starts);
+    case TILE_256x128: return conv_buf_launch_group<256, 128, 4, 2, F>(p, n, s, starts);
+    default: return hipErrorInvalidValue;
+  }
+}
+
+static_assert(sizeof(ConvGroupParams) <= 4096, "kernel argument block");
+
+hipError_t film_launch_conv_group(const ConvParams* p, int n, int tile, hipStream_t s, int* starts) {
+  const int fam = conv_family_of(tile);
+  if (!p || n < 2 || n > FILM_MAX_GROUP || !(tile & CONV_TILE_XCD) || (fam != FAM_W2D && fam != FAM_BUF)) return hipErrorInvalidValue;
+  for (int i = 0; i < n; ++i)
+    if (p[i].pw_out != nullptr || (fam == FAM_BUF && p[i].pool_out != nullptr) || (fam == FAM_W2D && p[i].ksize != 3)) return hipErrorInvalidValue;
+  const int shape = conv_tile_shape(tile);
+  const hipError_t e = fam == FAM_W2D ? launch_group_wino2d(p, n, shape, s, starts) : launch_group_buf(p, n, shape, s, starts);
+  if (e != hipSuccess) return e;
+  for (int i = 0; i < n; ++i)
+    if (p[i].ksplit > 1)
+      if (const hipError_t r = launch_splitk_reduce(p[i], s); r != hipSuccess) return r;
+  return hipSuccess;
+}
+
+long long film_conv_workgroups(int tile, int NB, int H, int W, int Cout, int ksplit, int fold) {
+  const int fam = conv_family_of(tile), shape = conv_tile_shape(tile);
+  const long long z = ksplit > 1 ? ksplit : 1;
+  if (fam == FAM_W2D) {
+    const bool sq = film_w2d_square(shape);
+    const long long ntx = sq ? (W + 15) / 16 : (W + 31) / 32, nty = sq ? (H + 15) / 16 : (H + 7) / 8;
+    return NB * ntx * nty * (Cout / (film_w2d_64(shape) ? 64 : 32)) * z;
+  }
+  if (fam == FAM_BUF) {
+    const TileShape t = film_tile_shape(tile);
+    return (((long long)NB * H * W + t.bm - 1) / t.bm) * (Cout / t.bn) * (fold == 2 ? 4 : z);
+  }
+  return -1;
+}
+
+hipError_t film_launch_conv(const ConvParams& p, int tile, hipStream_t s) {
+  const int fam = conv_family_of(tile);
+  if (fam < 0 || (p.ksplit > 1 && !kConvFamily[fam].splitk)) return hipErrorInvalidValue;
+  const hipError_t e = film_launch_conv_main(p, fam, tile, s);
+  if (e != hipSuccess || p.ksplit <= 1) return e;
+  return launch_splitk_reduce(p, s);
+}
diff --git a/frame-interpolation_amd/csrc/conv_wino2d_impl.h b/frame-interpolation_amd/csrc/conv_wino2d_impl.h
--- a/frame-interpolation_amd/csrc/conv_wino2d_impl.h
+++ b/frame-interpolation_amd/csrc/conv_wino2d_impl.h
@@ -20,8 +20,20 @@
 }
 template <bool SQ> __device__ const W2dSlotTable<SQ> w2d_slot_table = w2d_make_slot_table<SQ>();
 
-template <int BN, int FLAGS, int NS_ = 3>
-__global__ __launch_bounds__(4 * (BN / 32) * 64, (BN == 32) ? 2 : 1) void conv_wino2d_kernel(ConvParams p) {
+template <int BN, int FLAGS, int NS_ = 3, bool GRP = false>
+__global__ __launch_bounds__(4 * (BN / 32) * 64, (BN == 32) ? 2 : 1) void conv_wino2d_kernel(std::conditional_t<GRP, ConvGroupParams, ConvParams> p_arg) {
+  int grp_lin = 0, grp_gx = 0, grp_gy = 0;
+  const ConvParams* grp_p = nullptr;
+  if constexpr (GRP) {
+    const int lin = (int)blockIdx.x;
+    const int mi = (lin >= p_arg.start[1] ? 1 : 0) + (lin >= p_arg.start[2] ? 1 : 0) + (lin >= p_arg.start[3] ? 1 : 0);
+    grp_lin = lin - p_arg.start[mi];
+    grp_gx = p_arg.gx[mi]; grp_gy = p_arg.gy[mi];
+    grp_p = &p_arg.m[mi];
+  } else {
+    grp_p = &p_arg;
+  }
+  const ConvParams& p = *grp_p;
   constexpr bool SQ = (FLAGS & W2D_F_SQ) != 0;
   constexpr int QW = SQ ? 4 : 8, TH = SQ ? 16 : 8, HR = TH + 2, PXW = 4 * QW, PW = PXW + 2;
   static_assert(QW * (TH / 2) == 32, "32 units per tile");
@@ -52,7 +64,8 @@
   int aH = p.H, aW = p.W, aNB = p.NB, aCtot = p.Ctot, aKsplit = p.ksplit, aNseg = p.nseg, aUnused = p.unused_chain;
   unsigned a_tpi = p.mg_tpi, a_ntx = p.mg_ntx, a_nby = p.mg_nby;
   int ntx_ = p.tl_ntx, tpi_ = p.tl_tpi;
-  int aGx = (int)gridDim.x, aGy = (int)gridDim.y;
+  int aGx, aGy;
+  if constexpr (GRP) { aGx = grp_gx; aGy = grp_gy; } else { aGx = (int)gridDim.x; aGy = (int)gridDim.y; }
   const float* aS0ptr = p.seg[0].ptr;
   int aS0stride = p.seg[0].stride, aS0C = p.seg[0].C, aS0boff = p.seg[0].boff, aS0bmod = p.seg[0].bmod;
   const float* aWptr = p.w;
@@ -68,7 +81,9 @@
   }
   unsigned long long tmK = 0, tmT = 0;
   if constexpr ((FLAGS & W2D_DBG_TIME) != 0) tmK = __builtin_readcyclecounter();
-  int bx = blockIdx.x, by = blockIdx.y;
+  int bx, by;
+  if constexpr (GRP) { bx = grp_lin; by = 0; } else { bx = blockIdx.x; by = blockIdx.y; }
+  static_assert(!GRP || (FLAGS & CONV_B_XCD_M) != 0, "a conv group runs the XCD block mapping");
   if constexpr ((FLAGS & CONV_B_XCD_M) != 0) {
     const int nbx = aGx, nby = aGy;
     const int nwg = nbx * nby;
@@ -488,10 +503,9 @@
 }
 
 template <int BN, int FLAGS, int NS = 3>
-hipError_t conv_wino2d_launch(const ConvParams& p, hipStream_t s) {
+hipError_t conv_wino2d_prepare(const ConvParams& p, ConvParams& q, dim3& grid, size_t& lds) {
   if (!(FLAGS & W2D_F_XEPI) && (p.ksplit > 1 || p.pool_out || p.pw_out)) return hipErrorInvalidValue;
-  const size_t lds = p.pw_out ? (size_t)2 * (BN / 32) * 16 * 1024 + 256 * 68 * 4 + 1024 : (size_t)NS * 24 * 1024;
-  constexpr int NT = 4 * (BN / 32) * 64;
+  lds = p.pw_out ? (size_t)2 * (BN / 32) * 16 * 1024 + 256 * 68 * 4 + 1024 : (size_t)NS * 24 * 1024;
   if (p.ksize != 3 || p.Ctot % 16 || p.Cout % BN) return hipErrorInvalidValue;
   if (p.ksplit > 1 && (!p.part || (reinterpret_cast<uintptr_t>(p.part) & 15) || p.Cout % 4 || p.pool_out || p.pw_out || p.ksplit > p.Ctot / 16)) return hipErrorInvalidValue;
   if (p.pw_out) {
@@ -510,15 +524,46 @@
   constexpr bool SQ = (FLAGS & W2D_F_SQ) != 0;
   const int ntx = SQ ? (p.W + 15) / 16 : (p.W + 31) / 32, nty = SQ ? (p.H + 15) / 16 : (p.H + 7) / 8;
   const int ntiles = p.NB * ntx * nty;
-  dim3 grid((unsigned)ntiles, p.Cout / BN, (unsigned)(p.ksplit > 1 ? p.ksplit : 1));
-  ConvParams q = p;
+  grid = dim3((unsigned)ntiles, p.Cout / BN, (unsigned)(p.ksplit > 1 ? p.ksplit : 1));
+  q = p;
   bool exact = true;
   q.mg_nby = conv_magic(grid.y, (unsigned long long)grid.x * grid.y, exact);
   q.mg_tpi = conv_magic((unsigned long long)ntx * nty, (unsigned long long)ntiles + 1, exact);
   q.mg_ntx = conv_magic(ntx, (unsigned long long)ntx * nty, exact);
   q.tl_ntx = ntx; q.tl_tpi = ntx * nty;
   if (!exact) return hipErrorInvalidValue;
-  return conv_launch<conv_wino2d_kernel<BN, FLAGS, NS>>(grid, dim3(NT), lds, s, q, 144 * 1024);
+  return hipSuccess;
+}
+
+template <int BN, int FLAGS, int NS = 3>
+hipError_t conv_wino2d_launch(const ConvParams& p, hipStream_t s) {
+  ConvParams q;
+  dim3 grid;
+  size_t lds = 0;
+  if (const hipError_t e = conv_wino2d_prepare<BN, FLAGS, NS>(p, q, grid, lds); e != hipSuccess) return e;
+  return conv_launch<conv_wino2d_kernel<BN, FLAGS, NS>>(grid, dim3(4 * (BN / 32) * 64), lds, s, q, 144 * 1024);
+}
+
+template <int BN, int FLAGS, int NS = 3>
+hipError_t conv_wino2d_launch_group(const ConvParams* p, int n, hipStream_t s, int* starts) {
+  static_assert((FLAGS & CONV_B_XCD_M) != 0, "a conv group runs the XCD block mapping");
+  if (n < 1 || n > FILM_MAX_GROUP) return hipErrorInvalidValue;
+  ConvGroupParams g{};
+  long long total = 0;
+  size_t lds = 0;
+  for (int i = 0; i < FILM_MAX_GROUP; ++i) { g.start[i] = 0x7fffffff; g.gx[i] = g.gy[i] = g.gz[i] = 1; }
+  for (int i = 0; i < n; ++i) {
+    dim3 grid;
+    if (p[i].ksplit > 1 || p[i].pw_out) return hipErrorInvalidValue;
+    if (const hipError_t e = conv_wino2d_prepare<BN, FLAGS, NS>(p[i], g.m[i], grid, lds); e != hipSuccess) return e;
+    g.start[i] = (int)total; g.gx[i] = (int)grid.x; g.gy[i] = (int)grid.y;
+    if (starts) starts[i] = (int)total;
+    total += (long long)grid.x * grid.y;
+    if (total >= (1ll << 31)) return hipErrorInvalidValue;
+  }
+  g.n = n;
+  if (starts) starts[n] = (int)total;
+  return conv_launch<conv_wino2d_kernel<BN, FLAGS, NS, true>>(dim3((unsigned)total), dim3(4 * (BN / 32) * 64), lds, s, g, 144 * 1024);
 }
 
 template <int BN, int FLAGS, int NS = 3>
@@ -526,3 +571,10 @@
   if (p.ksplit > 1 || p.pool_out || p.pw_out) return conv_wino2d_launch<BN, FLAGS | W2D_F_XEPI, NS>(p, s);
   return conv_wino2d_launch<BN, FLAGS, NS>(p, s);
 }
+
+template <int BN, int FLAGS, int NS = 3>
+hipError_t conv_wino2d_launch_group_any(const ConvParams* p, int n, hipStream_t s, int* starts) {
+  for (int i = 0; i < n; ++i)
+    if (p[i].pool_out) return conv_wino2d_launch_group<BN, FLAGS | W2D_F_XEPI, NS>(p, n, s, starts);
+  return conv_wino2d_launch_group<BN, FLAGS, NS>(p, n, s, starts);
+}
diff --git a/frame-interpolation_amd/csrc/film_engine.cpp b/frame-interpolation_amd/csrc/film_engine.cpp
--- a/frame-interpolation_amd/csrc/film_engine.cpp
+++ b/frame-interpolation_amd/csrc/film_engine.cpp
@@ -60,6 +60,7 @@
      "winograd = 2 (F(2,3) kernel on every level) needs a library built with FILM_EXTRA_FAMILIES=1"},
     {"halo_all", &film_t::opt_halo_all, BOOL, true, 0, 0, nullptr, FAM_HALO, 1, 1, "halo_all needs a library built with FILM_EXTRA_FAMILIES=1"},
     {"lanes", &film_t::opt_lanes, AS_IS, true, 0, 3, "lanes: 0, 1, 2 or 3"},
+    {"group", &film_t::opt_group, AS_IS, true, 0, 2, "group: 0 (off), 1 (conv groups among the ops of a lane) or 2 (and the whole extractor on lane 0)"},
     {"wino2d", &film_t::opt_wino2d, AS_IS, true, 0, 2, "wino2d: 0, 1 or 2"},
     {"w2d_small_px", &film_t::opt_w2d_small_px, AS_IS, true, 0, 1 << 30, "w2d_small_px: pixels per image, 0 = never"},
     {"w2d_min_px", &film_t::opt_w2d_min_px, AS_IS, true, 1, 1 << 30, "w2d_min_px: pixels per image"},
diff --git a/frame-interpolation_amd/csrc/film_exec.cpp b/frame-interpolation_amd/csrc/film_exec.cpp
--- a/frame-interpolation_amd/csrc/film_exec.cpp
+++ b/frame-interpolation_amd/csrc/film_exec.cpp
@@ -6,32 +6,34 @@
 inline float* mptr(float* base, const View& v) { return base + v.off; }
 }
 
+ConvParams conv_params(const OpDesc& op, float* arena, const float* wts) {
+  ConvParams p{};
+  p.nseg = op.nseg;
+  for (int i = 0; i < op.nseg; ++i) {
+    p.seg[i].ptr = cptr(arena, op.seg[i].v);
+    p.seg[i].stride = op.seg[i].v.stride;
+    p.seg[i].C = op.seg[i].v.C;
+    p.seg[i].boff = op.seg[i].boff; p.seg[i].bmod = op.seg[i].bmod; p.seg[i].up = op.seg[i].up;
+  }
+  p.ksize = op.ksize;
+  p.w = wts + op.*kConvFamily[op.family].weights;
+  p.bias = wts + op.b_off;
+  p.out = mptr(arena, op.out); p.ostride = op.out.stride;
+  p.NB = op.NB; p.H = op.H; p.W = op.W; p.Cout = op.Cout; p.Ctot = op.Ctot; p.leaky = op.leaky;
+  p.M = op.NB * op.H * op.W;
+  p.fold = op.fold; p.py = op.py; p.px = op.px; p.ftaps = op.ftaps;
+  p.ksplit = op.ksplit; p.part = op.ksplit > 1 ? arena + op.part_off : nullptr;
+  if (op.out2.buf >= 0) { p.pool_out = mptr(arena, op.out2); p.pool_ostride = op.out2.stride; }
+  if (op.pw_out.buf >= 0) {
+    p.pw_w = wts + op.w2_off; p.pw_bias = wts + op.b2_off; p.pw_out = mptr(arena, op.pw_out); p.pw_ostride = op.pw_out.stride; p.pw_cout = op.pw_cout;
+  }
+  for (int q = 0; q < 4; ++q) { p.tdy[q] = (signed char)op.tdy[q]; p.tdx[q] = (signed char)op.tdx[q]; p.fold_woff[q] = op.fold_woff[q]; }
+  return p;
+}
+
 hipError_t launch_op(const OpDesc& op, float* arena, const float* wts, hipStream_t s) {
   switch (op.kind) {
-    case OP_CONV: {
-      ConvParams p{};
-      p.nseg = op.nseg;
-      for (int i = 0; i < op.nseg; ++i) {
-        p.seg[i].ptr = cptr(arena, op.seg[i].v);
-        p.seg[i].stride = op.seg[i].v.stride;
-        p.seg[i].C = op.seg[i].v.C;
-        p.seg[i].boff = op.seg[i].boff; p.seg[i].bmod = op.seg[i].bmod; p.seg[i].up = op.seg[i].up;
-      }
-      p.ksize = op.ksize;
-      p.w = wts + op.*kConvFamily[op.family].weights;
-      p.bias = wts + op.b_off;
-      p.out = mptr(arena, op.out); p.ostride = op.out.stride;
-      p.NB = op.NB; p.H = op.H; p.W = op.W; p.Cout = op.Cout; p.Ctot = op.Ctot; p.leaky = op.leaky;
-      p.M = op.NB * op.H * op.W;
-      p.fold = op.fold; p.py = op.py; p.px = op.px; p.ftaps = op.ftaps;
-      p.ksplit = op.ksplit; p.part = op.ksplit > 1 ? arena + op.part_off : nullptr;
-      if (op.out2.buf >= 0) { p.pool_out = mptr(arena, op.out2); p.pool_ostride = op.out2.stride; }
-      if (op.pw_out.buf >= 0) {
-        p.pw_w = wts + op.w2_off; p.pw_bias = wts + op.b2_off; p.pw_out = mptr(arena, op.pw_out); p.pw_ostride = op.pw_out.stride; p.pw_cout = op.pw_cout;
-      }
-      for (int q = 0; q < 4; ++q) { p.tdy[q] = (signed char)op.tdy[q]; p.tdx[q] = (signed char)op.tdx[q]; p.fold_woff[q] = op.fold_woff[q]; }
-      return film_launch_conv(p, op.tile, s);
-    }
+    case OP_CONV: return film_launch_conv(conv_params(op, arena, wts), op.tile, s);
     case OP_FLOW_HEAD: {
       FlowHeadParams p{};
       p.in = cptr(arena, op.in); p.istride = op.in.stride; p.Cin = op.Ctot;
@@ -91,6 +93,38 @@
   return hipErrorInvalidValue;
 }
 
+std::vector<ItemLaunch> item_launches(const Plan& P, const SchedItem& it) {
+  std::vector<ItemLaunch> out;
+  if (it.ops.size() > 1 && !it.solo && it.tile >= 0) { out.push_back({it.ops, it.tile}); return out; }
+  std::vector<char> used(it.ops.size(), 0);
+  for (size_t a = 0; a < it.ops.size(); ++a) {
+    if (used[a]) continue;
+    const int tile = P.ops[it.ops[a]].tile;
+    ItemLaunch l{{it.ops[a]}, tile};
+    used[a] = 1;
+    if (!it.solo && (tile & CONV_TILE_XCD))
+      for (size_t b = a + 1; b < it.ops.size(); ++b)
+        if (!used[b] && P.ops[it.ops[b]].tile == tile) { l.ops.push_back(it.ops[b]); used[b] = 1; }
+    out.push_back(l);
+  }
+  return out;
+}
+
+hipError_t launch_item(const Plan& P, const SchedItem& it, const float* wts, hipStream_t s) {
+  if (it.ops.size() == 1) return launch_op(P.ops[it.ops[0]], P.arena, wts, s);
+  for (const ItemLaunch& l : item_launches(P, it)) {
+    hipError_t e;
+    if (l.ops.size() == 1) e = launch_op(P.ops[l.ops[0]], P.arena, wts, s);
+    else {
+      ConvParams cp[FILM_MAX_GROUP];
+      for (size_t i = 0; i < l.ops.size(); ++i) cp[i] = conv_params(P.ops[l.ops[i]], P.arena, wts);
+      e = film_launch_conv_group(cp, (int)l.ops.size(), l.tile, s);
+    }
+    if (e != hipSuccess) return e;
+  }
+  return hipSuccess;
+}
+
 bool batch_splittable(const OpDesc& op, int nparts) {
   return op.kind == OP_CONV && op.nseg == 1 && op.seg[0].bmod == 0 && op.seg[0].boff == 0 && op.seg[0].up == 0 && op.ksplit <= 1 && op.fold == 0 &&
          op.NB >= nparts && op.NB % nparts == 0 && (op.out2.buf < 0 || (!(op.H & 1) && !(op.W & 1)));
@@ -118,12 +152,25 @@
     return P->lane_ev[i];
   };
   const bool two_lanes = h->opt_lanes != 0;
+  const bool grouped = P->n_groups > 0 && !lp;
   hipError_t le = hipSuccess;
   if (two_lanes) {
     le = hipEventRecord(event_of(nops), main);
     if (le == hipSuccess) le = hipStreamWaitEvent(h->stream2, event_of(nops), 0);
   }
-  for (size_t i = 0; i < nops && le == hipSuccess; ++i) {
+  for (size_t i = 0; grouped && i < P->sched.size() && le == hipSuccess; ++i) {
+    const SchedItem& it = P->sched[i];
+    hipStream_t ls = (two_lanes && it.lane == 1) ? h->stream2 : main;
+    if (two_lanes)
+      for (int d : it.waits) {
+        le = hipStreamWaitEvent(ls, event_of((size_t)P->sched[d].ops[0]), 0);
+        if (le != hipSuccess) break;
+      }
+    if (le != hipSuccess) break;
+    le = launch_item(*P, it, h->packed_dev, ls);
+    if (le == hipSuccess && two_lanes && it.signal) le = hipEventRecord(event_of((size_t)it.ops[0]), ls);
+  }
+  for (size_t i = 0; !grouped && i < nops && le == hipSuccess; ++i) {
     const OpDesc& op = P->ops[i];
     const int lane = (two_lanes && op.lane == 1) ? 1 : 0;
     hipStream_t ls = lane ? h->stream2 : main;
@@ -199,6 +246,8 @@
   } else if (h->opt_graph == 2 && h->opt_lanes != 0) {
     const hipError_t le = issue_lanes(h, P, s, false);
     if (le != hipSuccess) return fail(h, FILM_ERR_HIP, "kernel launch failed: %s", hipGetErrorString(le));
+  } else if (P->n_groups > 0) {
+    for (const SchedItem& it : P->sched) HIPCHK(h, launch_item(*P, it, h->packed_dev, s));
   } else {
     for (const OpDesc& op : P->ops) HIPCHK(h, launch_op(op, P->arena, h->packed_dev, s));
   }
diff --git a/frame-interpolation_amd/csrc/film_internal.h b/frame-interpolation_amd/csrc/film_internal.h
--- a/frame-interpolation_amd/csrc/film_internal.h
+++ b/frame-interpolation_amd/csrc/film_internal.h
@@ -64,6 +64,7 @@
   int ftaps = 0; int tdy[4] = {0, 0, 0, 0}, tdx[4] = {0, 0, 0, 0};
   int64_t fold_woff[4] = {0, 0, 0, 0};
   int lane = 0;
+  int group = -1;
   std::vector<int> xdeps;
   bool signal = false;
   View in, in2, out;
@@ -100,6 +101,15 @@
   std::vector<float> data;
 };
 
+struct SchedItem {
+  std::vector<int> ops;
+  int lane = 0;
+  std::vector<int> waits;
+  bool signal = false;
+  bool solo = false;
+  int tile = -1;
+};
+
 struct Plan {
   int B = 0, H = 0, W = 0;
   int tiles = 0;
@@ -110,6 +120,9 @@
   uint64_t id = 0;
   std::vector<Buffer> bufs;
   std::vector<OpDesc> ops;
+  std::vector<SchedItem> sched;
+  int n_groups = 0;
+  size_t n_pyramid = 0;
   int64_t arena_floats = 0;
   float* arena = nullptr;
   hipGraphExec_t graph_exec = nullptr;
@@ -186,6 +199,7 @@
   int opt_tune_ms = 0;
   int opt_lanes = 1;
   hipStream_t stream2 = nullptr;
+  int opt_group = 0;
   int opt_precision = 0;
   int opt_wino2d = 1;
   int opt_w2d_min_px = 1536;
@@ -242,6 +256,10 @@
 int copy_out_string(film_t* h, const std::string& s, char* buf, int64_t cap, int64_t* needed);
 
 hipError_t launch_op(const OpDesc& op, float* arena, const float* wts, hipStream_t s);
+struct ItemLaunch { std::vector<int> ops; int tile; };
+std::vector<ItemLaunch> item_launches(const Plan& P, const SchedItem& it);
+hipError_t launch_item(const Plan& P, const SchedItem& it, const float* wts, hipStream_t s);
+ConvParams conv_params(const OpDesc& op, float* arena, const float* wts);
 bool batch_splittable(const OpDesc& op, int nparts);
 OpDesc batch_part(const OpDesc& op, int part, int nparts);
 struct LanePipe {
diff --git a/frame-interpolation_amd/csrc/film_kernels.h b/frame-interpolation_amd/csrc/film_kernels.h
--- a/frame-interpolation_amd/csrc/film_kernels.h
+++ b/frame-interpolation_amd/csrc/film_kernels.h
@@ -41,6 +41,14 @@
   const float* pw_bias;
   float* pw_out;
   int pw_ostride, pw_cout;
+};
+
+#define FILM_MAX_GROUP 4
+struct ConvGroupParams {
+  ConvParams m[FILM_MAX_GROUP];
+  int start[FILM_MAX_GROUP];
+  int gx[FILM_MAX_GROUP], gy[FILM_MAX_GROUP], gz[FILM_MAX_GROUP];
+  int n;
 };
 
 struct FlowHeadParams {
@@ -260,6 +268,8 @@
 constexpr int conv_default_tile(int f, int Cout, int64_t M) { return conv_tile(f, kConvFamily[f].default_shape(Cout, M), true); }
 
 hipError_t film_launch_conv(const ConvParams& p, int tile, hipStream_t s);
+hipError_t film_launch_conv_group(const ConvParams* p, int n, int tile, hipStream_t s, int* starts = nullptr);
+long long film_conv_workgroups(int tile, int NB, int H, int W, int Cout, int ksplit, int fold);
 hipError_t film_launch_conv_pw(const ConvPwParams& p, hipStream_t s);
 hipError_t film_launch_flow_head(const FlowHeadParams& p, hipStream_t s);
 hipError_t film_launch_pool(const PoolParams& p, hipStream_t s);
diff --git a/frame-interpolation_amd/csrc/film_planner.cpp b/frame-interpolation_amd/csrc/film_planner.cpp
--- a/frame-interpolation_amd/csrc/film_planner.cpp
+++ b/frame-interpolation_amd/csrc/film_planner.cpp
@@ -472,6 +472,7 @@
     P->B = B; P->H = H0; P->W = W0; P->tiles = T; P->slot = slot;
     add_buffers();
     emit_image_pyramids();
+    P->n_pyramid = P->ops.size();
     for (int i = 0; i < NL; ++i) emit_extractor(i);
     P->n_extract = P->ops.size();
     for (int l = NL - 1; l >= 0; --l) emit_flow(l);
@@ -492,6 +493,8 @@
     if (bad) return fail(h, FILM_ERR_INVALID, "%s", bad_msg.c_str());
     P->arena_floats = cursor;
     analyze_lanes();
+    mark_groups();
+    build_schedule();
     return FILM_OK;
   }
 
@@ -538,6 +541,139 @@
       }
     }
   }
+
+  std::vector<std::vector<char>> dep, direct;
+  void find_dependencies() {
+    const size_t n = P->ops.size();
+    std::vector<std::vector<Access>> rd(n), wr(n);
+    for (size_t i = 0; i < n; ++i) accesses(P->ops[i], rd[i], wr[i]);
+    dep.assign(n, std::vector<char>(n, 0));
+    direct.assign(n, std::vector<char>(n, 0));
+    for (size_t j = 0; j < n; ++j)
+      for (size_t i = 0; i < j; ++i) {
+        bool hit = false;
+        for (const Access& w : wr[i]) {
+          for (const Access& r : rd[j]) hit |= overlap(w, r);
+          for (const Access& w2 : wr[j]) hit |= overlap(w, w2);
+        }
+        for (const Access& r : rd[i])
+          for (const Access& w2 : wr[j]) hit |= overlap(r, w2);
+        if (!hit) continue;
+        direct[j][i] = dep[j][i] = 1;
+        for (size_t k = 0; k < i; ++k) dep[j][k] |= dep[i][k];
+      }
+  }
+  int issue_lane(size_t i) const {
+    if (h->opt_group >= 2 && i >= P->n_pyramid && i < P->n_extract) return 0;
+    return P->ops[i].lane ? 1 : 0;
+  }
+  void mark_groups() {
+    for (OpDesc& op : P->ops) op.group = -1;
+    P->n_groups = 0;
+    if (!h->opt_group) return;
+    find_dependencies();
+    std::vector<std::vector<int>> groups;
+    for (size_t i = 0; i < P->ops.size(); ++i) {
+      const OpDesc& op = P->ops[i];
+      if (op.kind != OP_CONV || (op.family != FAM_W2D && op.family != FAM_BUF) || op.fold || op.pw_out.buf >= 0) continue;
+      if (op.family == FAM_W2D && op.ksplit > 1) continue;
+      bool placed = false;
+      for (std::vector<int>& g : groups) {
+        const OpDesc& a = P->ops[g[0]];
+        if (g.size() >= FILM_MAX_GROUP || a.family != op.family || a.H != op.H || a.W != op.W || a.NB != op.NB || issue_lane(g[0]) != issue_lane(i)) continue;
+        bool free = true;
+        for (int m : g) free &= !dep[i][m];
+        if (!free) continue;
+        g.push_back((int)i);
+        placed = true;
+        break;
+      }
+      if (!placed) groups.push_back({(int)i});
+    }
+    for (const std::vector<int>& g : groups) {
+      if (g.size() < 2) continue;
+      for (int m : g) P->ops[m].group = P->n_groups;
+      ++P->n_groups;
+    }
+  }
+
+  void build_schedule() {
+    const size_t n = P->ops.size();
+    P->sched.clear();
+    if (!P->n_groups) {
+      for (size_t i = 0; i < n; ++i) {
+        SchedItem it;
+        it.ops = {(int)i}; it.lane = P->ops[i].lane ? 1 : 0; it.waits = P->ops[i].xdeps; it.signal = P->ops[i].signal;
+        P->sched.push_back(it);
+      }
+      return;
+    }
+    std::vector<char> done(n, 0);
+    auto ready = [&](size_t j) {
+      for (size_t i = 0; i < j; ++i)
+        if (direct[j][i] && !done[i]) return false;
+      return true;
+    };
+    size_t left = n;
+    while (left) {
+      bool went = false;
+      for (size_t j = 0; j < n && !went; ++j) {
+        if (done[j] || !ready(j)) continue;
+        SchedItem it;
+        const int g = P->ops[j].group;
+        if (g < 0) it.ops = {(int)j};
+        else {
+          bool all = true;
+          for (size_t m = 0; m < n; ++m)
+            if (P->ops[m].group == g) { all &= ready(m); it.ops.push_back((int)m); }
+          if (!all) continue;
+        }
+        it.lane = issue_lane(j);
+        for (int m : it.ops) done[m] = 1;
+        left -= it.ops.size();
+        P->sched.push_back(it);
+        went = true;
+      }
+      if (went) continue;
+      for (size_t j = 0; j < n; ++j)
+        if (!done[j] && P->ops[j].group >= 0) {
+          const int g = P->ops[j].group;
+          for (OpDesc& op : P->ops) if (op.group == g) op.group = -1;
+          break;
+        }
+    }
+    P->n_groups = 0;
+    for (SchedItem& it : P->sched) {
+      const int g = it.ops.size() > 1 ? P->n_groups++ : -1;
+      for (int m : it.ops) P->ops[m].group = g;
+    }
+    const size_t ni = P->sched.size();
+    std::vector<std::vector<Access>> rd(ni), wr(ni);
+    for (size_t a = 0; a < ni; ++a)
+      for (int m : P->sched[a].ops) {
+        std::vector<Access> r, w;
+        accesses(P->ops[m], r, w);
+        rd[a].insert(rd[a].end(), r.begin(), r.end());
+        wr[a].insert(wr[a].end(), w.begin(), w.end());
+      }
+    long waited[2] = {-1, -1};
+    for (size_t j = 0; j < ni; ++j) {
+      SchedItem& ij = P->sched[j];
+      for (size_t ii = j; ii-- > 0;) {
+        SchedItem& oi = P->sched[ii];
+        if (oi.lane == ij.lane) continue;
+        if ((long)ii <= waited[ij.lane]) break;
+        bool hit = false;
+        for (const Access& w : wr[ii]) {
+          for (const Access& r : rd[j]) hit |= overlap(w, r);
+          for (const Access& w2 : wr[j]) hit |= overlap(w, w2);
+        }
+        for (const Access& r : rd[ii])
+          for (const Access& w2 : wr[j]) hit |= overlap(r, w2);
+        if (hit) { ij.waits.push_back((int)ii); oi.signal = true; waited[ij.lane] = (long)ii; break; }
+      }
+    }
+  }
 };
 
 }
@@ -589,7 +725,7 @@
   j.num("ww_off", op.ww_off); j.num("wx_off", op.wx_off); j.num("wfx_off", op.wfx_off); j.num("w43_off", op.w43_off); j.num("w2d_off", op.w2d_off);
   j.num("wino", fc.wino); j.num("fold", op.fold); j.num("ksplit", op.ksplit);
   j.num("py", op.py); j.num("px", op.px); j.num("ftaps", op.ftaps); j.ints("tdy", op.tdy, 4); j.ints("tdx", op.tdx, 4);
-  j.ints("fold_woff", op.fold_woff, 4); j.num("lane", op.lane); j.ints("xdeps", op.xdeps.data(), op.xdeps.size());
+  j.ints("fold_woff", op.fold_woff, 4); j.num("lane", op.lane); j.num("group", op.group); j.ints("xdeps", op.xdeps.data(), op.xdeps.size());
   j.num("w2_off", op.w2_off); j.num("b2_off", op.b2_off); j.num("c3", fc.c3);
   j.num("fscale", op.fscale); j.num("src_brot", op.src_brot); j.num("flow_brot", op.flow_brot); j.num("misc_nb", op.misc_nb); j.num("n", op.n);
   j.num("flops", op.flops); j.num("bytes", op.bytes);
@@ -616,6 +752,22 @@
     e.num("w_off", L.w_off); e.num("b_off", L.b_off); e.num("wh_off", L.wh_off); e.num("ws_off", L.ws_off); e.num("ww_off", L.ww_off); e.num("wx_off", L.wx_off);
   });
   j.objects("ops", P.ops.data(), P.ops.size(), [&](JsonObject& e, const OpDesc& op) { json_op(e, op, P); });
+  j.num("n_groups", P.n_groups);
+  j.objects("schedule", P.sched.data(), P.sched.size(), [&](JsonObject& e, const SchedItem& it) {
+    e.ints("ops", it.ops.data(), it.ops.size()); e.num("lane", it.lane); e.ints("waits", it.waits.data(), it.waits.size()); e.num("signal", (int)it.signal);
+    e.num("solo", (int)it.solo); e.num("tile", it.tile);
+    const std::vector<ItemLaunch> ls = item_launches(P, it);
+    e.objects("launches", ls.data(), ls.size(), [&](JsonObject& l, const ItemLaunch& il) {
+      std::vector<long long> starts{0};
+      for (int m : il.ops) {
+        const OpDesc& op = P.ops[m];
+        const long long wg = op.kind == OP_CONV ? film_conv_workgroups(il.tile, op.NB, op.H, op.W, op.Cout, op.ksplit, op.fold) : -1;
+        starts.push_back(starts.back() + wg);
+      }
+      l.ints("ops", il.ops.data(), il.ops.size()); l.num("tile", il.tile);
+      if (il.ops.size() > 1) l.ints("starts", starts.data(), starts.size());
+    });
+  });
   o << "}";
   return o.str();
 }
diff --git a/frame-interpolation_amd/csrc/film_plans.cpp b/frame-interpolation_amd/csrc/film_plans.cpp
--- a/frame-interpolation_amd/csrc/film_plans.cpp
+++ b/frame-interpolation_amd/csrc/film_plans.cpp
@@ -114,6 +114,7 @@
         const int want = conv_tile(fam, shape, true);
         if (std::find(cands.begin(), cands.end(), want) != cands.end()) op.tile = want;
       }
+      for (SchedItem& it : R->sched) it.tile = -1;
     }
   }
   P->last_use = ++h->tick;
diff --git a/frame-interpolation_amd/csrc/film_tune.cpp b/frame-interpolation_amd/csrc/film_tune.cpp
--- a/frame-interpolation_amd/csrc/film_tune.cpp
+++ b/frame-interpolation_amd/csrc/film_tune.cpp
@@ -88,8 +88,40 @@
 
 std::vector<int> conv_candidates(const OpDesc& op) { return kConvFamily[op.family].candidates(op); }
 
+namespace {
+std::string group_signature(const Plan& P, const SchedItem& it) {
+  std::string k = "group";
+  for (int m : it.ops) k += "&" + conv_signature(P.ops[m]);
+  return k;
+}
+std::vector<int> group_candidates(const Plan& P, const SchedItem& it) {
+  std::vector<int> common;
+  for (int tile : conv_candidates(P.ops[it.ops[0]])) {
+    bool all = (tile & CONV_TILE_XCD) != 0;
+    for (size_t i = 1; i < it.ops.size() && all; ++i) {
+      const std::vector<int> c = conv_candidates(P.ops[it.ops[i]]);
+      all = std::find(c.begin(), c.end(), tile) != c.end();
+    }
+    if (all) common.push_back(tile);
+  }
+  return common;
+}
+void apply_group_choice(SchedItem& it, int choice) { it.solo = choice == 0; it.tile = choice == 0 ? -1 : choice; }
+}
+
 int autotune_plan(film_t* h, Plan* P) {
   bool need = false;
+  for (const SchedItem& it : P->sched) {
+    if (it.ops.size() < 2) continue;
+    const std::string sig = group_signature(*P, it);
+    if (h->tune_cache.count(sig)) continue;
+    auto imp = h->tune_import.find(sig);
+    if (imp != h->tune_import.end()) {
+      const std::vector<int> cands = group_candidates(*P, it);
+      if (imp->second == 0 || std::find(cands.begin(), cands.end(), imp->second) != cands.end()) { h->tune_cache[sig] = imp->second; continue; }
+    }
+    need = true;
+  }
   for (const OpDesc& op : P->ops) {
     if (op.kind != OP_CONV) continue;
     const std::string sig = conv_signature(op);
@@ -161,6 +193,45 @@
       }
       h->tune_cache[sig] = best;
     }
+    for (const SchedItem& it : P->sched) {
+      if (it.ops.size() < 2) continue;
+      const std::string sig = group_signature(*P, it);
+      if (h->tune_cache.count(sig)) continue;
+      auto best_of = [&](const std::function<hipError_t()>& launch, float* ms_out) -> int {
+        HIPCHK(h, launch());
+        float ms_min = 1e30f;
+        for (int rep = 0; rep < 3; ++rep) {
+          float ms = 0;
+          HIPCHK(h, hipEventRecord(e0, h->stream));
+          HIPCHK(h, launch());
+          HIPCHK(h, hipEventRecord(e1, h->stream));
+          HIPCHK(h, hipEventSynchronize(e1));
+          HIPCHK(h, hipEventElapsedTime(&ms, e0, e1));
+          ms_min = std::min(ms_min, ms);
+        }
+        *ms_out = ms_min;
+        return FILM_OK;
+      };
+      float solo_ms = 0.f;
+      ConvParams cp[FILM_MAX_GROUP];
+      for (size_t i = 0; i < it.ops.size(); ++i) {
+        OpDesc trial = P->ops[it.ops[i]];
+        trial.tile = h->tune_cache.at(conv_signature(trial));
+        cp[i] = conv_params(trial, P->arena, h->packed_dev);
+        float ms = 0;
+        if (int trc = best_of([&]() { return launch_op(trial, P->arena, h->packed_dev, h->stream); }, &ms)) return trc;
+        solo_ms += ms;
+      }
+      int choice = 0;
+      float best_ms = solo_ms;
+      for (int tile : group_candidates(*P, it)) {
+        if (film_launch_conv_group(cp, (int)it.ops.size(), tile, h->stream) != hipSuccess) { (void)hipGetLastError(); continue; }
+        float ms = 0;
+        if (int trc = best_of([&]() { return film_launch_conv_group(cp, (int)it.ops.size(), tile, h->stream); }, &ms)) return trc;
+        if (ms < best_ms) { best_ms = ms; choice = tile; }
+      }
+      h->tune_cache[sig] = choice;
+    }
     (void)hipEventDestroy(e0);
     (void)hipEventDestroy(e1);
     HIPCHK(h, hipMemsetAsync(P->arena, 0, (size_t)P->arena_floats * sizeof(float), h->stream));
@@ -168,6 +239,8 @@
   }
   for (OpDesc& op : P->ops)
     if (op.kind == OP_CONV) op.tile = h->tune_cache.at(conv_signature(op));
+  for (SchedItem& it : P->sched)
+    if (it.ops.size() > 1) apply_group_choice(it, h->tune_cache.at(group_signature(*P, it)));
   return FILM_OK;
 }
 
```

After: 29.97 frames/s. Within noise of the previous version (-0.5%).
